# OSU-NLP-Group/saev

Measured on AMD Instinct MI355X. Metric: activations/sec (train step), d_in=1024 x32 k=32, higher is better.
Workload: dtype f32 (encoder: fp16 MFMA first pass with a rigorous error margin, survivors recomputed exactly in fp32; all else fp32)

## Files before the change

### saev_amd/csrc/ctx.hip

```cpp
#include <hip/hip_runtime.h>

#include <algorithm>
#include <cmath>
#include <cstdio>
#include <cstdlib>
#include <cstring>
#include <dlfcn.h>
#include <mutex>
#include <string>
#include <vector>

#include "kernels.h"

namespace {
constexpr int AUX_KSPLIT_MAX = 16;
constexpr int CAND_CAP = 4096;
constexpr int CAND_STRIDE = CAND_CAP + 256;
constexpr int TIMING_RING = 512;
constexpr int DEAD_LAG = 4;
constexpr int DEAD_RING = 16;
enum { AUX_NONE = 0, AUX_SMALL_DEVICE = 1, AUX_SMALL_HOST = 2, AUX_DENSE = 3 };
}

struct saev_ctx {
    saev_cfg cfg{};
    saev_debug_cfg dbg{};
    int device = 0;
    std::string err;
    float* params = nullptr;
    float* grads = nullptr;
    float* adam_m = nullptr;
    float* adam_v = nullptr;
    long n_params = 0;
    long off_W_dec = 0, off_b_dec = 0, off_W_enc = 0, off_b_enc = 0;
    int shard_world = 1;
    long chunk_a = 0, chunk_b = 0;
    double* sumsq_bound = nullptr;
    hipEvent_t wdec_ready = nullptr;
    hipEvent_t wenc_ready = nullptr;
    std::vector<void*> allocs;
    size_t scratch_bytes = 0, aux_bytes = 0;
    int cuts_last[MAX_PREFIXES] = {0};
    int32_t *cand_cnt = nullptr, *gmax = nullptr, *cand_idx = nullptr;
    int gmax_stride = 0;
    float* cand_val = nullptr;
    float* h_dense = nullptr;
    int32_t *idx = nullptr, *aux_idx = nullptr;
    float *val = nullptr, *aux_val = nullptr;
    float *x_hat = nullptr, *g = nullptr, *g_aux = nullptr;
    RowStats* rowstats = nullptr;
    uint32_t* bitmap = nullptr;
    int32_t* grp_prefix = nullptr;
    int32_t* scan_totals = nullptr;
    int32_t csc_epoch = 0;
    int bitmap_words = 0;
    int back_rows = 0;
    int bitmap_words_last = 0;
    bool bitmap_clean = false;
    int bitmap_clean_words = 0;
    int bitmap_prefill_words = 0, bitmap_prefill_rows = 0;
    bool last_backward_gathered = false;
    int32_t *counts = nullptr, *starts = nullptr;
    int2* pairs = nullptr;
    float* colsum_partials = nullptr;
    float* dval_pairs = nullptr;
    double *sumsq_partials = nullptr, *sumsq_total = nullptr;
    bool wenc_sq_valid = false;
    float2* row_proj = nullptr;
    float* enc_sq = nullptr;
    bool row_proj_valid = false, tail_proj_in_adam = false;
    bool wenc_t_pending = false;
    int64_t* toks = nullptr;
    int32_t *fired = nullptr, *dead = nullptr;
    int32_t* flags = nullptr;
    int32_t *chunk_starts = nullptr, *part_starts = nullptr, *work_latent = nullptr;
    float *dW_encT = nullptr, *partials = nullptr, *db_partials = nullptr;
    bool dws_ok = false;
    int dws_rows = 0;
    bool dws_pairs = false;
    float *gS = nullptr, *xS = nullptr, *dvp = nullptr;
    float* xS_ov = nullptr;
    float* xS_bwd = nullptr;
    float* dval_rows = nullptr;
    bool dval_fwd = false;
    float* wn2 = nullptr;
    float* sq_wave = nullptr;
    int sq_wave_n = 0;
    bool wn2_fresh = false;
    float* WdS = nullptr;
    double* dec_part = nullptr;
    bool wds_fresh = false;
    bool dval_pairs_ready = false;
    bool fused_forward = false;
    bool fwd_slices = false;
    bool fwd_step = false;
    float* rs_part = nullptr;
    float* xS_c = nullptr;
    int2 *pv = nullptr, *pv2 = nullptr;
    int32_t *plat = nullptr, *cut_lat = nullptr, *cut_list = nullptr;
    int32_t* lat_unused = nullptr;
    bool fused_step = false;
    bool unused_valid = false;
    int P = 1;
    int32_t cuts[MAX_PREFIXES] = {0};
    float* G = nullptr;
    float* GS = nullptr;
    int P_cap = 0;
    int n_dead_host = 0, k_use_host = 0;
    int64_t tokens_seen = 0;
    bool tracker_dirty = false;
    int nd_cap = 0;
    DeadRecord* rec_host = nullptr;
    DeadRecord* rec_dev = nullptr;
    hipEvent_t dead_ev[DEAD_RING];
    bool dead_ev_created = false;
    int64_t dead_steps = 0;
    int64_t rec_valid_from = 1;
    int aux_route = AUX_NONE;
    int64_t n_readbacks = 0;
    std::vector<void*> aux_allocs;
    int32_t* dead_list = nullptr;
    float *Wenc_dead = nullptr, *Wdec_dead = nullptr, *H_dead = nullptr, *A_dead = nullptr, *dWd = nullptr, *dWe = nullptr,
          *dbe = nullptr, *aux_partials = nullptr, *WencT_dead = nullptr, *aux_small_part = nullptr, *aux_small_part2 = nullptr, *aux_small_partbe = nullptr;
    bool aux_dev_count = false;
    bool aux_small = false;
    int aux_mfma_bound = 0;
    int aux_ndp = AUX_SMALL_MAX;
    int aux_mfma_cap = AUX_SMALL_MAX;
    bool aux_mfma = false;
    bool aux_fused = false;
    bool aux_all = false;
    uint8_t* A_mask = nullptr;
    _Float16 *aux_ws1 = nullptr, *aux_ws2 = nullptr, *aux_xsA = nullptr, *aux_xsg = nullptr, *aux_kA = nullptr, *aux_kD = nullptr, *aux_kX = nullptr;
    bool aux_both = false;
    float* aux_parts = nullptr;
    int aux_kpad = 0;
    float *bias_dead = nullptr, *zero_bias = nullptr, *aux_scales = nullptr;
    float* aux_sync = nullptr;
    int aux_Dp2 = 0;
    float *row_margin = nullptr, *wnorm_scratch = nullptr, *surv_val = nullptr;
    int32_t *surv_idx = nullptr, *surv_cnt = nullptr, *surv_rng = nullptr;
    int rs_lat_range = 0, rs_n_ranges = 0;
    int32_t* tau_max = nullptr;
    float* heur_state = nullptr;
    float *f16r_scales = nullptr, *mu = nullptr, *xnorm = nullptr, *b_shift = nullptr, *dot_part = nullptr, *xabs_part = nullptr,
          *sq_part = nullptr, *wmax_prev = nullptr;
    bool wmax_known = false;
    bool mu_ready = false;
    bool stream_ok = false;
    float *WeS = nullptr;
    float *xn_part = nullptr, *amax_part = nullptr, *cmax_part = nullptr;
    float* b_seen = nullptr;
    int32_t *stale_host = nullptr, *stale_dev = nullptr;
    uint32_t* wchk = nullptr;
    float *mu_keep = nullptr, *xside_keep = nullptr;
    bool fwd_streamed = false;
    bool fwd_moves_mu = false;
    int64_t fwd_mu_serial = -1;
    bool borrow_streamed = false;
    bool follow_stream = false;
    bool wchk_valid = false;
    bool fwd_reused_wimg = false;
    uint32_t stale_salt = 0;
    int scale_par = 0;
    bool prep_valid = false;
    bool wimg_fresh = false;
    int64_t mu_serial = 0, wimg_mu_serial = -1;
    bool wimg_bf16_fresh = false;
    bool stream_step = false;
    bool stats_pending = false, stats_lists = false;
    bool aux_stats_pending = false;
    bool dead_list_ready = false;
    bool train_fused = false;
    const float* gather_pool = nullptr;
    const int64_t* gather_rows = nullptr;
    float *upper_c = nullptr, *mu_c = nullptr, *xnorm_c = nullptr, *xabs_c = nullptr;
    _Float16* xs_c = nullptr;
    saev_ctx* leader = nullptr;
    void* comm = nullptr;
    int comm_rank = 0, comm_world = 0;
    std::vector<saev_ctx*> followers;
    const float* xprep_x = nullptr;
    int xprep_n = 0;
    int64_t xprep_serial = 0;
    int64_t leader_serial_seen = 0;
    _Float16 *xs = nullptr, *ws = nullptr;
    int Dp = 0, S_pad = 0, MB_pad = 0;
    int max_work = 0, max_part = 0;
    float* upper = nullptr;
    saev_step_stats* stats = nullptr;
    double* stats_scratch = nullptr;
    int* tickets = nullptr;
    const float *ov_x = nullptr, *ov_g = nullptr, *ov_val = nullptr;
    const int32_t* ov_idx = nullptr;
    int ov_n = 0;
    float* db_aux = nullptr;
    bool trust_grads = false;
    const float* x_last = nullptr;
    int n_last = 0;
    int training_last = 0;
    int P_last = 1;
    bool timing = false;
    hipEvent_t ev_start[TIMING_RING], ev_stop[TIMING_RING];
    bool ev_created = false;
    long ev_count = 0;
};

#define HIPCHK(ctx, expr)                                                                    \
    do {                                                                                     \
        hipError_t _e = (expr);                                                              \
        if (_e != hipSuccess) {                                                              \
            (ctx)->err = std::string(#expr) + ": " + hipGetErrorString(_e);                  \
            return SAEV_HIP_ERROR;                                                           \
        }                                                                                    \
    } while (0)

#define REQUIRE(ctx, cond, code, msg)                                                        \
    do {                                                                                     \
        if (!(cond)) {                                                                       \
            (ctx)->err = (msg);                                                              \
            return (code);                                                                   \
        }                                                                                    \
    } while (0)

namespace {

template <typename T>
int alloc(saev_ctx* c, T** p, size_t count) {
    void* q = nullptr;
    if (count == 0) count = 1;
    hipError_t e = hipMalloc(&q, count * sizeof(T));
    if (e != hipSuccess) {
        c->err = std::string("hipMalloc failed: ") + hipGetErrorString(e);
        return SAEV_HIP_ERROR;
    }
// ... 56 lines not shown

int saev_create(const saev_cfg* cfg, int device, saev_ctx** out) { return saev_create_ex(cfg, nullptr, device, out); }

int saev_create_ex(const saev_cfg* cfg, const saev_debug_cfg* dbg, int device, saev_ctx** out) {
    if (!cfg || !out) return SAEV_INVALID_ARG;
    *out = nullptr;
    if (cfg->activation != SAEV_ACT_TOPK && cfg->activation != SAEV_ACT_RELU) return SAEV_INVALID_ARG;
    saev_cfg relu_cfg;
    if (cfg->activation == SAEV_ACT_RELU) {
        if (cfg->k_aux != 0) return SAEV_UNSUPPORTED;
        relu_cfg = *cfg;
        relu_cfg.top_k = 1;
        cfg = &relu_cfg;
    }
    if (cfg->d_model <= 0 || cfg->d_sae <= 0 || cfg->top_k <= 0 || cfg->max_batch <= 0) return SAEV_INVALID_ARG;
    if ((uint64_t)cfg->max_batch * CAND_STRIDE * 4ull >= (1ull << 32)) return SAEV_INVALID_ARG;
    if (cfg->d_model % 4 != 0 || cfg->d_sae % 4 != 0 || cfg->d_model > 4096) return SAEV_UNSUPPORTED;
    if (cfg->k_aux < 0 || cfg->k_aux > 1024) return SAEV_UNSUPPORTED;
    if (cfg->encoder_mode != SAEV_ENCODER_F32 && cfg->encoder_mode != SAEV_ENCODER_F16X3 && cfg->encoder_mode != SAEV_ENCODER_BF16 &&
        cfg->encoder_mode != SAEV_ENCODER_F16R)
        return SAEV_INVALID_ARG;
    saev_ctx* c = new saev_ctx();
    c->cfg = *cfg;
    c->cfg.top_k = std::min(cfg->top_k, cfg->d_sae);
    if (dbg != nullptr && dbg->struct_size > 0)
        std::memcpy(&c->dbg, dbg, std::min((size_t)dbg->struct_size, sizeof(saev_debug_cfg)));
    c->device = device;
    if (hipSetDevice(device) != hipSuccess) {
        delete c;
        return SAEV_HIP_ERROR;
    }
    const long S = cfg->d_sae, D = cfg->d_model, MB = cfg->max_batch, K = c->cfg.top_k, KA = cfg->k_aux;
    const long MBB = std::max<long>(MB, cfg->max_backward_rows);
    c->back_rows = (int)MBB;
    if ((uint64_t)MBB * K >= (1ull << 31)) { delete c; return SAEV_INVALID_ARG; }
    {
        saev_layout_t lay;
        saev_layout(cfg, &lay);
        c->shard_world = std::max(1, cfg->shard_world);
        c->chunk_a = lay.chunk_a; c->chunk_b = lay.chunk_b;
        c->off_W_dec = lay.off_W_dec; c->off_b_dec = lay.off_b_dec; c->off_W_enc = lay.off_W_enc; c->off_b_enc = lay.off_b_enc;
        c->n_params = lay.n_total;
    }
    int rc = SAEV_OK;
#define A(p, n) if (rc == SAEV_OK) rc = alloc(c, &c->p, (size_t)(n))
    c->gmax_stride = (int)((MB + 255) / 256 * 256);
    A(cand_cnt, MB); A(gmax, (size_t)64 * c->gmax_stride); A(cand_idx, MB * CAND_STRIDE); A(cand_val, MB * CAND_STRIDE);
    A(h_dense, MB * S);
    A(idx, MB * K); A(val, MB * K);
    if (KA > 0) { A(aux_idx, MB * KA); A(aux_val, MB * KA); A(g_aux, MB * D); A(dead_list, S); }
    A(x_hat, MB * D); A(g, MB * D);
    A(rowstats, MB);
    c->bitmap_words = (int)(((MBB + 31) / 32 + 7) / 8 * 8);
    A(bitmap, S * c->bitmap_words);
    A(grp_prefix, S * (c->bitmap_words / 8));
    A(scan_totals, ((S + 1023) / 1024) * 4);
    A(counts, S); A(starts, S + 1); A(pairs, MBB * K); A(dval_pairs, MBB * (size_t)cfg->top_k);
    {
        const long max_pairs = MBB * K;
        c->max_work = (int)(S + (max_pairs + DW_CHUNK - 1) / DW_CHUNK);
        c->max_part = (int)(2 * ((max_pairs + DW_CHUNK - 1) / DW_CHUNK) + 2);
    }
    A(chunk_starts, S + 1); A(part_starts, S); A(work_latent, c->max_work);
    A(dW_encT, S * D); A(partials, (size_t)c->max_part * 2 * D); A(db_partials, c->max_part); A(row_proj, S); A(enc_sq, S);
    {
        const bool rows_only = c->dbg.dw_route == 1;
        c->dws_ok = !rows_only && D % DWS_SLICE == 0 && (uint64_t)S * D * 4ull < (1ull << 32) && MBB < (1l << 24) &&
                    (uint64_t)MBB * K < (1ull << 31);
    }
    c->fwd_slices = c->cfg.encoder_mode == SAEV_ENCODER_F16R && (c->dbg.fwd_route == 0 || c->dbg.fwd_route == 2) && c->dbg.fused_chain == 0 && D % RS_SLICE == 0 &&
                    (uint64_t)S * 128ull < (1ull << 32) - 256ull && fused_supported(c->cfg);
    if (c->fwd_slices) {
        A(rs_part, (size_t)(D / RS_SLICE) * MB * REFINE_CAP); A(surv_rng, MB * RS_MAX_RANGES);
        c->rs_lat_range = (int)std::max<long>(RS_LAT_RANGE, ((S + RS_MAX_RANGES - 1) / RS_MAX_RANGES + 255) / 256 * 256);
        c->rs_n_ranges = (int)((S + c->rs_lat_range - 1) / c->rs_lat_range);
    }
    if (c->fwd_slices && !c->dws_ok) A(xS, MBB * D);
    if (c->dws_ok) {
        A(gS, MBB * D); A(xS, MBB * D); A(dvp, (size_t)(D / DWS_SLICE) * MBB * K);
        if (c->dbg.dw_route != 2 && decode_forms_dval((int)D, (int)K)) A(dval_rows, MB * K);
        if (c->dval_rows != nullptr && c->dbg.dw_route == 4 && decode_slices_supported((int)D, (int)S, (int)K, (int)K) && c->cfg.normalize_w_dec) {
            A(WdS, S * D); A(dec_part, (size_t)(D / 32) * MB * 3);
        }
        A(pv, MBB * K); A(pv2, MBB * K); A(plat, MBB * K); A(cut_lat, (MBB * K + DWS_RUN - 1) / DWS_RUN); A(cut_list, 4 * (1 + (MBB * K + DWS_RUN - 1) / DWS_RUN)); A(lat_unused, S);
        if (c->dval_rows != nullptr && c->dbg.fin_route == 0) { A(wn2, S); A(sq_wave, (size_t)2 * dw_slices_waves((int)D, (int)(MBB * K))); }
    }
    A(colsum_partials, ((MBB + 63) / 64) * D);
    A(sumsq_partials, 2 * 1024 + (S + 3) / 4 + 8 + transpose_blocks((int)S, (int)D)); A(sumsq_total, 1);
    if (c->cfg.encoder_mode != SAEV_ENCODER_F32 || KA > 0) {
        c->Dp = (int)((D + 31) / 32 * 32);
        c->S_pad = (int)((S + 255) / 256 * 256);
        c->MB_pad = (int)((MB + 255) / 256 * 256);
        A(zero_bias, std::max(S, D)); A(aux_scales, 16); A(aux_sync, absmax_parts_max((int)MB));
    }
    if (c->cfg.encoder_mode != SAEV_ENCODER_F32) {
        A(xs, (size_t)c->MB_pad * 2 * c->Dp);
        A(ws, (size_t)c->S_pad * 2 * c->Dp);
        A(row_margin, MB); A(wnorm_scratch, std::max((S + 3) / 4, 3 * ((S + 255) / 256))); A(f16r_scales, 16); A(mu, D); A(xnorm, 2 * MB); A(b_shift, S);
        A(xabs_part, (MB + 3) / 4);
        if (c->cfg.encoder_mode == SAEV_ENCODER_F16R) { A(dot_part, (size_t)2 * (c->Dp / 32) * c->S_pad); A(sq_part, (size_t)2 * (c->Dp / 32) * c->S_pad); A(wmax_prev, 1); }
        if (c->cfg.encoder_mode == SAEV_ENCODER_F16R) { A(surv_idx, MB * REFINE_CAP); A(surv_val, MB * REFINE_CAP); A(surv_cnt, MB); }
    }
    c->stream_ok = c->fwd_slices && c->cfg.bound_mode == 0 && c->dbg.prep_route == 0 && D % 32 == 0 && c->Dp == (int)D;
    if (c->stream_ok) {
        A(WeS, S * D); A(xn_part, (size_t)(D / 32) * c->MB_pad * 2);
        A(amax_part, (size_t)(c->MB_pad / 256) * (D / 32)); A(cmax_part, (size_t)(c->MB_pad / 256) * (D / 32)); A(b_seen, S);
        A(mu_keep, D); A(xside_keep, 4);
    }
    if (c->stream_ok || c->cfg.encoder_mode == SAEV_ENCODER_BF16) A(wchk, (size_t)2 * ((S + 255) / 256) * ((D + 31) / 32));
    A(toks, S); A(fired, S); A(dead, S); A(flags, 16); A(upper, 1); A(stats, 1);
    A(tau_max, MB); A(heur_state, 8); A(stats_scratch, STATS_SCRATCH_DOUBLES); A(tickets, 8); A(db_aux, D);
#undef A
    if (rc != SAEV_OK) {
        for (void* p : c->allocs) hipFree(p);
        delete c;
        return rc;
    }
    hipMemset(c->toks, 0, S * sizeof(int64_t));
    hipMemset(c->fired, 0, S * sizeof(int32_t));
    hipMemset(c->dead, 0, S * sizeof(int32_t));
    hipMemset(c->flags, 0, 16 * sizeof(int32_t));
    if (c->stream_ok || c->cfg.encoder_mode == SAEV_ENCODER_BF16) {
        void* hp = nullptr;
        if (hipHostMalloc(&hp, 64, hipHostMallocMapped) == hipSuccess &&
            hipHostGetDevicePointer(reinterpret_cast<void**>(&c->stale_dev), hp, 0) == hipSuccess) {
            c->stale_host = static_cast<int32_t*>(hp);
            c->stale_host[0] = 0; c->stale_host[1] = 0;
        } else {
            if (hp) hipHostFree(hp);
            c->stale_host = nullptr; c->stale_dev = nullptr;
        }
    }
    hipMemset(c->scan_totals, 0, ((S + 1023) / 1024) * 4 * sizeof(int32_t));
    hipMemset(c->stats, 0, sizeof(saev_step_stats));
    hipMemset(c->stats_scratch, 0, STATS_SCRATCH_DOUBLES * sizeof(double));
    hipMemset(c->tickets, 0, 8 * sizeof(int));
    {
        const float init[8] = {2.6f, 0.f, 0.f, 0.f, 0.f, 0.f, 0.f, 0.f};
        hipMemcpy(c->heur_state, init, sizeof(init), hipMemcpyHostToDevice);
    }
    hipMemset(c->rowstats, 0, MB * sizeof(RowStats));
    if (c->xs) hipMemset(c->xs, 0, (size_t)c->MB_pad * 2 * c->Dp * sizeof(_Float16));
    if (c->zero_bias) hipMemset(c->zero_bias, 0, std::max(S, D) * sizeof(float));
    if (c->f16r_scales) hipMemset(c->f16r_scales, 0, 16 * sizeof(float));
    if (KA > 0) {
        const int s4 = (int)((S + 3) / 4 * 4);
        const int want = cfg->aux_dead_cap > 0 ? cfg->aux_dead_cap : std::max(4096, 8 * (int)KA);
        const int cap = std::min((want + 3) / 4 * 4, s4);
        rc = alloc_aux_buffers(c, cap);
        if (rc == SAEV_OK) {
            void* h = nullptr;
            if (hipHostMalloc(&h, DEAD_RING * sizeof(DeadRecord), hipHostMallocMapped) != hipSuccess ||
                hipHostGetDevicePointer(reinterpret_cast<void**>(&c->rec_dev), h, 0) != hipSuccess) {
                rc = SAEV_HIP_ERROR;
            } else {
                c->rec_host = static_cast<DeadRecord*>(h);
                std::memset(h, 0, DEAD_RING * sizeof(DeadRecord));
                for (int i = 0; i < DEAD_RING && rc == SAEV_OK; ++i)
                    if (hipEventCreateWithFlags(&c->dead_ev[i], hipEventDisableTiming) != hipSuccess) rc = SAEV_HIP_ERROR;
                c->dead_ev_created = rc == SAEV_OK;
            }
        }
        if (rc != SAEV_OK) {
            for (void* q : c->allocs) hipFree(q);
            for (void* q : c->aux_allocs) hipFree(q);
            if (c->rec_host) hipHostFree(c->rec_host);
            delete c;
// ... 192 lines not shown
    c->ev_count = 0;
    return SAEV_OK;
}

float saev_last_encoder_ms(saev_ctx* c) {
    if (!c || !c->ev_created || c->ev_count == 0) return -1.f;
    const long n = std::min<long>(c->ev_count, TIMING_RING);
    double tot = 0;
    for (long i = 0; i < n; ++i) {
        float ms = 0.f;
        if (hipEventElapsedTime(&ms, c->ev_start[i], c->ev_stop[i]) != hipSuccess) return -1.f;
        tot += ms;
    }
    return (float)(tot / n);
}


int saev_normalize_w_dec(saev_ctx* c, void* stream) {
    if (!c) return SAEV_INVALID_ARG;
    REQUIRE(c, c->params, SAEV_NOT_BOUND, "parameters not bound");
    if (!c->cfg.normalize_w_dec) return SAEV_OK;
    HIPCHK(c, launch_normalize_rows(c->params + c->off_W_dec, c->cfg.d_sae, c->cfg.d_model, (hipStream_t)stream));
    return SAEV_OK;
}

static bool bind_x_sources(saev_ctx* c, const float* x, int n, bool allow_borrow) {
    saev_ctx* l = c->leader;
    const bool borrow = allow_borrow && l != nullptr && l->xprep_x == x && l->xprep_n == n && l->xprep_serial != c->leader_serial_seen;
    saev_ctx* src = borrow ? l : c;
    c->upper_c = src->upper; c->mu_c = src->mu; c->xnorm_c = src->xnorm; c->xabs_c = src->xabs_part; c->xs_c = src->xs;
    c->borrow_streamed = borrow && l->fwd_streamed && l->mu_keep != nullptr;
    if (c->borrow_streamed) c->mu_c = l->mu_keep;
    c->fwd_step = c->fwd_slices && (src == c || src->fwd_slices);
    c->xS_c = c->fwd_step ? src->xS : nullptr;
    if (borrow) c->leader_serial_seen = l->xprep_serial;
    return borrow;
}

static int wait_wenc(saev_ctx* c, hipStream_t s) {
    if (c->wenc_ready != nullptr) {
        hipEvent_t ev = c->wenc_ready;
        c->wenc_ready = nullptr;
        HIPCHK(c, hipStreamWaitEvent(s, ev, 0));
    }
    return SAEV_OK;
}

static int prepare_encoder(saev_ctx* c, const float* x, int n, int32_t* pre_flag, hipStream_t s,
                           const float* xmax_dev = nullptr, bool x_borrowed = false, bool defer_margins = false) {
    if (c->cfg.encoder_mode == SAEV_ENCODER_F32) return SAEV_OK;
    const int D = c->cfg.d_model, S = c->cfg.d_sae;
    const bool bf = c->cfg.encoder_mode == SAEV_ENCODER_BF16;
    if (c->cfg.encoder_mode == SAEV_ENCODER_F16R) {
        if (!c->wmax_known) {
            { int rcw = wait_wenc(c, s); if (rcw != SAEV_OK) return rcw; }
            HIPCHK(c, launch_transpose(c->params + c->off_W_enc, c->dW_encT, D, S, s));
            HIPCHK(c, launch_wnorm_max(c->dW_encT, S, D, c->wnorm_scratch, c->wmax_prev, s));
            c->wmax_known = true;
        }
        if (!x_borrowed) {
            if (!c->mu_ready) { HIPCHK(c, launch_colsum(x, n, D, c->colsum_partials, c->mu, 0, nullptr, s, 0, 1.0f / (float)n)); c->mu_serial++; }
            HIPCHK(c, launch_center_stats(x, c->mu, n, D, c->xnorm, c->xabs_part, s, xmax_dev));
        }
        c->mu_ready = false;
        if (c->borrow_streamed)
            HIPCHK(c, launch_follower_scales(c->leader->xside_keep, c->wmax_prev, scl(c), pre_flag != nullptr ? pre_flag : c->flags, 0, s));
        else
        HIPCHK(c, launch_f16r_scales(c->xabs_c, (n + 3) / 4, c->wmax_prev, scl(c), s));
        float* const wt_out = (c->fwd_step && c->stream_ok) ? c->WeS : c->dW_encT;
        if (!x_borrowed && c->wenc_ready == nullptr) {
            HIPCHK(c, launch_split_f16r(x, n, D, c->Dp, c->xs, scl(c), c->mu, c->params + c->off_W_enc, S, c->S_pad, c->ws,
                                        reinterpret_cast<double*>(c->dot_part), c->sq_part, wt_out, s, c->fwd_step ? c->xS : nullptr,
                                        c->fwd_step ? 1 : 0));
        } else {
            if (!x_borrowed) HIPCHK(c, launch_split_rows(x, n, D, c->Dp, c->xs, 2, s, 1.0f, scl(c), c->mu, c->fwd_step ? c->xS : nullptr));
            { int rcw = wait_wenc(c, s); if (rcw != SAEV_OK) return rcw; }
            HIPCHK(c, launch_split_wT(c->params + c->off_W_enc, D, S, c->S_pad, c->Dp, 1.0f, c->ws, 2, s, scl(c) + 1,
                                      c->mu_c, reinterpret_cast<double*>(c->dot_part), c->sq_part, wt_out, c->fwd_step ? 1 : 0));
        }
        c->wimg_fresh = c->stream_ok && c->fwd_step && !x_borrowed && c->leader == nullptr;
        c->wimg_mu_serial = c->mu_serial;
        HIPCHK(c, launch_bias_finish(reinterpret_cast<const double*>(c->dot_part), c->sq_part, c->Dp, S, c->S_pad,
                                     scl(c) + 1, c->params + c->off_b_enc, c->b_shift, c->wnorm_scratch, s, c->b_seen));
        if (!defer_margins)
            HIPCHK(c, launch_row_margins(c->xnorm_c, n, D, c->wnorm_scratch, (S + 255) / 256, scl(c), pre_flag,
                                         c->wmax_prev, c->row_margin, s));
        return SAEV_OK;
    }
    if (!x_borrowed) HIPCHK(c, launch_split_rows(x, n, D, c->Dp, c->xs, bf ? 1 : 0, s));
    { int rcw = wait_wenc(c, s); if (rcw != SAEV_OK) return rcw; }
    c->fwd_reused_wimg = bf && c->wimg_bf16_fresh;
    if (!(bf && c->wimg_bf16_fresh))
        HIPCHK(c, launch_split_wT(c->params + c->off_W_enc, D, S, c->S_pad, c->Dp, bf ? 1.0f : 256.0f, c->ws, bf ? 1 : 0, s));
    if (bf && c->dbg.prep_route == 0 && c->Dp == D && D % 32 == 0) c->wimg_bf16_fresh = true;
    return SAEV_OK;
}

static int run_encoder(saev_ctx* c, const float* x, int n, int epi, float* h_out, const int32_t* flag, int when,
                       hipStream_t s, bool predicted = false) {
    const bool f16r = c->cfg.encoder_mode == SAEV_ENCODER_F16R;
    if (c->cfg.encoder_mode != SAEV_ENCODER_F32 && !(f16r && epi == EPI_DENSE)) {
        const bool bf = c->cfg.encoder_mode == SAEV_ENCODER_BF16;
        EncodeF16Args a{};
        a.xs = c->xs_c; a.ws = c->ws;
        a.b_enc = f16r ? c->b_shift : c->params + c->off_b_enc;
        a.n_rows = n; a.Dp = c->Dp; a.S = c->cfg.d_sae; a.w_scale = (bf || f16r) ? 1.0f : 256.0f;
        a.scale_dev = f16r ? scl(c) : nullptr;
        a.arith = bf ? 1 : (f16r ? 2 : 0);
        a.row_margin = f16r ? c->row_margin : nullptr;
        const int enc_wgs = c->dbg.enc_wgs > 0 ? c->dbg.enc_wgs : 256;
        a.mfma32 = c->dbg.enc_mfma == 32 ? 1 : 0;
        a.s_splits = encoder_splits(n, a.S, encode_f16x3_tile_rows(), encode_f16x3_tile_latents(), enc_wgs);
        a.no_rot = c->dbg.enc_rot == 1 ? 1 : 0;
        a.h_out = h_out;
        a.ngroups = f16_ngroups(c); a.top_k = c->cfg.top_k;
        a.gmax = c->gmax; a.gmax_stride = c->gmax_stride; a.cand_cnt = c->cand_cnt; a.cand_val = c->cand_val; a.cand_idx = c->cand_idx;
        a.cand_cap = CAND_CAP; a.cand_stride = CAND_STRIDE;
        a.enable_flag = flag; a.enable_when = when;
        if (predicted) { a.heur_z = c->heur_state; a.tau_max = c->tau_max; }
        {
            const int rf = c->dbg.refresh_first > 0 ? c->dbg.refresh_first : 8, re = c->dbg.refresh_every;
            a.refresh_first = std::max(1, rf);
            a.refresh_every = (re >= 1 && (re & (re - 1)) == 0) ? re : 2;
            if (a.ngroups > 32 && re <= 0) a.refresh_every = 1;
        }
        HIPCHK(c, launch_encode_f16x3(a, epi, s));
        return SAEV_OK;
    }
    EncodeArgs a{};
    a.x = x;
    a.W_enc = c->params + c->off_W_enc;
    a.b_enc = c->params + c->off_b_enc;
    a.n_rows = n;
    a.D = c->cfg.d_model;
    a.S = c->cfg.d_sae;
    a.s_splits = encoder_splits(n, a.S, encode_gemm_tile_rows(), encode_gemm_tile_latents(), 512);
    a.h_out = h_out;
    a.ngroups = c->cfg.top_k <= 32 ? 32 : 64;
    a.gmax = c->gmax;
    a.gmax_stride = c->gmax_stride;
    a.cand_cnt = c->cand_cnt;
    a.cand_val = c->cand_val;
    a.cand_idx = c->cand_idx;
    a.cand_cap = CAND_CAP; a.cand_stride = CAND_STRIDE;
    a.enable_flag = flag;
    a.enable_when = when;
    HIPCHK(c, launch_encode_gemm(a, epi, s));
    return SAEV_OK;
}

int saev_encode_dense(saev_ctx* c, const float* x, int32_t n, float* h_out, void* stream) {
    if (!c) return SAEV_INVALID_ARG;
    REQUIRE(c, c->params, SAEV_NOT_BOUND, "parameters not bound");
    REQUIRE(c, x && h_out && n > 0, SAEV_INVALID_ARG, "saev_encode_dense: bad arguments");
    REQUIRE(c, n <= c->cfg.max_batch || c->cfg.encoder_mode == SAEV_ENCODER_F32, SAEV_INVALID_ARG,
            "saev_encode_dense: n_rows > max_batch");
    bind_x_sources(c, x, n, false);
    c->xprep_x = nullptr;
    if (c->cfg.encoder_mode != SAEV_ENCODER_F16R) {
        int rc = prepare_encoder(c, x, n, nullptr, (hipStream_t)stream);
        if (rc != SAEV_OK) return rc;
    }
    return run_encoder(c, x, n, EPI_DENSE, h_out, nullptr, 0, (hipStream_t)stream);
}

int saev_topk_dense(saev_ctx* c, const float* h, int32_t n, int32_t k, const int32_t* mask, int32_t* idx_out,
                    float* val_out, void* stream) {
    if (!c) return SAEV_INVALID_ARG;
    REQUIRE(c, h && idx_out && val_out && n > 0 && k > 0, SAEV_INVALID_ARG, "saev_topk_dense: bad arguments");
    REQUIRE(c, k <= c->cfg.d_sae, SAEV_INVALID_ARG, "saev_topk_dense: k > d_sae");
    SelectDenseArgs a{};
    a.h = h; a.n_rows = n; a.S = c->cfg.d_sae; a.k = k; a.mask = mask;
    a.idx_out = idx_out; a.val_out = val_out; a.out_stride = k;
    HIPCHK(c, launch_select_dense(a, (hipStream_t)stream));
    return SAEV_OK;
}

static int encode_topk_impl(saev_ctx* c, const float* x, int n, int32_t* idx_out, float* val_out,
                            const int32_t* pre_flag, hipStream_t s, const float* xmax_dev = nullptr, bool x_borrowed = false) {
    const int K = c->cfg.top_k;
    int32_t* need_dense = c->flags + 1;
    const bool f16r_mode = c->cfg.encoder_mode == SAEV_ENCODER_F16R;
    const bool predict_mode = fused_supported(c->cfg) && c->cfg.bound_mode != 0 && c->cfg.encoder_mode != SAEV_ENCODER_F32 &&
                              f16_ngroups(c) == 32;
    const bool one_launch_pre = fused_supported(c->cfg) && !predict_mode;
    if (c->follow_stream) {
        HIPCHK(c, launch_follower_scales(c->leader->xside_keep, c->wmax_prev, scl(c), const_cast<int32_t*>(pre_flag), 1, s));
    } else if (!c->stream_step) {
        int rc0 = prepare_encoder(c, x, n, const_cast<int32_t*>(pre_flag), s, xmax_dev, x_borrowed, one_launch_pre);
        if (rc0 != SAEV_OK) return rc0;
        rc0 = wait_wenc(c, s);
        if (rc0 != SAEV_OK) return rc0;
    }
    if (fused_supported(c->cfg)) {
        const int ng = c->cfg.encoder_mode == SAEV_ENCODER_F32 ? (c->cfg.top_k <= 32 ? 32 : 64) : f16_ngroups(c);
        const bool f16r = c->cfg.encoder_mode == SAEV_ENCODER_F16R;
        auto select_stage = [&](const int32_t* flag, int when, int32_t* bad, const int32_t* tau_max, int32_t* ovf = nullptr,
                                const int32_t* first_flag = nullptr) -> int {
            SelectCandArgs sc{};
            sc.cand_cnt = c->cand_cnt; sc.cand_val = c->cand_val; sc.cand_idx = c->cand_idx;
            sc.cand_cap = CAND_CAP; sc.cand_stride = CAND_STRIDE; sc.n_rows = n; sc.k = K;
            sc.idx_out = idx_out; sc.val_out = val_out; sc.out_stride = K;
            sc.enable_flag = first_flag ? first_flag : flag; sc.enable_when = when;
            sc.tau_max = tau_max; sc.invalid = bad; sc.ovf = ovf;
            if (f16r) {
                sc.row_margin = c->row_margin; sc.x = x; sc.W_encT = c->dW_encT; sc.b_enc = c->params + c->off_b_enc;
                sc.D = c->cfg.d_model; sc.refine_overflow = bad;
                sc.surv_idx = c->surv_idx; sc.surv_val = c->surv_val; sc.surv_cnt = c->surv_cnt;
                if (c->fwd_step) { sc.surv_rng = c->surv_rng; sc.lat_range = c->rs_lat_range; sc.n_ranges = c->rs_n_ranges; }
                const bool chain_fused = c->dbg.fused_chain != 0;
                if (chain_fused && tau_max == nullptr && first_flag != nullptr) {
                    HIPCHK(c, launch_select_refine(sc, s));
                    return SAEV_OK;
                }
                HIPCHK(c, launch_select_cand(sc, s));
                sc.enable_flag = flag; sc.ovf = nullptr;
                if (c->fwd_step) {
                    RefineSlicesArgs rs{};
                    rs.surv_idx = c->surv_idx; rs.surv_cnt = c->surv_cnt; rs.surv_val = c->surv_val; rs.surv_rng = c->surv_rng;
                    rs.xS = c->xS_c; rs.WeS = c->stream_ok ? c->WeS : c->dW_encT; rs.b_enc = sc.b_enc; rs.part = c->rs_part;
                    rs.n_rows = n; rs.S = c->cfg.d_sae; rs.D = c->cfg.d_model;
                    rs.lat_range = c->rs_lat_range; rs.n_ranges = c->rs_n_ranges;
                    rs.enable_flag = flag; rs.enable_when = when;
                    const bool fold = c->dbg.fwd_route != 2;
                    HIPCHK(c, launch_refine_slices(rs, s, !fold));
                    if (fold) { sc.sum_part = c->rs_part; sc.sum_bias = sc.b_enc; sc.sum_n = c->cfg.d_model / RS_SLICE; sc.sum_plane = (size_t)n * REFINE_CAP; }
                } else {
                    HIPCHK(c, launch_refine_exact(sc, s));
                }
                sc.row_margin = nullptr; sc.tau_max = nullptr;
                sc.cand_cnt = c->surv_cnt; sc.cand_val = c->surv_val; sc.cand_idx = c->surv_idx; sc.cand_cap = REFINE_CAP; sc.cand_stride = REFINE_CAP;
            }
            HIPCHK(c, launch_select_cand(sc, s));
            return SAEV_OK;
        };
        const bool predict = c->cfg.bound_mode != 0 && ng == 32 && c->cfg.encoder_mode != SAEV_ENCODER_F32;
        int32_t *bad1 = c->flags + 9, *run2 = c->flags + 10, *gate = c->flags + 11;
        if (predict) {
            HIPCHK(c, launch_heur_gate(c->heur_state, pre_flag, gate, s));
            HIPCHK(c, launch_encoder_init(c->cand_cnt, n, c->gmax, 0, s, c->tau_max));
            timing_begin(c, s);
            int rc = run_encoder(c, x, n, EPI_TOPK, nullptr, gate, 0, s, true);
            if (rc != SAEV_OK) return rc;
            timing_end(c, s);
            HIPCHK(c, launch_overflow_check(c->cand_cnt, n, CAND_CAP, gate, bad1, c->flags + 2, c->flags + 3, s, need_dense,
                                            nullptr, c->heur_state + 3, nullptr, pre_flag));
            rc = select_stage(bad1, 0, bad1, c->tau_max);
            if (rc != SAEV_OK) return rc;
            HIPCHK(c, launch_heur_update(c->heur_state, bad1, c->heur_state + 3, K, gate, s));
            HIPCHK(c, launch_encoder_init(c->cand_cnt, n, c->gmax, ng * c->gmax_stride, s, nullptr, bad1, 1));
            rc = run_encoder(c, x, n, EPI_TOPK, nullptr, bad1, 1, s);
            if (rc != SAEV_OK) return rc;
            HIPCHK(c, launch_overflow_check(c->cand_cnt, n, CAND_CAP, pre_flag, need_dense, c->flags + 2, c->flags + 3, s, need_dense,
                                            run2, nullptr, bad1));
            rc = select_stage(run2, 1, need_dense, nullptr);
            if (rc != SAEV_OK) return rc;
        } else {
            const int S_ = c->cfg.d_sae;
            if (c->stream_step) {
                const int D_ = c->cfg.d_model;
                XprepArgs xp{};
                xp.x = c->gather_pool != nullptr ? c->gather_pool : x; xp.rows = c->gather_rows; xp.x_out = c->gather_pool != nullptr ? const_cast<float*>(x) : nullptr;
                xp.n = n; xp.D = D_; xp.nks = D_ / 32; xp.n_pad = c->MB_pad; xp.scales = scl(c); xp.mu = c->mu; xp.xs = c->xs; xp.xS = c->xS;
                xp.xn_part = c->xn_part; xp.col_part = c->colsum_partials; xp.amax_part = c->amax_part; xp.cmax_part = c->cmax_part;
                xp.W_enc = c->params + c->off_W_enc; xp.WeS = c->WeS; xp.b_enc = c->params + c->off_b_enc; xp.b_seen = c->b_seen;
                xp.S = S_; xp.salt = ++c->stale_salt; xp.stale = c->flags + 12;
                if (!c->followers.empty()) { xp.mu_keep = c->mu_keep; xp.xside_keep = c->xside_keep; }
                HIPCHK(c, launch_xprep(xp, s));
                PreEncode2Args pe{};
                pe.cand_cnt = c->cand_cnt; pe.n_rows = n; pe.gmax = c->gmax; pe.n_gmax = ng * c->gmax_stride;
                pe.xn_part = c->xn_part; pe.nks = D_ / 32; pe.n_pad = c->MB_pad; pe.D = D_;
                pe.wg_part = c->wnorm_scratch; pe.n_part = (S_ + 255) / 256; pe.scales = scl(c); pe.scales_next = scl_next(c);
                pe.pre_flag = const_cast<int32_t*>(pre_flag); pe.wmax_prev = c->wmax_prev; pe.margin = c->row_margin; pe.xnorm = c->xnorm;
                pe.flags1 = c->flags + 1; pe.col_part = c->colsum_partials; pe.n_rowblk = (n + 255) / 256; pe.mu = c->mu;
                pe.inv_n = 1.0f / (float)n; pe.update_mu = c->train_fused ? 1 : 0;
                pe.amax_part = c->amax_part; pe.cmax_part = c->cmax_part; pe.n_img = ((n + 255) / 256) * (D_ / 32);
                pe.upper = c->upper; pe.stats = c->stats; pe.stale = c->flags + 12; pe.stale_host = c->stale_dev;
                pe.xside_keep = c->followers.empty() ? nullptr : c->xside_keep;
                HIPCHK(c, launch_pre_encode2(pe, s));
                if (c->train_fused) c->mu_serial++;
            } else
            HIPCHK(c, launch_pre_encode(c->cand_cnt, n, c->gmax, ng * c->gmax_stride, f16r_mode ? c->xnorm_c : nullptr, c->cfg.d_model,
                                        c->wnorm_scratch, (S_ + 255) / 256, f16r_mode ? scl(c) : nullptr, const_cast<int32_t*>(pre_flag),
                                        c->wmax_prev, c->row_margin, c->flags + 1, s));
            timing_begin(c, s);
            int rc = run_encoder(c, x, n, EPI_TOPK, nullptr, pre_flag, 0, s);
            if (rc != SAEV_OK) return rc;
            timing_end(c, s);
            rc = select_stage(need_dense, 0, need_dense, nullptr, c->flags + 1, pre_flag);
            if (rc != SAEV_OK) return rc;
        }
    } else {
        HIPCHK(c, launch_init_i32(need_dense, 1, 1, s));
        HIPCHK(c, hipMemsetAsync(c->flags + 2, 0, 2 * sizeof(int32_t), s));
        timing_begin(c, s);
        timing_end(c, s);
    }
    int rc = run_encoder(c, x, n, EPI_DENSE, c->h_dense, need_dense, 1, s);
    if (rc != SAEV_OK) return rc;
    SelectDenseArgs sd{};
    sd.h = c->h_dense; sd.n_rows = n; sd.S = c->cfg.d_sae; sd.k = K;
    sd.idx_out = idx_out; sd.val_out = val_out; sd.out_stride = K;
    sd.enable_flag = need_dense; sd.enable_when = 1;
    HIPCHK(c, launch_select_dense(sd, s));
    return SAEV_OK;
}

int saev_encode_topk(saev_ctx* c, const float* x, int32_t n, int32_t* idx_out, float* val_out, void* stream) {
    if (!c) return SAEV_INVALID_ARG;
    REQUIRE(c, c->cfg.activation == SAEV_ACT_TOPK, SAEV_UNSUPPORTED, "saev_encode_topk: a ReLU context runs the forward entries only");
    REQUIRE(c, c->params, SAEV_NOT_BOUND, "parameters not bound");
    REQUIRE(c, x && idx_out && val_out && n > 0 && n <= c->cfg.max_batch, SAEV_INVALID_ARG,
            "saev_encode_topk: bad arguments (n_rows must be in 1..max_batch)");
    hipStream_t s = (hipStream_t)stream;
    HIPCHK(c, hipMemsetAsync(c->flags, 0, sizeof(int32_t), s));
    bind_x_sources(c, x, n, false);
    c->xprep_x = nullptr;
    c->stream_step = false;
    c->follow_stream = false;
    return encode_topk_impl(c, x, n, idx_out, val_out, c->flags, s);
}

int saev_scatter_dense(saev_ctx* c, const int32_t* idx, const float* val, int32_t n, int32_t k, float* f_out,
                       void* stream) {
    if (!c) return SAEV_INVALID_ARG;
    REQUIRE(c, idx && val && f_out && n > 0 && k > 0, SAEV_INVALID_ARG, "saev_scatter_dense: bad arguments");
    HIPCHK(c, launch_scatter_dense(idx, val, n, k, k, c->cfg.d_sae, f_out, (hipStream_t)stream));
    return SAEV_OK;
}

int saev_decode_sparse(saev_ctx* c, const int32_t* idx, const float* val, int32_t n, int32_t k,
                       const int64_t* prefixes_host, int32_t n_prefixes, float* x_hats_out, void* stream) {
    if (!c) return SAEV_INVALID_ARG;
    REQUIRE(c, c->params, SAEV_NOT_BOUND, "parameters not bound");
    REQUIRE(c, idx && val && x_hats_out && n > 0 && k > 0, SAEV_INVALID_ARG, "saev_decode_sparse: bad arguments");
    const int S = c->cfg.d_sae, D = c->cfg.d_model;
    int64_t single = S;
    if (!prefixes_host) { prefixes_host = &single; n_prefixes = 1; }
    REQUIRE(c, n_prefixes >= 1 && prefixes_host[n_prefixes - 1] == S && prefixes_host[0] >= 1, SAEV_INVALID_ARG,
            "prefixes must end at d_sae and start at >= 1");
    for (int p = 1; p < n_prefixes; ++p)
        REQUIRE(c, prefixes_host[p] > prefixes_host[p - 1], SAEV_INVALID_ARG, "prefixes must be strictly increasing");
    REQUIRE(c, n <= c->cfg.max_batch || n_prefixes == 1, SAEV_INVALID_ARG, "n_rows > max_batch");
    hipStream_t s = (hipStream_t)stream;
    for (int p = 0; p < n_prefixes; ++p) {
        DecodeArgs a{};
        a.x = nullptr;
        a.idx = idx; a.val = val; a.code_stride = k; a.k = k;
        a.W_dec = c->params + c->off_W_dec; a.b_dec = c->params + c->off_b_dec;
        a.n_rows = n; a.D = D; a.S = S; a.idx_limit = (int)prefixes_host[p];
// ... 530 lines not shown
                c->aux_route = AUX_SMALL_DEVICE;
                return auxk_small_forward(c, s, bound);
            }
            if ((bound + 3) / 4 * 4 <= c->nd_cap) {
                c->aux_route = AUX_DENSE;
                c->aux_dev_count = true;
                c->n_dead_host = bound;
                c->k_use_host = std::min(c->cfg.k_aux, bound);
                return auxk_forward(c, s);
            }
        }
    }
    int32_t host[2] = {0, 0};
    HIPCHK(c, hipMemcpyAsync(host, c->flags + 4, 2 * sizeof(int32_t), hipMemcpyDeviceToHost, s));
    HIPCHK(c, hipStreamSynchronize(s));
    c->n_readbacks++;
    c->n_dead_host = host[0];
    c->k_use_host = host[1];
    if (c->n_dead_host <= 0) return SAEV_OK;
    if ((c->n_dead_host + 3) / 4 * 4 > c->nd_cap && !(c->n_dead_host <= small_max && c->cfg.d_model <= 2048)) {
        const int s4 = (S + 3) / 4 * 4;
        const int cap = std::min(s4, std::max(2 * c->nd_cap, (2 * c->n_dead_host + 1023) / 1024 * 1024));
        for (void* q : c->aux_allocs) hipFree(q);
        c->aux_allocs.clear();
        c->aux_bytes = 0;
        c->nd_cap = 0;
        int rcg = alloc_aux_buffers(c, cap);
        if (rcg != SAEV_OK) {
            c->err = "AuxK: " + std::to_string(c->n_dead_host) + " dead latents exceed saev_cfg.aux_dead_cap and the buffers could not be grown to " +
                     std::to_string(cap) + " (out of device memory)";
            return rcg;
        }
        std::fprintf(stderr, "[saev_amd] AuxK: %d dead latents exceeded the dead-set buffers; grown to %d inside the step "
                             "(device-synchronising; saev_cfg.aux_dead_cap sizes them up front)\n", c->n_dead_host, cap);
    }
    if (c->n_dead_host <= small_max && c->cfg.d_model <= 2048) {
        c->aux_route = AUX_SMALL_HOST;
        return auxk_small_forward(c, s, c->n_dead_host);
    }
    c->aux_route = AUX_DENSE;
    return auxk_forward(c, s);
}


int saev_backward_begin(saev_ctx* c, void* stream) {
    if (!c) return SAEV_INVALID_ARG;
    REQUIRE(c, c->x_last && c->training_last, SAEV_INVALID_ARG, "saev_backward_begin: no training forward in flight");
    REQUIRE(c, c->grads, SAEV_NOT_BOUND, "gradient buffer not bound");
    hipStream_t s = (hipStream_t)stream;
    const int S = c->cfg.d_sae, D = c->cfg.d_model, K = c->cfg.top_k;
    const bool ov = c->ov_x != nullptr;
    const int n = ov ? c->ov_n : c->n_last;
    const int words = ((n + 31) / 32 + 7) / 8 * 8;
    c->row_proj_valid = false;
    CscArgs a{};
    a.idx = ov ? c->ov_idx : c->idx; a.code_stride = K; a.k = K; a.k_dev = nullptr; a.n_rows = n; a.S = S;
    a.bitmap = c->bitmap; a.words = words; a.grp_prefix = c->grp_prefix; a.scan_totals = c->scan_totals;
    a.counts = c->counts; a.starts = c->starts; a.pairs = c->pairs;
    a.chunk_starts = c->chunk_starts; a.part_starts = c->part_starts; a.work_latent = c->work_latent;
    const bool ov_slices = ov && c->dws_ok && c->P_last == 1 && n <= c->back_rows;
    c->dws_pairs = ov ? ov_slices : c->dws_rows == n;
    if (ov_slices) {
        c->xS_bwd = c->xS;
        if (!c->followers.empty()) {
            if (c->xS_ov == nullptr) {
                int rca = alloc(c, &c->xS_ov, (size_t)c->back_rows * D);
                if (rca != SAEV_OK) return rca;
            }
            c->xS_bwd = c->xS_ov;
        }
        HIPCHK(c, launch_slice_major_copy(c->ov_g, c->ov_x, n, D, c->gS, c->xS_bwd, s));
        c->dws_rows = 0;
    }
    c->csc_epoch = c->csc_epoch == 0x7fffffff ? 1 : c->csc_epoch + 1;
    a.epoch = c->dbg.csc_route == 2 ? 0 : c->csc_epoch;
    if (c->dws_pairs) {
        a.zero_word = c->cut_list;
        a.pv = c->pv; a.plat = c->plat; a.val = ov ? c->ov_val : c->val;
        a.P = c->P_last;
        for (int p = 0; p < c->P_last; ++p) a.cuts[p] = c->cuts_last[p];
        if (!ov && c->dval_fwd) { a.pv2 = c->pv2; a.dval = c->dval_rows; }
    }
    c->dval_pairs_ready = c->dws_pairs && a.pv2 != nullptr;
    if (c->fused_step && c->dws_pairs) { a.pairs = nullptr; a.chunk_starts = nullptr; a.part_starts = nullptr; a.work_latent = nullptr; }
    const float* gmat = ov ? c->ov_g : (c->P_last > 1 ? c->G : c->g);
    const bool prefilled = !ov && c->bitmap_prefill_words == words && c->bitmap_prefill_rows == n;
    HIPCHK(c, launch_csc_build(a, s, c->bitmap_clean && words <= c->bitmap_clean_words, gmat, D, (long)c->P_last * D,
                               c->colsum_partials, c->grads + c->off_b_dec, prefilled));
    c->bitmap_prefill_words = 0;
    c->last_backward_gathered = ov;
    c->bitmap_clean = false;
    c->bitmap_words_last = words;
    if (c->aux_route != AUX_NONE) {
        int rc = auxk_backward(c, s);
        if (rc != SAEV_OK) return rc;
    }
    return SAEV_OK;
}

int saev_backward_rows(saev_ctx* c, int32_t lat_lo, int32_t lat_hi, void* stream) {
    return saev_backward_rows_part(c, lat_lo, lat_hi, 0, stream);
}

int saev_backward_rows_part(saev_ctx* c, int32_t lat_lo, int32_t lat_hi, int32_t part, void* stream) {
    if (!c) return SAEV_INVALID_ARG;
    REQUIRE(c, part >= 0 && part <= 2, SAEV_INVALID_ARG, "saev_backward_rows_part: part must be 0 (both), 1 (decoder) or 2 (encoder)");
    REQUIRE(c, c->x_last && c->training_last && c->grads, SAEV_INVALID_ARG, "saev_backward_rows: call saev_backward_begin first");
    const int S = c->cfg.d_sae, D = c->cfg.d_model, K = c->cfg.top_k;
    const bool ov = c->ov_x != nullptr;
    const int n = ov ? c->ov_n : c->n_last;
    REQUIRE(c, 0 <= lat_lo && lat_lo < lat_hi && lat_hi <= S, SAEV_INVALID_ARG, "saev_backward_rows: bad latent range");
    hipStream_t s = (hipStream_t)stream;
    DwRowsArgs a{};
    a.starts = c->starts; a.chunk_starts = c->chunk_starts; a.work_latent = c->work_latent;
    a.part_starts = c->part_starts; a.pairs = c->pairs; a.val = ov ? c->ov_val : c->val; a.W_dec = c->params + c->off_W_dec;
    a.g = ov ? c->ov_g : (c->P_last > 1 ? c->G : c->g);
    a.x = ov ? c->ov_x : c->x_last;
    a.D = D; a.S = S; a.k_dev = nullptr; a.accumulate = 0;
    a.P = c->P_last;
    for (int p = 0; p < c->P_last; ++p) a.cuts[p] = c->cuts_last[p];
    a.dW_dec = c->grads + c->off_W_dec; a.dW_encT = c->dW_encT; a.db_enc = c->grads + c->off_b_enc;
    a.partials = c->partials; a.db_partials = c->db_partials;
    a.lat_lo = lat_lo; a.lat_hi = lat_hi;
    a.part = part; a.dval = c->dval_pairs;
    const bool all_rows = part == 0 && lat_lo == 0 && lat_hi == S;
    const bool clears = part != 2 && lat_lo == 0 && lat_hi == S && c->bitmap_words_last > 0;
    if (clears) { a.clear_bitmap = c->bitmap; a.clear_words = c->bitmap_words_last; }
    a.row_proj = all_rows ? c->row_proj : nullptr; a.project = c->cfg.remove_parallel_grads ? 1 : 0;
    a.enc_sq = all_rows ? c->enc_sq : nullptr;
    const int max_work = (lat_hi - lat_lo) + (int)(((long)n * K + DW_CHUNK - 1) / DW_CHUNK);
    if (lat_lo == 0 && lat_hi == S && c->dws_pairs && (ov || c->dws_rows == n)) {
        DwSlicesArgs w{};
        w.starts = c->starts; w.pv = c->pv; w.pv2 = c->pv2; w.plat = c->plat; w.gS = c->P_last > 1 ? c->GS : c->gS; w.W_dec = a.W_dec; w.P = c->P_last;
        w.xS = ov ? c->xS_bwd : (c->fwd_step ? c->xS_c : c->xS);
        w.n_rows = n; w.D = D; w.S = S; w.pair_cap = (int)((long)c->back_rows * K);
        w.dvp = c->dvp; w.dW_dec = a.dW_dec; w.dW_encT = a.dW_encT; w.db_enc = a.db_enc;
        const size_t runs_cap = ((size_t)w.pair_cap + DWS_RUN - 1) / DWS_RUN;
        w.part_dec = c->partials; w.part_enc = c->partials + 2 * runs_cap * D;
        w.cut_lat = c->cut_lat; w.cut_list = c->cut_list;
        w.lat_unused = (all_rows && c->fused_step) ? c->lat_unused : nullptr;
        c->unused_valid = w.lat_unused != nullptr;
        w.row_proj = a.row_proj; w.project = a.project; w.enc_sq = a.enc_sq;
        w.clear_bitmap = a.clear_bitmap; w.clear_words = a.clear_words;
        w.have_dval = c->dval_pairs_ready ? 1 : 0;
        c->sq_wave_n = 0;
        if (c->dval_pairs_ready && c->wn2_fresh && part == 0) {
            w.wn2 = c->wn2;
            if (c->fused_step && all_rows && c->sq_wave != nullptr && c->dbg.fin_route != 2) {
                c->sq_wave_n = dw_slices_waves(D, (int)((long)n * K));
                w.sq_wave_dec = c->sq_wave; w.sq_wave_enc = c->sq_wave + c->sq_wave_n;
            }
        }
        HIPCHK(c, launch_dw_slices(w, (int)((long)n * K), part, s));
    } else {
        c->unused_valid = false;
        HIPCHK(c, launch_dw_rows(a, max_work, s));
    }
    if (c->aux_route == AUX_DENSE)
        HIPCHK(c, launch_scatter_add_dead(c->dead_list, c->n_dead_host, D, c->dWd, c->dWe, c->dbe, c->grads + c->off_W_dec,
                                          c->dW_encT, c->grads + c->off_b_enc, lat_lo, lat_hi, s,
                                          c->aux_dev_count ? c->flags + 4 : nullptr, part, a.row_proj, a.W_dec, a.project, a.enc_sq,
                                          c->unused_valid ? c->lat_unused : nullptr, c->sq_wave_n > 0 ? c->starts : nullptr));
    else if (c->aux_route != AUX_NONE)
        HIPCHK(c, launch_scatter_add_dead(c->dead_list, c->aux_mfma ? c->aux_ndp : AUX_SMALL_MAX, D, c->dWd, c->dWe, c->dbe, c->grads + c->off_W_dec,
                                          c->dW_encT, c->grads + c->off_b_enc, lat_lo, lat_hi, s, c->flags + 4, part,
                                          a.row_proj, a.W_dec, a.project, a.enc_sq, c->unused_valid ? c->lat_unused : nullptr,
                                          c->sq_wave_n > 0 ? c->starts : nullptr));
    if (ov && c->aux_route != AUX_NONE && part != 2 && lat_lo == 0)
        HIPCHK(c, launch_colsum(c->db_aux, 1, D, c->colsum_partials, c->grads + c->off_b_dec, 1, nullptr, s));
    c->row_proj_valid = all_rows;
    if (clears) { c->bitmap_clean = true; c->bitmap_clean_words = c->bitmap_words_last; }
    return SAEV_OK;
}

float* saev_grad_w_enc_t(saev_ctx* c) { return c ? c->dW_encT : nullptr; }

int saev_bind_w_enc_t(saev_ctx* c, float* scratch) {
    if (!c || !scratch) return SAEV_INVALID_ARG;
    c->dW_encT = scratch;
    return SAEV_OK;
}

int saev_copy_step_state(saev_ctx* c, int32_t n_rows, float* g_out, int32_t* idx_out, float* val_out, void* stream) {
    if (!c) return SAEV_INVALID_ARG;
    REQUIRE(c, c->n_last > 0 && c->training_last && n_rows == c->n_last, SAEV_INVALID_ARG,
            "saev_copy_step_state: n_rows must be the row count of the training forward in flight");
    hipStream_t s = (hipStream_t)stream;
    const size_t nk = (size_t)n_rows * c->cfg.top_k, nd = (size_t)n_rows * c->cfg.d_model * (size_t)c->P_last;
    if (g_out) HIPCHK(c, hipMemcpyAsync(g_out, c->P_last > 1 ? c->G : c->g, nd * sizeof(float), hipMemcpyDeviceToDevice, s));
    if (idx_out) HIPCHK(c, hipMemcpyAsync(idx_out, c->idx, nk * sizeof(int32_t), hipMemcpyDeviceToDevice, s));
    if (val_out) HIPCHK(c, hipMemcpyAsync(val_out, c->val, nk * sizeof(float), hipMemcpyDeviceToDevice, s));
    return SAEV_OK;
}

int saev_backward_override(saev_ctx* c, const float* x_all, const float* g_all, const int32_t* idx_all, const float* val_all,
                           int32_t n_all) {
    if (!c) return SAEV_INVALID_ARG;
    if (x_all == nullptr) { c->ov_x = nullptr; c->ov_n = 0; return SAEV_OK; }
    REQUIRE(c, g_all && idx_all && val_all && n_all > 0, SAEV_INVALID_ARG, "saev_backward_override: NULL buffer");
    REQUIRE(c, n_all <= c->back_rows, SAEV_INVALID_ARG,
            "saev_backward_override: the gathered row count exceeds saev_cfg.max_backward_rows (set it to the GLOBAL batch)");
    REQUIRE(c, c->x_last && c->training_last, SAEV_INVALID_ARG, "saev_backward_override: no training forward in flight");
    REQUIRE(c, ((uintptr_t)x_all % 16) == 0 && ((uintptr_t)g_all % 16) == 0, SAEV_INVALID_ARG, "x_all / g_all must be 16-byte aligned");
    c->ov_x = x_all; c->ov_g = g_all; c->ov_idx = idx_all; c->ov_val = val_all; c->ov_n = n_all;
    return SAEV_OK;
}

int32_t saev_aux_compact_rows(const saev_ctx* c) {
    if (!c || c->aux_route == AUX_NONE) return 0;
    return c->aux_route == AUX_DENSE ? (c->n_dead_host + 3) / 4 * 4 : (c->aux_mfma ? c->aux_ndp : AUX_SMALL_MAX);
}

static int aux_compact_copy(saev_ctx* c, float* buf, bool out, hipStream_t s) {
    const size_t rows = (size_t)saev_aux_compact_rows(c), D = c->cfg.d_model;
    if (rows == 0) return SAEV_OK;
    REQUIRE(c, buf != nullptr, SAEV_INVALID_ARG, "saev_aux_compact_*: NULL buffer");
    float* seg[4] = {c->dWd, c->dWe, c->dbe, c->db_aux};
    const size_t len[4] = {rows * D, rows * D, rows, D};
    size_t off = 0;
    for (int i = 0; i < 4; ++i) {
        if (out) HIPCHK(c, hipMemcpyAsync(buf + off, seg[i], len[i] * sizeof(float), hipMemcpyDeviceToDevice, s));
        else HIPCHK(c, hipMemcpyAsync(seg[i], buf + off, len[i] * sizeof(float), hipMemcpyDeviceToDevice, s));
        off += len[i];
    }
    return SAEV_OK;
}
int saev_aux_compact_export(saev_ctx* c, float* buf, void* stream) {
    if (!c) return SAEV_INVALID_ARG;
    return aux_compact_copy(c, buf, true, (hipStream_t)stream);
}
// ... 68 lines not shown
    if (rc != SAEV_OK) return rc;
    hipStream_t s = (hipStream_t)stream;
    const long S = c->cfg.d_sae, D = c->cfg.d_model;
    c->tail_proj_in_adam = false;
    if (c->wenc_t_pending) {
        REQUIRE(c, c->row_proj_valid && shard_rank < 0, SAEV_INVALID_ARG, "saev_tail_prepare: pending transposed gradient without a full backward");
        c->row_proj_valid = false;
        HIPCHK(c, launch_sumsq_final_ex(nullptr, 0, c->row_proj, (int)S, c->grads + S * D, r.a_hi - S * D,
                                        c->grads + c->off_b_enc, r.b_hi - c->off_b_enc, saev_sumsq_device(c), c->sumsq_partials,
                                        c->tickets + 1, s, c->enc_sq, c->sq_wave_n > 0 ? c->sq_wave : nullptr, 2l * c->sq_wave_n));
        c->sq_wave_n = 0;
        c->tail_proj_in_adam = true;
        return SAEV_OK;
    }
    if (c->trust_grads && c->wenc_sq_valid && c->row_proj_valid && shard_rank < 0) {
        c->wenc_sq_valid = false; c->row_proj_valid = false;
        const double* tsq = c->sumsq_partials + 2 * sumsq_blocks() + (S + 3) / 4;
        HIPCHK(c, launch_sumsq_final_ex(tsq, transpose_blocks((int)S, (int)D), c->row_proj, (int)S, c->grads + S * D, r.a_hi - S * D,
                                        c->grads + c->off_b_enc, r.b_hi - c->off_b_enc, saev_sumsq_device(c), c->sumsq_partials,
                                        c->tickets + 1, s));
        c->tail_proj_in_adam = true;
        return SAEV_OK;
    }
    c->row_proj_valid = false;
    const long row_lo = std::min(r.a_lo / D, S), row_hi = std::min(r.a_hi / D, S);
    const int n_rows = (int)(row_hi - row_lo);
    const int nb = sumsq_blocks();
    double* part = c->sumsq_partials;
    HIPCHK(c, launch_rpg(c->grads + row_lo * D, c->params + row_lo * D, n_rows, (int)D, s, part + 2 * nb,
                         c->cfg.remove_parallel_grads ? 1 : 0));
    const long rest_lo = std::max(r.a_lo, S * D);
    HIPCHK(c, launch_sumsq_partials(c->grads + rest_lo, std::max(0L, r.a_hi - rest_lo), part, s));
    c->wenc_sq_valid = false;
    HIPCHK(c, launch_sumsq_partials(c->grads + r.b_lo, r.b_hi - r.b_lo, part + nb, s));
    HIPCHK(c, launch_sumsq_final(part, 2 * nb + (n_rows + 3) / 4, saev_sumsq_device(c), s));
    return SAEV_OK;
}

int saev_tail_apply(saev_ctx* c, float lr, float max_norm, float grad_scale, int64_t adam_step, int32_t shard_rank,
                    void* stream) {
    if (!c) return SAEV_INVALID_ARG;
    REQUIRE(c, c->cfg.activation == SAEV_ACT_TOPK, SAEV_UNSUPPORTED, "saev_tail_apply: a ReLU context runs the forward entries only");
    REQUIRE(c, c->params && c->grads && c->adam_m && c->adam_v, SAEV_NOT_BOUND,
            "saev_tail_apply: params/grads/adam state not bound");
    REQUIRE(c, adam_step >= 1, SAEV_INVALID_ARG, "adam_step is 1-based");
    TailRanges r;
    int rc = tail_ranges(c, shard_rank, &r);
    if (rc != SAEV_OK) return rc;
    hipStream_t s = (hipStream_t)stream;
    c->wn2_fresh = false;
    const bool emit_follow = c->leader != nullptr && c->borrow_streamed && c->leader->fwd_moves_mu && c->dbg.group_route == 0 &&
                             c->cfg.encoder_mode == SAEV_ENCODER_F16R && c->fwd_step;
    const bool emit = c->train_fused && c->stream_ok && (c->leader == nullptr ? c->prep_valid && (c->followers.empty() || c->dbg.group_route == 0) : emit_follow) &&
                      shard_rank < 0 && c->tail_proj_in_adam && c->wenc_t_pending;
    c->wimg_fresh = false;
    const bool chk_was_valid = c->wchk_valid;
    c->wchk_valid = false;
    const bool emit_bf16 = c->train_fused && c->cfg.encoder_mode == SAEV_ENCODER_BF16 && c->wimg_bf16_fresh && shard_rank < 0 &&
                           c->tail_proj_in_adam && c->wenc_t_pending;
    c->wimg_bf16_fresh = false;
    AdamArgs a{};
    a.lr = lr; a.beta1 = 0.9f; a.beta2 = 0.999f; a.eps = 1e-8f;
    a.omb1 = (float)(1.0 - 0.9); a.omb2 = (float)(1.0 - 0.999);
    a.bc1 = (float)(1.0 - std::pow(0.9, (double)adam_step));
    a.bc2_sqrt = (float)std::sqrt(1.0 - std::pow(0.999, (double)adam_step));
    a.grad_scale = grad_scale; a.max_norm = max_norm; a.sumsq = saev_sumsq_device(c); a.stats = c->stats;
    const long lo[2] = {r.a_lo, r.b_lo}, hi[2] = {r.a_hi, r.b_hi};
    if (shard_rank < 0 && c->tail_proj_in_adam && c->wenc_t_pending) {
        c->tail_proj_in_adam = false; c->wenc_t_pending = false;
        const long S = c->cfg.d_sae, D = c->cfg.d_model;
        a.p = c->params; a.g = c->grads; a.m = c->adam_m; a.v = c->adam_v; a.n = c->n_params;
        AdamImageArgs im{};
        if (emit) {
            if (!c->stream_step) HIPCHK(c, hipMemcpyAsync(scl_next(c), scl(c), 8 * sizeof(float), hipMemcpyDeviceToDevice, s));
            im.ws = c->ws; im.WeS = c->WeS; im.dot_part = reinterpret_cast<double*>(c->dot_part); im.sq_part = c->sq_part;
            im.mu = c->leader != nullptr ? c->leader->mu : c->mu; im.wmax_prev = c->wmax_prev; im.scales_next = scl_next(c); im.nks = c->Dp / 32; im.S_pad = c->S_pad;
        }
        if (emit_bf16) { im.ws = c->ws; im.nks = c->Dp / 32; im.S_pad = c->S_pad; im.mode = 1; }
        if ((emit || emit_bf16) && c->wchk != nullptr && c->dbg.own_check == 0) {
            im.chk = c->wchk; im.late = c->stale_dev != nullptr ? c->stale_dev + 1 : nullptr;
            im.verify = (chk_was_valid && c->fwd_reused_wimg && im.late != nullptr) ? 1 : 0;
            im.early = (emit && c->leader == nullptr) ? c->flags + 13 : nullptr;
        }
        HIPCHK(c, launch_adam_fused(a, c->row_proj, c->dW_encT, (int)S, (int)D, S * D, c->off_W_enc - S * D, c->off_W_enc,
                                    c->off_b_enc, c->n_params - c->off_b_enc, s, c->unused_valid ? c->lat_unused : nullptr,
                                    (emit || emit_bf16) ? &im : nullptr));
        c->unused_valid = false;
        c->wchk_valid = (emit || emit_bf16) && c->wchk != nullptr && c->dbg.own_check == 0;
        c->wimg_bf16_fresh = emit_bf16;
        if (emit) {
            HIPCHK(c, launch_bias_finish(reinterpret_cast<const double*>(c->dot_part), c->sq_part, c->Dp, (int)S, c->S_pad, scl_next(c) + 1,
                                         c->params + c->off_b_enc, c->b_shift, c->wnorm_scratch, s, c->b_seen));
            c->scale_par ^= 1;
            c->wimg_fresh = true;
            c->wimg_mu_serial = c->leader != nullptr ? c->leader->mu_serial : c->mu_serial;
        }
        return SAEV_OK;
    }
    if (shard_rank < 0 && c->tail_proj_in_adam) {
        c->tail_proj_in_adam = false;
        const long S = c->cfg.d_sae, D = c->cfg.d_model;
        a.p = c->params; a.g = c->grads; a.m = c->adam_m; a.v = c->adam_v; a.n = S * D;
        HIPCHK(c, launch_adam_rows(a, c->row_proj, (int)S, (int)D, s));
        a.p += S * D; a.g += S * D; a.m += S * D; a.v += S * D; a.n = c->n_params - S * D;
        HIPCHK(c, launch_adam(a, s));
        return SAEV_OK;
    }
    c->tail_proj_in_adam = false;
    if (shard_rank < 0) {
        a.p = c->params; a.g = c->grads; a.m = c->adam_m; a.v = c->adam_v; a.n = c->n_params;
        HIPCHK(c, launch_adam(a, s));
        return SAEV_OK;
    }
    for (int h = 0; h < 2; ++h) {
        a.p = c->params + lo[h]; a.g = c->grads + lo[h]; a.m = c->adam_m + lo[h]; a.v = c->adam_v + lo[h]; a.n = hi[h] - lo[h];
        HIPCHK(c, launch_adam(a, s));
    }
    return SAEV_OK;
}

int saev_step_tail(saev_ctx* c, float lr, float max_norm, float grad_scale, int64_t adam_step, void* stream) {
    int rc = saev_tail_prepare(c, -1, stream);
    if (rc != SAEV_OK) return rc;
    return saev_tail_apply(c, lr, max_norm, grad_scale, adam_step, -1, stream);
}

int saev_train_step_gather(saev_ctx* c, const float* pool, const int64_t* rows, float* x_out, int32_t n, float lr, float max_norm,
                           int64_t adam_step, void* stream) {
    if (!c) return SAEV_INVALID_ARG;
    REQUIRE(c, pool && rows && x_out, SAEV_INVALID_ARG, "saev_train_step_gather: NULL buffer");
    c->gather_pool = pool; c->gather_rows = rows;
    const int rc = saev_train_step(c, x_out, n, lr, max_norm, adam_step, stream);
    c->gather_pool = nullptr; c->gather_rows = nullptr;
    return rc;
}

int saev_params_touched(saev_ctx* c) {
    if (!c) return SAEV_INVALID_ARG;
    c->wchk_valid = false;
    c->wimg_fresh = false;
    c->wimg_bf16_fresh = false;
    c->wn2_fresh = false;
    return SAEV_OK;
}

int saev_train_step(saev_ctx* c, const float* x, int32_t n, float lr, float max_norm, int64_t adam_step,
                    void* stream) {
    if (!c) return SAEV_INVALID_ARG;
    c->fused_forward = c->dws_ok && c->GS != nullptr;
    c->train_fused = true;
    int rc = saev_step_forward(c, x, n, n, 1, stream);
    c->fused_forward = false;
    if (rc != SAEV_OK) { c->train_fused = false; return rc; }
    rc = saev_step_dead(c, n, stream);
    if (rc != SAEV_OK) { c->train_fused = false; return rc; }
    c->fused_step = true;
    rc = saev_backward_begin(c, stream);
    if (rc == SAEV_OK) rc = saev_backward_rows(c, 0, c->cfg.d_sae, stream);
    c->fused_step = false;
    if (rc != SAEV_OK) { c->train_fused = false; return rc; }
    c->wenc_t_pending = true;
    rc = saev_step_tail(c, lr, max_norm, 1.0f, adam_step, stream);
    c->wenc_t_pending = false;
    c->train_fused = false;
    return rc;
}

namespace {
struct RcclApi {
    void* lib = nullptr;
    int (*GetUniqueId)(void*) = nullptr;
    int (*CommInitRank)(void**, int, const void*, int) = nullptr;
    int (*CommDestroy)(void*) = nullptr;
    int (*CommAbort)(void*) = nullptr;
    int (*AllReduce)(const void*, void*, size_t, int, int, void*, hipStream_t) = nullptr;
// ... 100 lines not shown
```

### saev_amd/csrc/kernels.h

```cpp
#pragma once
#include <hip/hip_runtime.h>
#include <stdint.h>

#include "../../include/saev_amd.h"

enum { EPI_DENSE = 0, EPI_TOPK = 1 };

struct EncodeArgs {
    const float* x;
    const float* W_enc;
    const float* b_enc;
    int n_rows, D, S;
    int s_splits;
    float* h_out;
    int ngroups;
    int32_t* gmax;
    int gmax_stride;
    int32_t* cand_cnt;
    float* cand_val;
    int32_t* cand_idx;
    int cand_cap;
    int cand_stride;
    const int32_t* enable_flag;
    int enable_when;
// ... 77 lines not shown
hipError_t launch_pow2_scale(const float* absmax, float* pair, hipStream_t stream);
hipError_t launch_center_stats(const float* x, const float* mu, int n, int D, float* xnorm, float* wg_absmax,
                               hipStream_t stream, const float* xmax = nullptr);
hipError_t launch_row_margins(const float* xnorm, int n, int D, const float* wg_part, int n_part, const float* scales,
                              int32_t* pre_flag, float* wmax_prev, float* margin, hipStream_t stream);
hipError_t launch_overflow_check(const int32_t* cand_cnt, int n_rows, int cap, const int32_t* pre_flag,
                                 int32_t* need_dense, int32_t* n_overflow, int32_t* cand_max, hipStream_t stream,
                                 int32_t* dense_out = nullptr, int32_t* run_out = nullptr, float* cand_mean = nullptr,
                                 const int32_t* enable_flag = nullptr, const int32_t* dense_src = nullptr);

struct __attribute__((aligned(8))) RowStats {
    float sse_scaled;
    float l0;
    float l1;
    float aux_sse;
    double sse64;
    double sumsq64;
};

struct DecodeArgs {
    const float* x;
    const int32_t* idx;
    const float* val;
    int code_stride, k;
    const float* W_dec;
    const float* b_dec;
    int n_rows, D, S;
    int idx_limit;
    const float* upper;
    float gscale;
    int training;
    float* g;
    float* x_hat;
    int32_t* fired;
    RowStats* rowstats;
    float* gS;
    float* xS;
    float* dval_out;
    uint32_t* csc_bitmap;
    int csc_words;
};
hipError_t launch_decode(const DecodeArgs& a, hipStream_t stream);
bool decode_forms_dval(int D, int k);
bool decode_matry_forms_dval(int D, int k);
struct DecodeSliceArgs {
    DecodeArgs d;
    const float* WdS;
    double* part;
    float* dvp;
    long dvp_pitch;
};
bool decode_slices_supported(int D, int S, int k, int code_stride);
hipError_t launch_decode_slices(const DecodeSliceArgs& a, hipStream_t stream);

constexpr int MAX_PREFIXES = 16;
struct MatryArgs {
    int P;
    int32_t cuts[MAX_PREFIXES];
    float* G;
    int g_rows_all;
};
hipError_t launch_decode_matry(const DecodeArgs& a, const MatryArgs& m, hipStream_t stream);

struct CscArgs {
    const int32_t* idx;
    int code_stride, k;
    const int32_t* k_dev;
    int n_rows, S;
    uint32_t* bitmap;
    int words;
    int32_t* grp_prefix;
    int32_t* counts;
    int32_t* scan_totals;
    int32_t* starts;
    int2* pairs;
    int32_t* chunk_starts;
    int32_t* part_starts;
    int32_t* work_latent;
    int2* pv;
    int32_t* plat;
    const float* val;
    int2* pv2;
    const float* dval;
    int P;
    int32_t cuts[16];
    int32_t* zero_word;
    int32_t epoch;
};
hipError_t launch_csc_build(const CscArgs& a, hipStream_t stream, bool bitmap_clean = false, const float* colsum_m = nullptr,
                            int colsum_D = 0, long colsum_row_stride = 0, float* colsum_partials = nullptr,
                            float* colsum_out = nullptr, bool prefilled = false);

constexpr int DW_CHUNK = 64;

struct DwRowsArgs {
    const int32_t* starts;
    const int32_t* chunk_starts;
    const int32_t* work_latent;
    const int32_t* part_starts;
    const int2* pairs;
    const float* val;
    const float* W_dec;
    const float* g;
    const float* x;
    int D, S;
    int P;
    int32_t cuts[MAX_PREFIXES];
    const int32_t* k_dev;
    int accumulate;
    float* dW_dec;
    float* dW_encT;
    float* db_enc;
    float* partials;
    float* db_partials;
    int lat_lo, lat_hi;
    int part;
    float* dval;
    float2* row_proj;
    int project;
    float* enc_sq;
    uint32_t* clear_bitmap;
    int clear_words;
};
hipError_t launch_dw_rows(const DwRowsArgs& a, int max_work, hipStream_t stream);

constexpr int DWS_RUN = 64, DWS_SLICE = 32;
constexpr int DWS_FIRST = 1, DWS_LAST = 2, DWS_END = 4;
struct DwSlicesArgs {
    const int32_t* starts;
    const int2* pv;
    int2* pv2;
    const int32_t* plat;
    const float* gS;
    const float* xS;
    const float* W_dec;
    int n_rows, D, S, pair_cap;
    int P;
    float* dvp;
    float* dW_dec;
    float* dW_encT;
    float* db_enc;
    float* part_dec;
    float* part_enc;
    int32_t* cut_lat;
    int32_t* cut_list;
    float2* row_proj;
    int project;
    float* enc_sq;
    uint32_t* clear_bitmap;
    int clear_words;
    int32_t* lat_unused;
    int have_dval;
    const float* wn2;
    float* sq_wave_dec;
    float* sq_wave_enc;
};
hipError_t launch_dw_slices(const DwSlicesArgs& a, int max_pairs, int part, hipStream_t stream);
int dw_slices_waves(int D, int max_pairs);
hipError_t launch_slice_major_copy(const float* g, const float* x, int n, int D, float* gS, float* xS, hipStream_t stream);
hipError_t launch_transpose(const float* in, float* out, int S, int D, hipStream_t stream, double* sq_part = nullptr);
int transpose_blocks(int S, int D);

hipError_t launch_colsum(const float* m, int n_rows, int D, float* partials, float* out, int accumulate,
                         const int32_t* k_dev, hipStream_t stream, long row_stride = 0, float out_scale = 1.0f,
                         int col_mult = 0);
hipError_t launch_colsum_absmax(const float* m, int n_rows, int D, float* partials, float* out, float* wg_scratch,
                                float* absmax_out, hipStream_t stream, float out_scale = 1.0f,
                                saev_step_stats* zero_stats = nullptr, int32_t* zero_flag = nullptr);

hipError_t launch_normalize_rows(float* W, int S, int D, hipStream_t stream, float* WS = nullptr, float* wn2 = nullptr);
hipError_t launch_rpg(float* gW, const float* W, int S, int D, hipStream_t stream, double* sq_partials = nullptr,
                      int project = 1);
int sumsq_blocks();
hipError_t launch_sumsq_partials(const float* g, long n, double* partials, hipStream_t stream);
hipError_t launch_sumsq_final(const double* partials, int nb, double* total, hipStream_t stream);
hipError_t launch_sumsq(const float* g, long n, double* partials, double* total, hipStream_t stream);
struct AdamArgs {
    float* p; const float* g; float* m; float* v;
    long n;
    float lr, beta1, beta2, eps, bc1, bc2_sqrt;
    float omb1, omb2;
    float grad_scale;
    float max_norm;
    const double* sumsq;
    saev_step_stats* stats;
};
hipError_t launch_adam(const AdamArgs& a, hipStream_t stream);
hipError_t launch_adam_rows(const AdamArgs& a, const float2* row_proj, int S, int D, hipStream_t stream);
hipError_t launch_sumsq_final_ex(const double* partials, int nb, const float2* row_proj, int n_rows, const float* e1, long n1,
                                 const float* e2, long n2, double* total, double* blk_part, int* ticket, hipStream_t stream,
                                 const float* enc_sq = nullptr,
                                 const float* plain = nullptr, long n_plain = 0);
struct AdamImageArgs {
    _Float16* ws; float* WeS; double* dot_part; float* sq_part;
    const float* mu; const float* wmax_prev; float* scales_next;
    int nks, S_pad;
    int mode;
    uint32_t* chk; int32_t* late; int verify;
    const int32_t* early;
};
hipError_t launch_adam_fused(const AdamArgs& a, const float2* row_proj, const float* gT, int S, int D, long off_b_dec, long n_b_dec,
                             long off_W_enc, long off_b_enc, long n_b_enc, hipStream_t stream, const int32_t* lat_unused = nullptr,
                             const AdamImageArgs* img = nullptr);
constexpr int SUMSQ_EX_BLOCKS = 32;

struct DeadRecord {
    int64_t step;
    int64_t cum_tokens;
    int64_t horizon_tokens;
    int32_t n_dead;
    int32_t n_near;
};

struct DeadArgs {
    int64_t* toks;
    int32_t* fired;
    int32_t* dead;
    int S;
    int64_t add_tokens, threshold;
    int k_aux;
    int32_t* n_dead;
    int32_t* k_use;
    saev_step_stats* stats;
    int32_t* scratch;
    int64_t horizon_tokens;
    int64_t step, cum_tokens;
    DeadRecord* rec;
    int32_t* dead_list;
};
hipError_t launch_dead_update(const DeadArgs& a, hipStream_t stream);
hipError_t launch_stats_dead(const RowStats* rs, int n_rows, int D, int P, float alpha, const float* upper, const int32_t* n_overflow,
                             saev_step_stats* stats, double* scratch, const int32_t* cand_cnt, int cand_cap, const DeadArgs& d,
                             hipStream_t stream);
hipError_t launch_absmax(const float* x, long n, float* out_zeroed, hipStream_t stream);
hipError_t launch_gather_rows(const float* pool, const int64_t* rows, int n_rows, int D, float* out, hipStream_t stream);
hipError_t launch_scatter_dense(const int32_t* idx, const float* val, int n_rows, int k, int stride, int S, float* f,
                                hipStream_t stream);
hipError_t launch_stats_reduce(const RowStats* rs, int n_rows, int D, int P, float alpha, int with_aux, const float* upper,
                               const int32_t* n_overflow_and_max, saev_step_stats* stats, hipStream_t stream,
                               const int32_t* n_dead_dev, double* scratch,
                               const int32_t* cand_cnt = nullptr, int cand_cap = 0);
constexpr int STATS_SCRATCH_DOUBLES = 16 * 8 + 1;

struct EncodeF16Args {
    const _Float16* xs;
    const _Float16* ws;
    const float* b_enc;
    int n_rows, Dp, S;
    float w_scale;
    int arith;
    const float* row_margin;
    const float* scale_dev;
    const float* scale_dev_b;
    int s_splits;
    int no_rot;
    float* h_out;
    int ngroups;
    int top_k;
    int32_t* gmax;
    int gmax_stride;
    int32_t* cand_cnt;
    float* cand_val;
    int32_t* cand_idx;
    int cand_cap, cand_stride;
    const int32_t* enable_flag;
    int enable_when;
    const float* heur_z;
    int32_t* tau_max;
    int refresh_first, refresh_every;
    int n_batches;
    int blk_imgs;
    long out_bstride;
    int mfma32;
};
hipError_t launch_encode_f16x3(const EncodeF16Args& a, int epi, hipStream_t stream);
int encode_f16x3_tile_rows();
int encode_f16x3_tile_latents();
hipError_t launch_split_rows(const float* x, int n, int D, int Dp, void* xs, int mode, hipStream_t stream, float scale = 1.0f,
                             const float* scale_dev = nullptr,
                             const float* mu = nullptr,
                             float* xS = nullptr);
hipError_t launch_split_wT(const float* W, int D, int S, int S_pad, int Dp, float scale, void* ws, int mode,
                           hipStream_t stream, const float* scale_dev = nullptr,
                           const float* mu = nullptr, double* dot_part = nullptr, float* sq_part = nullptr,
                           float* W_T = nullptr,
                           int wt_slices = 0);
struct XprepArgs {
    const float* x;
    const int64_t* rows;
    float* x_out;
    int n, D, nks, n_pad;
    const float* scales;
    const float* mu;
    _Float16* xs;
    float* xS;
    float* xn_part;
    float* col_part;
    float* amax_part;
    float* cmax_part;
    const float* W_enc; const float* WeS; const float* b_enc; const float* b_seen;
    int S; uint32_t salt; int32_t* stale;
    float* mu_keep; float* xside_keep;
};
hipError_t launch_xprep(const XprepArgs& a, hipStream_t stream);
struct PreEncode2Args {
    int32_t* cand_cnt; int n_rows;
    int32_t* gmax; int n_gmax;
    const float* xn_part; int nks, n_pad, D;
    const float* wg_part; int n_part;
    const float* scales;
    float* scales_next;
    int32_t* pre_flag;
    float* wmax_prev;
    float* margin;
    float* xnorm;
    int32_t* flags1;
    const float* col_part; int n_rowblk;
    float* mu; float inv_n; int update_mu;
    const float* amax_part; const float* cmax_part; int n_img;
    float* upper;
    int32_t* stale; int32_t* stale_host;
    float* xside_keep;
    saev_step_stats* stats;
    int nb_rows;
};
hipError_t launch_pre_encode2(PreEncode2Args a, hipStream_t stream);
hipError_t launch_follower_scales(const float* xside, const float* wmax, float* scales, int32_t* pre_flag, int keep_w, hipStream_t stream);
hipError_t launch_split_both(const float* M, int R, int C, float scale, const float* scale_dev, void* rf, int kp_r, void* tf, int kp_t,
                             hipStream_t stream);
hipError_t launch_split_f16r(const float* x, int n, int D, int Dp, void* xs, const float* scales, const float* mu, const float* W,
                             int S, int S_pad, void* ws, double* dot_part, float* sq_part, float* W_T, hipStream_t stream,
                             float* xS = nullptr, int wt_slices = 0);
hipError_t launch_bias_finish(const double* dot_part, const float* sq_part, int Dp, int S, int S_pad, const float* w_scale,
                              const float* b_enc, float* b_shift, float* wg_part, hipStream_t stream, float* b_seen = nullptr);
hipError_t launch_max_reduce(const float* v, int n, float* out, hipStream_t stream);

hipError_t launch_dead_compact(const int32_t* dead, int S, int32_t* list, hipStream_t s,
                               const int32_t* n_dead_dev = nullptr);
hipError_t launch_gather_dead(const float* W_enc, const float* W_dec, const int32_t* dl, int nd, int ndp, int D, int S,
                              float* Wenc_dead, float* Wdec_dead, hipStream_t s,
                              const int32_t* nd_dev = nullptr);
hipError_t launch_dead_bias_vec(const float* b_enc, const int32_t* dl, int nd, int ndp, float* out, hipStream_t s,
                                bool pad_zero = false,
                                const int32_t* nd_dev = nullptr);
hipError_t launch_aux_scatter(const int32_t* idx, const float* val, int n_rows, int k, int stride, int ndp, float* A,
                              uint8_t* mask, hipStream_t s, const int32_t* k_dev = nullptr);
hipError_t launch_aux_resid(float* E, const float* x, const float* x_hat, const float* b_dec, int n_rows, int D,
                            float gscale, RowStats* rowstats, hipStream_t s, const int32_t* nd_dev = nullptr, float* part = nullptr,
                            float* pair = nullptr);
int absmax_parts_max(int n_rows_cap);
hipError_t launch_absmax_pow2(const float* x, long n, float* part, float* pair, hipStream_t s);
hipError_t launch_mask_apply_absmax(float* dA, const uint8_t* mask, long n, float* part, float* pair, hipStream_t s);
bool aux_select_supported(int ndp);
hipError_t launch_aux_select(const float* H, int n_rows, int ndp, int k, const int32_t* k_dev, float* A, uint8_t* mask, float* part,
                             float* pair, hipStream_t s);
hipError_t launch_mask_apply(float* dA, const uint8_t* mask, long n, hipStream_t s);
constexpr int AUX_SMALL_MAX = 64;
constexpr int AUX_SMALL_DEFAULT = 40;
hipError_t launch_gather_dead_small(const float* W_enc, const float* W_dec, const int32_t* dl, const int32_t* nd_dev, int D,
                                    int S, float* WencT_dead, float* Wdec_dead, hipStream_t s, int cap = AUX_SMALL_MAX);
hipError_t launch_aux_small_fwd(const float* x, const float* x_hat, const float* WencT_dead, const float* Wdec_dead,
                                const float* b_enc, const float* b_dec, const int32_t* dl, int n_rows, int D,
                                const int32_t* nd_dev, float gscale, float* A, float* dA, float* g_aux, RowStats* rowstats,
                                hipStream_t s);
hipError_t launch_aux_small_wsum(const float* part, int n_blk, int D, const int32_t* nd_dev, float* dWd, float* dWe, hipStream_t s,
                                 int ndp = AUX_SMALL_MAX);
constexpr int AUX_FUSED_MAX = 8;
constexpr int AUX_FUSED_ROWS = 32;
#ifndef AUX_FUSED_PF8
#define AUX_FUSED_PF8 1
#endif
#ifndef AUX_FUSED_PF4
#define AUX_FUSED_PF4 1
#endif
bool aux_fused_supported(int D);
constexpr int AUX_MFMA_MAX = 128;
bool aux_mfma_supported(int D);
hipError_t launch_aux_mfma_forward(const float* x, const float* x_hat, const float* WencT_dead, const float* Wdec_dead, const float* b_enc,
                                   const float* b_dec, const int32_t* dl, int n_rows, int D, const int32_t* nd_dev, float gscale, float* A,
                                   float* dA, float* g_aux, RowStats* rowstats, hipStream_t s, int bound, int ndp = AUX_SMALL_MAX);
hipError_t launch_aux_mfma_wgrad(const float* A, const float* dA, const float* g_aux, const float* x, int n_rows, int D,
                                 const int32_t* nd_dev, float* part, float* partb, float* partbe, hipStream_t s, int bound, int ndp = AUX_SMALL_MAX);
hipError_t launch_aux_fused_wsum(const float* part, int n_blk, int D, const int32_t* nd_dev, float* dWd, float* dWe, hipStream_t s,
                                 const float* partb, float* db_out, int db_accumulate, const float* partbe, float* dbe,
// ... 46 lines not shown
```

### saev_amd/csrc/select.hip

```cpp
#include "common.h"
#include "kernels.h"

namespace {

constexpr int SD_THREADS = 256;

__device__ __forceinline__ int block_excl_scan_256(int v, int* lds_wave_tot, int& total) {
    const int lane = threadIdx.x & 63, w = threadIdx.x >> 6;
    int incl = v;
#pragma unroll
    for (int o = 1; o < 64; o <<= 1) {
        int n = __shfl_up(incl, o, 64);
        if (lane >= o) incl += n;
    }
    if (lane == 63) lds_wave_tot[w] = incl;
    __syncthreads();
    int base = 0, tot = 0;
#pragma unroll
    for (int i = 0; i < 4; ++i) {
        const int t = lds_wave_tot[i];
        if (i < w) base += t;
        tot += t;
    }
    total = tot;
    __syncthreads();
    return base + incl - v;
}

__global__ __launch_bounds__(SD_THREADS) void select_dense_kernel(SelectDenseArgs a) {
    if (a.enable_flag != nullptr && (*a.enable_flag != 0) != (a.enable_when != 0)) return;
    __shared__ int hist[256];
    __shared__ int sh_digit, sh_need;
    __shared__ int wave_tot[4];

    const int row = blockIdx.x;
    const int S = a.S;
    int k = a.k_dev ? min(*a.k_dev, a.k) : a.k;
    if (a.k_dev && k <= 0) return;
    const float* h = a.h + (size_t)row * S;
    const int tid = threadIdx.x;
    const int S4 = S >> 2;

    uint32_t prefix = 0, pmask = 0;
    int need = k;

    for (int pass = 0; pass < 4; ++pass) {
        const int shift = 24 - 8 * pass;
        hist[tid] = 0;
        __syncthreads();
        for (int q = tid; q < S4; q += SD_THREADS) {
            const f32x4 v = *reinterpret_cast<const f32x4*>(h + 4 * q);
            int4 mk = {1, 1, 1, 1};
            if (a.mask) mk = *reinterpret_cast<const int4*>(a.mask + 4 * q);
            const int m[4] = {mk.x, mk.y, mk.z, mk.w};
#pragma unroll
            for (int e = 0; e < 4; ++e) {
                const uint32_t key = f2ukey(v[e]);
                if (m[e] != 0 && (key & pmask) == prefix) atomicAdd(&hist[(key >> shift) & 255], 1);
            }
        }
        __syncthreads();
        if (tid < 64) {
            const int c0 = hist[4 * tid], c1 = hist[4 * tid + 1], c2 = hist[4 * tid + 2], c3 = hist[4 * tid + 3];
            const int c = c0 + c1 + c2 + c3;
            int suf = c;
#pragma unroll
            for (int o = 1; o < 64; o <<= 1) {
                int n = __shfl_down(suf, o, 64);
                if (tid + o < 64) suf += n;
            }
            const unsigned long long ge = __ballot(suf >= need);
            const int L = 63 - __builtin_clzll(ge | 1ull);
            if (tid == L) {
                int running = suf - c;
                const int cs[4] = {c0, c1, c2, c3};
                int d = 4 * tid, nn = need;
                for (int j = 3; j >= 0; --j) {
                    if (running + cs[j] >= need) { d = 4 * tid + j; nn = need - running; break; }
                    running += cs[j];
                }
                sh_digit = d;
                sh_need = nn;
            }
        }
        __syncthreads();
        prefix |= (uint32_t)sh_digit << shift;
        pmask |= 0xFFu << shift;
        need = sh_need;
        __syncthreads();
    }
    const uint32_t T = prefix;
    int base_gt = 0, base_eq = 0;
    int32_t* oi = a.idx_out + (size_t)row * a.out_stride;
    float* ov = a.val_out + (size_t)row * a.out_stride;
    for (int q0 = 0; q0 < S4; q0 += SD_THREADS) {
        const int q = q0 + tid;
        f32x4 v = {0, 0, 0, 0};
        int flg[4] = {0, 0, 0, 0}, feq[4] = {0, 0, 0, 0};
        if (q < S4) {
            v = *reinterpret_cast<const f32x4*>(h + 4 * q);
            int4 mk = {1, 1, 1, 1};
            if (a.mask) mk = *reinterpret_cast<const int4*>(a.mask + 4 * q);
            const int m[4] = {mk.x, mk.y, mk.z, mk.w};
#pragma unroll
            for (int e = 0; e < 4; ++e) {
                const uint32_t key = f2ukey(v[e]);
                flg[e] = (m[e] != 0 && key > T);
                feq[e] = (m[e] != 0 && key == T);
            }
        }
        const int ngt = flg[0] + flg[1] + flg[2] + flg[3];
        const int neq = feq[0] + feq[1] + feq[2] + feq[3];
        int tot;
        const int ex = block_excl_scan_256(ngt | (neq << 16), wave_tot, tot);
        int gt_before = base_gt + (ex & 0xFFFF);
        int eq_before = base_eq + (ex >> 16);
#pragma unroll
        for (int e = 0; e < 4; ++e) {
            if (flg[e]) {
                const int pos = gt_before + min(eq_before, need);
                oi[pos] = 4 * q + e;
                ov[pos] = v[e];
                ++gt_before;
            } else if (feq[e]) {
                if (eq_before < need) {
                    const int pos = gt_before + eq_before;
                    oi[pos] = 4 * q + e;
                    ov[pos] = v[e];
                }
                ++eq_before;
            }
        }
        base_gt += tot & 0xFFFF;
        base_eq += tot >> 16;
    }
}


__device__ __forceinline__ float wave_reduce_scatter8(float (&p)[8], int lane) {
    int bit = 32;
#pragma unroll
    for (int h = 4; h >= 1; h >>= 1, bit >>= 1) {
        const bool up = (lane & bit) != 0;
#pragma unroll
        for (int i = 0; i < h; ++i) {
            const float keep = up ? p[i + h] : p[i];
            const float send = up ? p[i] : p[i + h];
            p[i] = keep + __shfl_xor(send, bit, 64);
        }
    }
    float r = p[0];
    for (; bit >= 1; bit >>= 1) r += __shfl_xor(r, bit, 64);
    return r;
}

__device__ __forceinline__ void sort_by_idx_and_store(const SelectCandArgs& a, int row, int k, int32_t my_idx, float my_val,
                                                      int lane) {
#pragma unroll
    for (int size = 2; size <= 64; size <<= 1) {
#pragma unroll
        for (int stride = size >> 1; stride > 0; stride >>= 1) {
            const int32_t o_idx = __shfl_xor(my_idx, stride, 64);
            const float o_val = __shfl_xor(my_val, stride, 64);
            const bool up = ((lane & size) == 0);
            const bool lower = ((lane & stride) == 0);
            const bool take_other = (lower == up) ? (o_idx < my_idx) : (o_idx > my_idx);
            if (take_other) { my_idx = o_idx; my_val = o_val; }
        }
    }
    if (lane < a.k) {
        const bool ok = lane < k;
        a.idx_out[(size_t)row * a.out_stride + lane] = ok ? my_idx : -1;
        a.val_out[(size_t)row * a.out_stride + lane] = ok ? my_val : 0.f;
    }
}

template <int EPL>
__device__ __forceinline__ void select_cand_row(const SelectCandArgs& a, int row, int n, int32_t (&s_idx)[4][64],
                                                float (&s_val)[4][64], const float* cv, const int32_t* ci) {
    const int lane = threadIdx.x & 63;
    const int w = threadIdx.x >> 6;
    const int k = min(a.k, n);

    uint32_t key[EPL];
    int32_t idx[EPL];
#pragma unroll
    for (int e = 0; e < EPL; ++e) {
        const int p = e * 64 + lane;
        if (p < n) { key[e] = f2ukey(cv[p]); idx[e] = ci[p]; }
        else { key[e] = 0u; idx[e] = 0x7fffffff; }
    }
    auto kth_largest = [&]() {
        uint32_t t = 0;
        for (int bit = 31; bit >= 0; --bit) {
            const uint32_t trial = t | (1u << bit);
            int c = 0;
#pragma unroll
            for (int e = 0; e < EPL; ++e) c += __popcll(__ballot(key[e] >= trial));
            if (c == k) {
                uint32_t m = 0xffffffffu;
#pragma unroll
                for (int e = 0; e < EPL; ++e) m = min(m, key[e] >= trial ? key[e] : 0xffffffffu);
#pragma unroll
                for (int o = 32; o > 0; o >>= 1) m = min(m, (uint32_t)__shfl_xor((int)m, o, 64));
                return m;
            }
            if (c > k) t = trial;
        }
        return t;
    };
    uint32_t T = kth_largest();
    if (a.tau_max != nullptr && lane == 0 && (n < a.k || ukey2f(T) < key2f(a.tau_max[row]))) *a.invalid = 1;
    if (a.row_margin != nullptr) {
        const uint32_t key_lo = f2ukey(ukey2f(T) - a.row_margin[row]);
        int32_t* so = a.surv_idx + (size_t)row * REFINE_CAP;
        int base = 0;
        const int n_rng = a.surv_rng != nullptr ? a.n_ranges : 1;
// ... 735 lines not shown
    if (threadIdx.x == 0) {
        const float m = *absmax;
        pair[0] = (m > 0.f && m < 3.0e38f) ? exp2f(13.0f - floorf(log2f(m))) : 1.0f;
        pair[1] = 1.0f;
    }
}
__global__ __launch_bounds__(256) void f16r_scales_kernel(const float* xmax_part, int n_part, const float* wmax, float* scales) {
    __shared__ float sh[4];
    float m = 0.f;
    for (int i = threadIdx.x; i < n_part; i += 256) m = fmaxf(m, xmax_part[i]);
    m = wave_max(m);
    if ((threadIdx.x & 63) == 0) sh[threadIdx.x >> 6] = m;
    __syncthreads();
    if (threadIdx.x == 0) {
        const float xm = fmaxf(fmaxf(sh[0], sh[1]), fmaxf(sh[2], sh[3])), wm = *wmax;
        scales[0] = (xm > 0.f && xm < 3.0e38f) ? exp2f(13.0f - floorf(log2f(xm))) : 1.0f;
        scales[1] = (wm > 0.f && wm < 3.0e38f) ? exp2f(13.0f - floorf(log2f(wm))) : 1.0f;
        scales[2] = scales[0];
        scales[3] = 1.0f;
    }
}

__global__ void overflow_check_kernel(const int32_t* cand_cnt, int n_rows, int cap, const int32_t* pre_flag,
                                      int32_t* bad_out, int32_t* n_overflow, int32_t* cand_max, int32_t* dense_out,
                                      int32_t* run_out, float* cand_mean, const int32_t* enable_flag,
                                      const int32_t* dense_src) {
    if (enable_flag != nullptr && *enable_flag == 0) {
        if (threadIdx.x == 0 && run_out != nullptr) *run_out = 0;
        return;
    }
    __shared__ int sh, shmax, shsum;
    if (threadIdx.x == 0) { sh = 0; shmax = 0; shsum = 0; }
    __syncthreads();
    int c = 0, m = 0, t = 0;
    for (int i = threadIdx.x; i < n_rows; i += blockDim.x) { const int v = cand_cnt[i]; c += (v > cap); m = max(m, v); t += min(v, cap); }
    c = wave_sum_i(c);
    t = wave_sum_i(t);
#pragma unroll
    for (int o = 32; o > 0; o >>= 1) m = max(m, __shfl_xor(m, o, 64));
    if ((threadIdx.x & 63) == 0) { if (c) atomicAdd(&sh, c); atomicMax(&shmax, m); atomicAdd(&shsum, t); }
    __syncthreads();
    if (threadIdx.x == 0) {
        const int pre = (pre_flag && *pre_flag) ? 1 : 0;
        *n_overflow = sh;
        *cand_max = shmax;
        if (cand_mean != nullptr) *cand_mean = (float)shsum / (float)max(n_rows, 1);
        if (run_out == nullptr) {
            *bad_out = (pre || sh > 0) ? 1 : 0;
            if (dense_out != nullptr) *dense_out = dense_src != nullptr ? (*dense_src != 0 ? 1 : 0) : pre;
        } else {
            const int dense = (*dense_out != 0 || sh > 0) ? 1 : 0;
            *dense_out = dense;
            *run_out = dense ? 0 : 1;
        }
    }
}

__global__ void heur_gate_kernel(float* state, const int32_t* pre_flag, int32_t* gate) {
    if (threadIdx.x != 0) return;
    int g = (pre_flag != nullptr && *pre_flag != 0) ? 1 : 0;
    if (state[5] > 0.f) { state[5] -= 1.f; g = 1; }
    *gate = g;
}
__global__ void heur_update_kernel(float* state, const int32_t* bad, const float* cand_mean, int k, const int32_t* gate) {
    if (threadIdx.x != 0 || *gate != 0) return;
    float z = state[0];
    state[2] += 1.f;
    if (*bad != 0) {
        z -= 0.3f;
        state[1] += 1.f;
        state[4] += 1.f;
        if (state[4] >= 3.f) { state[4] = 0.f; state[5] = 256.f; z = 1.5f; }
    } else {
        state[4] = 0.f;
        if (*cand_mean > 3.f * (float)k) z += 0.002f;
    }
    state[0] = fminf(fmaxf(z, 0.5f), 3.5f);
}

}

hipError_t launch_select_dense(const SelectDenseArgs& a, hipStream_t stream) {
    if (a.n_rows <= 0) return hipSuccess;
    hipLaunchKernelGGL(select_dense_kernel, dim3(a.n_rows), dim3(SD_THREADS), 0, stream, a);
    return hipGetLastError();
}

hipError_t launch_select_cand(const SelectCandArgs& a, hipStream_t stream) {
    if (a.n_rows <= 0) return hipSuccess;
    if (a.cand_cap > 4096 || (a.sum_part != nullptr && a.cand_cap > REFINE_CAP)) return hipErrorInvalidValue;
    if (a.k > 32) hipLaunchKernelGGL(select_cand_kernel<true>, dim3((a.n_rows + 3) / 4), dim3(256), 0, stream, a);
    else hipLaunchKernelGGL(select_cand_kernel<false>, dim3((a.n_rows + 3) / 4), dim3(256), 0, stream, a);
    return hipGetLastError();
}

hipError_t launch_init_i32(int32_t* p, int32_t v, int n, hipStream_t stream) {
    if (n <= 0) return hipSuccess;
    hipLaunchKernelGGL(init_i32_kernel, dim3((n + 255) / 256), dim3(256), 0, stream, p, v, n);
    return hipGetLastError();
}

hipError_t launch_encoder_init(int32_t* cand_cnt, int n_rows, int32_t* gmax, int n_gmax, hipStream_t stream, int32_t* tau_max,
                               const int32_t* enable_flag, int enable_when) {
    const int n = n_rows > n_gmax ? n_rows : n_gmax;
    if (n <= 0) return hipSuccess;
    hipLaunchKernelGGL(encoder_init_kernel, dim3((n + 255) / 256), dim3(256), 0, stream, cand_cnt, n_rows, gmax, n_gmax, tau_max,
                       enable_flag, enable_when);
    return hipGetLastError();
}
hipError_t launch_pre_encode(int32_t* cand_cnt, int n_rows, int32_t* gmax, int n_gmax, const float* xnorm, int D,
                             const float* wg_part, int n_part, const float* scales, int32_t* pre_flag, float* wmax_prev,
                             float* margin, int32_t* flags1, hipStream_t stream) {
    const int n = std::max(1, n_rows > n_gmax ? n_rows : n_gmax);
    hipLaunchKernelGGL(pre_encode_kernel, dim3((n + 255) / 256), dim3(256), 0, stream, cand_cnt, n_rows, gmax, n_gmax, xnorm, D,
                       wg_part, n_part, scales, pre_flag, wmax_prev, margin, flags1);
    return hipGetLastError();
}
hipError_t launch_follower_scales(const float* xside, const float* wmax, float* scales, int32_t* pre_flag, int keep_w, hipStream_t stream) {
    hipLaunchKernelGGL(follower_scales_kernel, dim3(1), dim3(64), 0, stream, xside, wmax, scales, pre_flag, keep_w);
    return hipGetLastError();
}
hipError_t launch_pre_encode2(PreEncode2Args a, hipStream_t stream) {
    a.nb_rows = (std::max(1, std::max(a.n_rows, a.n_gmax)) + 255) / 256;
    hipLaunchKernelGGL(pre_encode2_kernel, dim3(a.nb_rows + (a.D + 255) / 256), dim3(256), 0, stream, a);
    return hipGetLastError();
}
hipError_t launch_heur_gate(float* state, const int32_t* pre_flag, int32_t* gate, hipStream_t stream) {
    hipLaunchKernelGGL(heur_gate_kernel, dim3(1), dim3(64), 0, stream, state, pre_flag, gate);
    return hipGetLastError();
}
hipError_t launch_heur_update(float* state, const int32_t* bad, const float* cand_mean, int k, const int32_t* gate,
                              hipStream_t stream) {
    hipLaunchKernelGGL(heur_update_kernel, dim3(1), dim3(64), 0, stream, state, bad, cand_mean, k, gate);
    return hipGetLastError();
}
hipError_t launch_step_zero(saev_step_stats* stats, float* upper, int32_t* flag0, hipStream_t stream) {
    hipLaunchKernelGGL(step_zero_kernel, dim3(1), dim3(64), 0, stream, stats, upper, flag0);
    return hipGetLastError();
}

hipError_t launch_wnorm_max(const float* W_encT, int S, int D, float* wg_scratch, float* wmax, hipStream_t stream) {
    const int nwg = (S + 3) / 4;
    hipLaunchKernelGGL(rownorm_wgmax_kernel, dim3(nwg), dim3(256), 0, stream, W_encT, S, D, wg_scratch);
    hipLaunchKernelGGL(max_reduce_kernel, dim3(1), dim3(1024), 0, stream, wg_scratch, nwg, wmax);
    return hipGetLastError();
}
hipError_t launch_f16r_scales(const float* xmax_part, int n_part, const float* wmax, float* scales, hipStream_t stream) {
    hipLaunchKernelGGL(f16r_scales_kernel, dim3(1), dim3(256), 0, stream, xmax_part, n_part, wmax, scales);
    return hipGetLastError();
}
hipError_t launch_pow2_scale(const float* absmax, float* pair, hipStream_t stream) {
    hipLaunchKernelGGL(pow2_scale_kernel, dim3(1), dim3(64), 0, stream, absmax, pair);
    return hipGetLastError();
}
hipError_t launch_center_stats(const float* x, const float* mu, int n, int D, float* xnorm, float* wg_absmax,
                               hipStream_t stream, const float* xmax) {
    hipLaunchKernelGGL(center_stats_kernel, dim3((n + 3) / 4), dim3(256), 0, stream, x, mu, n, D, xnorm, wg_absmax, xmax);
    return hipGetLastError();
}
hipError_t launch_max_reduce(const float* v, int n, float* out, hipStream_t stream) {
    hipLaunchKernelGGL(max_reduce_kernel, dim3(1), dim3(1024), 0, stream, v, n, out);
    return hipGetLastError();
}
hipError_t launch_row_margins(const float* xnorm, int n, int D, const float* wg_part, int n_part, const float* scales,
                              int32_t* pre_flag, float* wmax_prev, float* margin, hipStream_t stream) {
    hipLaunchKernelGGL(row_margin_kernel, dim3((n + 255) / 256), dim3(256), 0, stream, xnorm, n, D, wg_part, n_part, scales,
                       pre_flag, wmax_prev, margin);
// ... 50 lines not shown
```

### saev_amd/csrc/sparse.hip

```cpp
#include "common.h"
#include "kernels.h"

namespace {

template <int NV>
__device__ __forceinline__ void gather_rows_accum(f32x4 (&acc)[NV], const float* __restrict__ W, int D, int D4,
                                                  const int32_t* idx_row, const float* val_row, int k, int limit,
                                                  int lane) {
    for (int j0 = 0; j0 < k; j0 += 64) {
        const int cnt = min(64, k - j0);
        int32_t my_i = -1;
        float my_v = 0.f;
        if (lane < cnt) { my_i = idx_row[j0 + lane]; my_v = val_row[j0 + lane]; }
#pragma unroll 4
        for (int jj = 0; jj < cnt; ++jj) {
            const int32_t i = __shfl(my_i, jj, 64);
            const float v = __shfl(my_v, jj, 64);
            if (i < 0 || i >= limit) continue;
            const f32x4* wr = reinterpret_cast<const f32x4*>(W + (size_t)i * D);
#pragma unroll
            for (int n = 0; n < NV; ++n) {
                const int q = lane + 64 * n;
                if (q < D4) {
                    const f32x4 w = wr[q];
// ... 500 lines not shown
    const uint4* bm = reinterpret_cast<const uint4*>(a.bitmap + (size_t)i * a.words);
    int base = 0;
    for (int g0 = 0; g0 < groups; g0 += 64) {
        const int g = g0 + lane;
        int c = 0;
        if (g < groups) {
            const uint4 lo = bm[2 * g], hi = bm[2 * g + 1];
            c = __popc(lo.x) + __popc(lo.y) + __popc(lo.z) + __popc(lo.w) + __popc(hi.x) + __popc(hi.y) + __popc(hi.z) + __popc(hi.w);
        }
        int incl = c;
#pragma unroll
        for (int o = 1; o < 64; o <<= 1) {
            const int n = __shfl_up(incl, o, 64);
            if (lane >= o) incl += n;
        }
        if (g < groups) a.grp_prefix[(size_t)i * groups + g] = base + incl - c;
        base += __shfl(incl, 63, 64);
    }
    if (lane == 0) a.counts[i] = base;
}
__global__ __launch_bounds__(256) void csc_count_kernel(CscArgs a) { csc_count_body(a, blockIdx.x); }

__global__ __launch_bounds__(1024) void csc_scan_block_kernel(CscArgs a) {
    if (a.k_dev && *a.k_dev <= 0) return;
    __shared__ int wave_tot[16][3];
    const int tid = threadIdx.x, lane = tid & 63, w = tid >> 6;
    const int i = blockIdx.x * 1024 + tid;
    int v[3] = {0, 0, 0};
    if (i < a.S) {
        const int c = a.counts[i];
        const int nch = (c + DW_CHUNK - 1) / DW_CHUNK;
        v[0] = c; v[1] = max(1, nch); v[2] = nch > 1 ? nch : 0;
    }
    int incl[3] = {v[0], v[1], v[2]};
#pragma unroll
    for (int o = 1; o < 64; o <<= 1) {
#pragma unroll
        for (int q = 0; q < 3; ++q) {
            const int n = __shfl_up(incl[q], o, 64);
            if (lane >= o) incl[q] += n;
        }
    }
    if (lane == 63)
        for (int q = 0; q < 3; ++q) wave_tot[w][q] = incl[q];
    __syncthreads();
    int off[3] = {0, 0, 0};
    for (int j = 0; j < w; ++j)
        for (int q = 0; q < 3; ++q) off[q] += wave_tot[j][q];
    if (i < a.S) {
        a.starts[i] = off[0] + incl[0] - v[0];
        if (a.chunk_starts) {
            a.chunk_starts[i] = off[1] + incl[1] - v[1];
            a.part_starts[i] = off[2] + incl[2] - v[2];
        }
    }
    if (tid == 1023)
        for (int q = 0; q < 3; ++q) a.scan_totals[blockIdx.x * 3 + q] = off[q] + incl[q];
}
__global__ __launch_bounds__(1024) void csc_scan_offset_kernel(CscArgs a) {
    if (a.k_dev && *a.k_dev <= 0) return;
    __shared__ int base[3];
    const int tid = threadIdx.x, lane = tid & 63;
    if (tid < 64) {
        int s3[3] = {0, 0, 0};
        for (int b = lane; b < (int)blockIdx.x; b += 64)
            for (int q = 0; q < 3; ++q) s3[q] += a.scan_totals[b * 3 + q];
        for (int q = 0; q < 3; ++q) s3[q] = wave_sum_i(s3[q]);
        if (lane == 0)
            for (int q = 0; q < 3; ++q) base[q] = s3[q];
    }
    __syncthreads();
    const int i = blockIdx.x * 1024 + tid;
    if (i < a.S) {
        a.starts[i] += base[0];
        if (a.chunk_starts) { a.chunk_starts[i] += base[1]; a.part_starts[i] += base[2]; }
    }
    if (blockIdx.x == gridDim.x - 1 && tid == 0) {
        if (a.zero_word != nullptr) *a.zero_word = 0;
        a.starts[a.S] = base[0] + a.scan_totals[blockIdx.x * 3 + 0];
        if (a.chunk_starts) a.chunk_starts[a.S] = base[1] + a.scan_totals[blockIdx.x * 3 + 1];
    }
}

__global__ void csc_place_kernel(CscArgs a) {
    const int k = a.k_dev ? min(*a.k_dev, a.k) : a.k;
    if (k <= 0) return;
    const long n = (long)a.n_rows * k;
    const int groups = a.words >> 3;
    for (long p = (long)blockIdx.x * blockDim.x + threadIdx.x; p < max(n, (long)a.S); p += (long)gridDim.x * blockDim.x) {
        if (p < a.S && a.chunk_starts) {
            const int c1 = a.chunk_starts[p + 1];
            for (int c = a.chunk_starts[p]; c < c1; ++c) a.work_latent[c] = (int)p;
        }
        if (p >= n) continue;
        const int b = (int)(p / k), j = (int)(p % k);
        const int32_t i = a.idx[(size_t)b * a.code_stride + j];
        if (i < 0 || i >= a.S) continue;
        const int g = b >> 8, wi = (b >> 5) & 7;
        const uint4* grp = reinterpret_cast<const uint4*>(a.bitmap + (size_t)i * a.words + 8 * g);
        const uint4 lo = grp[0], hi = grp[1];
        const uint32_t wd[8] = {lo.x, lo.y, lo.z, lo.w, hi.x, hi.y, hi.z, hi.w};
        int rank = a.grp_prefix[(size_t)i * groups + g];
#pragma unroll
        for (int e = 0; e < 8; ++e) {
            const uint32_t m = e < wi ? 0xffffffffu : (e == wi ? ((1u << (b & 31)) - 1u) : 0u);
            rank += __popc(wd[e] & m);
        }
        const int slot = a.starts[i] + rank;
        if (a.pairs != nullptr) a.pairs[slot] = int2{b, (int)((size_t)b * a.code_stride + j)};
        if (a.pv != nullptr) {
            const int fl = (rank == 0 ? DWS_FIRST : 0) | (rank == a.counts[i] - 1 ? DWS_LAST : 0);
            int pblk = 0;
            if (a.P > 1) while (pblk < a.P - 1 && i >= a.cuts[pblk]) ++pblk;
            a.pv[slot] = int2{((pblk * a.n_rows + b) << 7) | fl, __float_as_int(a.val[(size_t)b * a.code_stride + j])};
            a.plat[slot] = i;
            if (a.pv2 != nullptr) a.pv2[slot] = int2{(b << 7) | fl, __float_as_int(a.dval[(size_t)b * a.code_stride + j])};
        }
    }
}


template <int NV>
__device__ __forceinline__ void write_row_proj(float2* row_proj, int i, const f32x4 (&g)[NV], const f32x4 (&w)[NV], int project,
                                               int lane) {
    float sc;
    const float sq = rpg_row_stats<NV>(g, w, project, &sc);
    if (lane == 0) row_proj[i] = float2{sc, sq};
}

template <int NV>
__device__ __forceinline__ float row_sumsq(const f32x4 (&g)[NV]) {
    float sq = 0.f;
#pragma unroll
    for (int n = 0; n < NV; ++n)
#pragma unroll
        for (int e = 0; e < 4; ++e) sq = __builtin_fmaf(g[n][e], g[n][e], sq);
    return wave_sum(sq);
}

#ifndef DW_MIN_WAVES
#define DW_MIN_WAVES 1
#endif
#ifndef DW_GROUP
#define DW_GROUP 8
#endif
template <int NV>
__global__ __launch_bounds__(256, DW_MIN_WAVES) void dw_rows_kernel(DwRowsArgs a) {
    if (a.k_dev && *a.k_dev <= 0) return;
    const int lane = threadIdx.x & 63;
    const int wi = a.chunk_starts[a.lat_lo] + blockIdx.x * 4 + (threadIdx.x >> 6);
    const int n_work = a.chunk_starts[a.lat_hi];
    if (wi >= n_work) return;
    const int i = a.work_latent[wi];
    const int c = wi - a.chunk_starts[i];
    const int nch = a.chunk_starts[i + 1] - a.chunk_starts[i];
    const int D = a.D, D4 = D >> 2;
    const int seg_beg = a.starts[i], seg_end = a.starts[i + 1];
    int pblk = 0;
    if (a.P > 1) while (pblk < a.P - 1 && i >= a.cuts[pblk]) ++pblk;
    const size_t g_stride = (size_t)a.P * D;
    const float* gbase = a.g + (size_t)pblk * D;
    const int beg = seg_beg + c * DW_CHUNK;
    const int end = min(seg_end, beg + DW_CHUNK);
    f32x4 accd[NV], acce[NV], wv[NV];
    {
        const f32x4* wr = reinterpret_cast<const f32x4*>(a.W_dec + (size_t)i * D);
#pragma unroll
        for (int n = 0; n < NV; ++n) {
            accd[n] = f32x4{0.f, 0.f, 0.f, 0.f};
            acce[n] = f32x4{0.f, 0.f, 0.f, 0.f};
            wv[n] = (a.part != 2 && lane + 64 * n < D4) ? wr[lane + 64 * n] : f32x4{0.f, 0.f, 0.f, 0.f};
        }
    }
    int my_b = 0;
    float my_v = 0.f, my_dv = 0.f;
    const int cnt = end - beg;
    const int part = a.part;
    if (lane < cnt) {
        const int2 pr = a.pairs[beg + lane];
        my_b = pr.x;
        my_v = a.val[pr.y];
        if (part == 2) my_dv = a.dval[beg + lane];
        if (a.clear_bitmap != nullptr) a.clear_bitmap[(size_t)i * a.clear_words + (my_b >> 5)] = 0u;
    }
    float dbs = 0.f;
    constexpr int G = DW_GROUP, GS = (G == 8 ? 3 : 4);
    for (int j0 = 0; j0 < cnt; j0 += G) {
        float p[G];
        float r = 0.f;
        if (part != 2) {
#pragma unroll
        for (int t = 0; t < G; t += 2) {
            p[t] = 0.f; p[t + 1] = 0.f;
// ... 69 lines not shown
            f32x4* pe = reinterpret_cast<f32x4*>(oe) + q;
            if (part != 2) { if (direct && a.accumulate) *pd = *pd + accd[n]; else *pd = accd[n]; }
            if (part != 1) { if (direct && a.accumulate) *pe = *pe + acce[n]; else *pe = acce[n]; }
        }
    }
    if (lane == 0 && part != 1) {
        if (direct) a.db_enc[i] = a.accumulate ? (a.db_enc[i] + dbs) : dbs;
        else a.db_partials[a.part_starts[i] + c] = dbs;
    }
    if (a.row_proj != nullptr && direct && part != 2 && !a.accumulate) write_row_proj<NV>(a.row_proj, i, accd, wv, a.project, lane);
    if (a.enc_sq != nullptr && direct && part != 1 && !a.accumulate) {
        const float sq = row_sumsq<NV>(acce);
        if (lane == 0) a.enc_sq[i] = sq;
    }
}

template <int NV>
__global__ __launch_bounds__(256) void dw_combine_kernel(DwRowsArgs a) {
    if (a.k_dev && *a.k_dev <= 0) return;
    const int lane = threadIdx.x & 63;
    const int i = a.lat_lo + blockIdx.x * 4 + (threadIdx.x >> 6);
    if (i >= a.lat_hi) return;
    const int enc = blockIdx.y;
    if ((enc == 0 && a.part == 2) || (enc == 1 && a.part == 1)) return;
    const int nch = a.chunk_starts[i + 1] - a.chunk_starts[i];
    if (nch <= 1) return;
    const int c0 = a.part_starts[i], c1 = c0 + nch;
    const int D = a.D, D4 = D >> 2;
    const float* base = a.partials + (enc ? D : 0);
    f32x4 acc[NV];
#pragma unroll
    for (int n = 0; n < NV; ++n) acc[n] = f32x4{0.f, 0.f, 0.f, 0.f};
    float dbs = 0.f;
    int c = c0;
    constexpr int TRIP = NV <= 4 ? 8 : (NV <= 8 ? 4 : 2);
    for (; c + TRIP <= c1; c += TRIP) {
        f32x4 t[TRIP][NV];
#pragma unroll
        for (int u = 0; u < TRIP; ++u) {
            const f32x4* p = reinterpret_cast<const f32x4*>(base + (size_t)(c + u) * 2 * D);
#pragma unroll
            for (int n = 0; n < NV; ++n) t[u][n] = (lane + 64 * n < D4) ? p[lane + 64 * n] : f32x4{0.f, 0.f, 0.f, 0.f};
        }
#pragma unroll
        for (int n = 0; n < NV; ++n) {
            if constexpr (TRIP == 8) acc[n] += ((t[0][n] + t[1][n]) + (t[2][n] + t[3][n])) + ((t[4][n] + t[5][n]) + (t[6][n] + t[7][n]));
            else if constexpr (TRIP == 4) acc[n] += (t[0][n] + t[1][n]) + (t[2][n] + t[3][n]);
            else acc[n] += t[0][n] + t[1][n];
        }
        if (enc) {
#pragma unroll
            for (int u = 0; u < TRIP; ++u) dbs += a.db_partials[c + u];
        }
    }
    for (; c < c1; ++c) {
        const f32x4* p = reinterpret_cast<const f32x4*>(base + (size_t)c * 2 * D);
#pragma unroll
        for (int n = 0; n < NV; ++n)
            if (lane + 64 * n < D4) acc[n] += p[lane + 64 * n];
        if (enc) dbs += a.db_partials[c];
    }
    f32x4* o = reinterpret_cast<f32x4*>((enc ? a.dW_encT : a.dW_dec) + (size_t)i * D);
#pragma unroll
    for (int n = 0; n < NV; ++n) {
        const int q = lane + 64 * n;
        if (q < D4) o[q] = a.accumulate ? o[q] + acc[n] : acc[n];
    }
    if (enc) {
        if (lane == 0) a.db_enc[i] = a.accumulate ? (a.db_enc[i] + dbs) : dbs;
        if (a.enc_sq != nullptr && !a.accumulate) {
            const float sq = row_sumsq<NV>(acc);
            if (lane == 0) a.enc_sq[i] = sq;
        }
    } else if (a.row_proj != nullptr && !a.accumulate) {
        f32x4 wv[NV];
        const f32x4* wr = reinterpret_cast<const f32x4*>(a.W_dec + (size_t)i * D);
#pragma unroll
        for (int n = 0; n < NV; ++n) wv[n] = (lane + 64 * n < D4) ? wr[lane + 64 * n] : f32x4{0.f, 0.f, 0.f, 0.f};
        write_row_proj<NV>(a.row_proj, i, acc, wv, a.project, lane);
    }
}


typedef int i32x2 __attribute__((ext_vector_type(2)));
typedef int i32x4 __attribute__((ext_vector_type(4)));

__device__ __forceinline__ f32x4 buf_load16(__amdgpu_buffer_rsrc_t r, uint32_t voff) {
    const i32x4 v = __builtin_amdgcn_raw_buffer_load_b128(r, voff, 0, 0);
    return f32x4{__int_as_float(v[0]), __int_as_float(v[1]), __int_as_float(v[2]), __int_as_float(v[3])};
}
__device__ __forceinline__ float group8_sum(float v) {
    v += __int_as_float(__builtin_amdgcn_mov_dpp(__float_as_int(v), 0xB1, 0xF, 0xF, true));
    v += __int_as_float(__builtin_amdgcn_mov_dpp(__float_as_int(v), 0x4E, 0xF, 0xF, true));
    v += __int_as_float(__builtin_amdgcn_mov_dpp(__float_as_int(v), 0x141, 0xF, 0xF, true));
    return v;
}

__global__ __launch_bounds__(256) void slice_major_copy_kernel(const float* __restrict__ g, const float* __restrict__ x, int n, int D,
                                                               float* __restrict__ gS, float* __restrict__ xS) {
    const int lane = threadIdx.x & 63;
    const int row = blockIdx.x * 4 + (threadIdx.x >> 6);
    if (row >= n) return;
    const f32x4* gr = reinterpret_cast<const f32x4*>(g + (size_t)row * D);
    const f32x4* xr = reinterpret_cast<const f32x4*>(x + (size_t)row * D);
    for (int q = lane; q < (D >> 2); q += 64) {
        const size_t o = ((size_t)(q >> 3) * n + row) * 8 + (q & 7);
        reinterpret_cast<f32x4*>(gS)[o] = gr[q];
        reinterpret_cast<f32x4*>(xS)[o] = xr[q];
    }
}

template <bool DEC, bool DVAL = true>
__global__ __launch_bounds__(256, (DEC && DVAL) ? 4 : 5) void dw_slices_kernel(DwSlicesArgs a, int wg_per_slice) {
    constexpr bool PASS_A = DEC && DVAL;
    constexpr int L = DWS_RUN;
    const int lane = threadIdx.x & 63, gi = lane >> 3, li = lane & 7;
    const int xcd = blockIdx.x & 7, q = blockIdx.x >> 3;
    const int slice = xcd + 8 * (q / wg_per_slice);
    const bool sq_on = (DEC ? a.sq_wave_dec : a.sq_wave_enc) != nullptr;
    auto sq_slot = [&]() -> float* {
        return (DEC ? a.sq_wave_dec : a.sq_wave_enc) + ((size_t)blockIdx.x * 4 + __builtin_amdgcn_readfirstlane((int)(threadIdx.x >> 6)));
    };
    if (slice * DWS_SLICE >= a.D) { if (sq_on && lane == 0) *sq_slot() = 0.f; return; }
    const int NP = a.starts[a.S];
    const int run0 = ((q % wg_per_slice) * 4 + (threadIdx.x >> 6)) * 8;
    if (run0 * L >= NP) { if (sq_on && lane == 0) *sq_slot() = 0.f; return; }
    const int run = run0 + gi;
    const int col = slice * DWS_SLICE + li * 4;
    const uint32_t colb = (uint32_t)col * 4u, rowb = (uint32_t)a.D * 4u, li16 = (uint32_t)li * 16u;
    auto bound = [&](int r) -> int {
        const long nb = (long)r * L;
        if (nb >= NP) return NP;
        const int lat = a.plat[nb];
        const int s = a.starts[lat];
        return (a.starts[lat + 1] - s < L) ? s : (int)nb;
    };
    const int p0 = bound(run), p1 = bound(run + 1);
    const bool live = p0 < p1;
    const int2* const pv = DEC ? a.pv : a.pv2;
    float* const out = DEC ? a.dW_dec : a.dW_encT;
    float* const part = DEC ? a.part_dec : a.part_enc;
    f32x4 acc = {0.f, 0.f, 0.f, 0.f};
    f32x4 w4 = {0.f, 0.f, 0.f, 0.f};
    float* const dvp = PASS_A ? a.dvp + (size_t)slice * a.pair_cap : nullptr;
    __shared__ float sh_sq[256];
    sh_sq[threadIdx.x] = 0.f;
    const int sel = (lane & 56) << 2;
    const __amdgpu_buffer_rsrc_t mres = __builtin_amdgcn_make_buffer_rsrc(
        const_cast<float*>(DEC ? a.gS : a.xS) + (size_t)slice * a.n_rows * DWS_SLICE * (DEC && a.P > 1 ? a.P : 1), 0,
        (uint32_t)a.n_rows * 128u * (uint32_t)(DEC && a.P > 1 ? a.P : 1), 0x00020000);
    const __amdgpu_buffer_rsrc_t wres = __builtin_amdgcn_make_buffer_rsrc(const_cast<float*>(a.W_dec), 0, (uint32_t)a.S * rowb, 0x00020000);

    auto load_info = [&](int t, int2& e, int& lat) {
        const int p = p0 + 8 * t + li;
        e = int2{0, 0};
        lat = 0;
        if (p < p1) {
            const i32x2 v = reinterpret_cast<const i32x2*>(pv)[p];
            e = int2{v[0], v[1]};
            lat = a.plat[p];
            if (p == p1 - 1) e.x |= DWS_END;
            if (p == p0) e.x &= ~DWS_FIRST;
        }
    };
    constexpr int PB = 4;
    auto issue = [&](const int2& e, int lat, int j0, int (&xj)[PB], int (&lj)[PB], f32x4 (&gt)[PB], f32x4 (&wt)[PB]) {
#pragma unroll
        for (int j = 0; j < PB; ++j) {
            xj[j] = __builtin_amdgcn_ds_bpermute(sel + 4 * (j0 + j), e.x);
            lj[j] = __builtin_amdgcn_ds_bpermute(sel + 4 * (j0 + j), lat);
            gt[j] = buf_load16(mres, ((uint32_t)xj[j] & ~127u) | li16);
            if (PASS_A && (xj[j] & DWS_FIRST)) wt[j] = buf_load16(wres, (uint32_t)lj[j] * rowb + colb);
        }
    };
    auto consume = [&](const int2& e, int j0, const int (&xc)[PB], const int (&lc)[PB], const f32x4 (&gc)[PB], const f32x4 (&wc)[PB],
                       const f32x4& wnext0, bool& head_open, float& dmine) {
        float vc[PB];
#pragma unroll
        for (int j = 0; j < PB; ++j) vc[j] = __int_as_float(__builtin_amdgcn_ds_bpermute(sel + 4 * (j0 + j), e.y));
#pragma unroll
        for (int j = 0; j < PB; ++j) {
            if (PASS_A) {
                float d = gc[j][0] * w4[0] + gc[j][1] * w4[1] + gc[j][2] * w4[2] + gc[j][3] * w4[3];
                d = group8_sum(d);
                dmine = li == j0 + j ? d : dmine;
            }
            acc += vc[j] * gc[j];
            if (xc[j] & (DWS_LAST | DWS_END)) {
                float* o;
                if (head_open) o = part + ((size_t)run * 2 + 0) * a.D + col;
                else if (!(xc[j] & DWS_LAST)) o = part + ((size_t)run * 2 + 1) * a.D + col;
                else {
                    o = out + (size_t)lc[j] * a.D + col;
                    if (sq_on)
                        sh_sq[threadIdx.x] += __builtin_fmaf(acc[3], acc[3], __builtin_fmaf(acc[2], acc[2], __builtin_fmaf(acc[1], acc[1], acc[0] * acc[0])));
                }
                *reinterpret_cast<f32x4*>(o) = acc;
                if (DEC && slice == 0 && li == 0 && (xc[j] & DWS_END)) {
                    const int cl = (!head_open && !(xc[j] & DWS_LAST)) ? lc[j] : -1;
                    a.cut_lat[run] = cl;
                    if (cl >= 0 && a.cut_list != nullptr)
                        reinterpret_cast<i32x4*>(a.cut_list)[1 + atomicAdd(&a.cut_list[0], 1)] = i32x4{run, cl, a.starts[cl], a.starts[cl + 1]};
                }
                head_open = false;
                acc = f32x4{0.f, 0.f, 0.f, 0.f};
                if (PASS_A) w4 = j + 1 < PB ? wc[j + 1 < PB ? j + 1 : 0] : wnext0;
            }
        }
    };
    int2 e_c, e_n;
    int lat_c, lat_n;
    int xa[PB], xb[PB], la[PB], lb[PB];
    f32x4 ga[PB], gb[PB], wa[PB], wb[PB];
    bool head_open = false;
    load_info(0, e_c, lat_c);
    if (live) {
        head_open = (pv[p0].x & DWS_FIRST) == 0;
        if (PASS_A) w4 = buf_load16(wres, (uint32_t)a.plat[p0] * rowb + colb);
    }
    issue(e_c, lat_c, 0, xa, la, ga, wa);
    load_info(1, e_n, lat_n);
#pragma unroll 1
    for (int t = 0; __any(p0 + 8 * t < p1); ++t) {
        float dmine = 0.f;
        issue(e_c, lat_c, PB, xb, lb, gb, wb);
        consume(e_c, 0, xa, la, ga, wa, wb[0], head_open, dmine);
        issue(e_n, lat_n, 0, xa, la, ga, wa);
        consume(e_c, PB, xb, lb, gb, wb, wa[0], head_open, dmine);
        if (PASS_A && p0 + 8 * t + li < p1) dvp[p0 + 8 * t + li] = dmine;
        e_c = e_n; lat_c = lat_n;
        load_info(t + 2, e_n, lat_n);
    }
    if (sq_on) {
        const float sq = wave_sum(sh_sq[threadIdx.x]);
        if (lane == 0) *sq_slot() = sq;
    }
}

__global__ __launch_bounds__(256) void dw_dval_sum_kernel(DwSlicesArgs a) {
    const int NP = a.starts[a.S];
    const int p = blockIdx.x * 256 + threadIdx.x;
    if (p >= NP) return;
    const int n_slices = a.D / DWS_SLICE;
    float s = 0.f;
    for (int c = 0; c < n_slices; ++c) s += a.dvp[(size_t)c * a.pair_cap + p];
    const int2 e = a.pv[p];
    const int b = a.P > 1 ? (e.x >> 7) % a.n_rows : (e.x >> 7);
    a.pv2[p] = int2{(b << 7) | (e.x & 127), __float_as_int(s)};
    if (a.clear_bitmap != nullptr) a.clear_bitmap[(size_t)a.plat[p] * a.clear_words + (b >> 5)] = 0u;
}

__global__ __launch_bounds__(256) void dw_clear_bitmap_kernel(DwSlicesArgs a) {
    const int NP = a.starts[a.S];
    const int p = blockIdx.x * 256 + threadIdx.x;
    if (p >= NP) return;
    a.clear_bitmap[(size_t)a.plat[p] * a.clear_words + (a.pv2[p].x >> 12)] = 0u;
}

template <int NV>
__global__ __launch_bounds__(256) void dw_finalize_cut_kernel(DwSlicesArgs a, int kind0) {
    constexpr int L = DWS_RUN;
    __shared__ f32x4 sh[3][NV * 64];
    __shared__ float shdb[4];
    const int lane = threadIdx.x & 63, w = threadIdx.x >> 6;
    const int NP = a.starts[a.S];
    const int r0 = blockIdx.x;
    if ((long)(r0 + 1) * L >= NP) return;
    const int i = a.cut_lat[r0];
    if (i < 0) return;
    const int s = a.starts[i], e = a.starts[i + 1];
    const int r1 = (e - 1) / L;
    const int enc = blockIdx.y + kind0;
    const int D = a.D, D4 = D >> 2;
    const float* const part = enc ? a.part_enc : a.part_dec;
    const int nh = r1 - r0, ch = (nh + 3) / 4;
    const int ra = r0 + 1 + w * ch, rb = min(r1 + 1, ra + ch);
    f32x4 acc[NV];
#pragma unroll
    for (int n = 0; n < NV; ++n) acc[n] = f32x4{0.f, 0.f, 0.f, 0.f};
    int r = ra;
    constexpr int TRIP = NV <= 4 ? 4 : 2;
    for (; r + TRIP <= rb; r += TRIP) {
        f32x4 t[TRIP][NV];
#pragma unroll
        for (int u = 0; u < TRIP; ++u) {
            const f32x4* p = reinterpret_cast<const f32x4*>(part + (size_t)(r + u) * 2 * D);
#pragma unroll
            for (int n = 0; n < NV; ++n) t[u][n] = (lane + 64 * n < D4) ? p[lane + 64 * n] : f32x4{0.f, 0.f, 0.f, 0.f};
        }
#pragma unroll
        for (int n = 0; n < NV; ++n) {
            if constexpr (TRIP == 4) acc[n] += (t[0][n] + t[1][n]) + (t[2][n] + t[3][n]);
            else acc[n] += t[0][n] + t[1][n];
        }
    }
    for (; r < rb; ++r) {
        const f32x4* p = reinterpret_cast<const f32x4*>(part + (size_t)r * 2 * D);
#pragma unroll
        for (int n = 0; n < NV; ++n)
            if (lane + 64 * n < D4) acc[n] += p[lane + 64 * n];
// ... 5 lines not shown
        for (int p0 = s + w * q4 + lane; p0 < pend; p0 += 64 * 8) {
            float t[8];
#pragma unroll
            for (int u = 0; u < 8; ++u) t[u] = (p0 + 64 * u < pend) ? __int_as_float(a.pv2[p0 + 64 * u].y) : 0.f;
#pragma unroll
            for (int u = 0; u < 8; ++u)
                if (p0 + 64 * u < pend) dbs += t[u];
        }
        dbs = wave_sum(dbs);
    }
    if (w != 0) {
#pragma unroll
        for (int n = 0; n < NV; ++n) sh[w - 1][lane + 64 * n] = acc[n];
    }
    if (lane == 0) shdb[w] = dbs;
    __syncthreads();
    if (w != 0) return;
    {
        const f32x4* p = reinterpret_cast<const f32x4*>(part + ((size_t)r0 * 2 + 1) * D);
#pragma unroll
        for (int n = 0; n < NV; ++n) {
            const f32x4 t = (lane + 64 * n < D4) ? p[lane + 64 * n] : f32x4{0.f, 0.f, 0.f, 0.f};
            acc[n] = (((t + acc[n]) + sh[0][lane + 64 * n]) + sh[1][lane + 64 * n]) + sh[2][lane + 64 * n];
        }
    }
    float* const row = (enc ? a.dW_encT : a.dW_dec) + (size_t)i * D;
#pragma unroll
    for (int n = 0; n < NV; ++n)
        if (lane + 64 * n < D4) reinterpret_cast<f32x4*>(row)[lane + 64 * n] = acc[n];
    if (enc) {
        if (lane == 0) a.db_enc[i] = ((shdb[0] + shdb[1]) + shdb[2]) + shdb[3];
        if (a.enc_sq != nullptr) {
            const float sq = row_sumsq<NV>(acc);
            if (lane == 0) a.enc_sq[i] = sq;
        }
    } else if (a.row_proj != nullptr) {
        f32x4 wv[NV];
        const f32x4* wr = reinterpret_cast<const f32x4*>(a.W_dec + (size_t)i * D);
#pragma unroll
        for (int n = 0; n < NV; ++n) wv[n] = (lane + 64 * n < D4) ? wr[lane + 64 * n] : f32x4{0.f, 0.f, 0.f, 0.f};
        write_row_proj<NV>(a.row_proj, i, acc, wv, a.project, lane);
    }
}

template <int NV>
__global__ __launch_bounds__(256) void dw_finalize_kernel(DwSlicesArgs a, int kind0) {
    constexpr int L = DWS_RUN;
    const int lane = threadIdx.x & 63;
    const int i = blockIdx.x * 4 + (threadIdx.x >> 6);
    if (i >= a.S) return;
    const int enc = blockIdx.y + kind0;
    const int D = a.D, D4 = D >> 2;
    const int s = a.starts[i], e = a.starts[i + 1];
    if (!enc && a.lat_unused != nullptr && lane == 0) a.lat_unused[i] = e == s ? 1 : 0;
    if (e - s >= L && s / L != (e - 1) / L) return;
    float* const row = (enc ? a.dW_encT : a.dW_dec) + (size_t)i * D;
    f32x4 acc[NV], wv[NV];
    const bool proj = !enc && a.row_proj != nullptr;
    const f32x4* wr = reinterpret_cast<const f32x4*>(a.W_dec + (size_t)i * D);
#pragma unroll
    for (int n = 0; n < NV; ++n) {
        acc[n] = f32x4{0.f, 0.f, 0.f, 0.f};
        wv[n] = f32x4{0.f, 0.f, 0.f, 0.f};
        if (lane + 64 * n < D4) {
            if (e > s) acc[n] = reinterpret_cast<const f32x4*>(row)[lane + 64 * n];
            else if (!(enc && a.lat_unused != nullptr)) reinterpret_cast<f32x4*>(row)[lane + 64 * n] = acc[n];
            if (proj) wv[n] = wr[lane + 64 * n];
        }
    }
    if (enc) {
        float dbs = 0.f;
        for (int p = s + lane; p < e; p += 64) dbs += __int_as_float(a.pv2[p].y);
        dbs = wave_sum(dbs);
        if (lane == 0) a.db_enc[i] = dbs;
        if (a.enc_sq != nullptr) {
            const float sq = row_sumsq<NV>(acc);
            if (lane == 0) a.enc_sq[i] = sq;
        }
    } else if (proj) {
        write_row_proj<NV>(a.row_proj, i, acc, wv, a.project, lane);
    }
}

template <int NV>
__global__ __launch_bounds__(256) void dw_finalize_light_kernel(DwSlicesArgs a, int n_cut_blocks) {
    constexpr int L = DWS_RUN;
    __shared__ f32x4 sh[3][NV * 64];
    __shared__ float shdb[4];
    const int lane = threadIdx.x & 63, w = threadIdx.x >> 6;
    const int D = a.D, D4 = D >> 2;
    if ((int)blockIdx.x < n_cut_blocks) {
      const i32x4 first = reinterpret_cast<const i32x4*>(a.cut_list)[1 + (blockIdx.x >> 1)];
      const int n_items = 2 * a.cut_list[0];
      for (int item = blockIdx.x; item < n_items; item += n_cut_blocks) {
        const i32x4 ent = item == (int)blockIdx.x ? first : reinterpret_cast<const i32x4*>(a.cut_list)[1 + (item >> 1)];
        const int r0 = ent[0], i = ent[1], s = ent[2], e = ent[3], enc = item & 1;
        const int r1 = (e - 1) / L;
        const float* const part = enc ? a.part_enc : a.part_dec;
        f32x4 tp[NV], wv[NV];
        if (w == 0) {
            const f32x4* p = reinterpret_cast<const f32x4*>(part + ((size_t)r0 * 2 + 1) * D);
            const f32x4* wr = reinterpret_cast<const f32x4*>(a.W_dec + (size_t)i * D);
            const bool need_w = !enc && a.row_proj != nullptr;
#pragma unroll
            for (int n = 0; n < NV; ++n) {
                const bool ok = lane + 64 * n < D4;
                tp[n] = ok ? p[lane + 64 * n] : f32x4{0.f, 0.f, 0.f, 0.f};
                wv[n] = (ok && need_w) ? wr[lane + 64 * n] : f32x4{0.f, 0.f, 0.f, 0.f};
            }
        }
        const int nh = r1 - r0, ch = (nh + 3) / 4;
        const int ra = r0 + 1 + w * ch, rb = min(r1 + 1, ra + ch);
        f32x4 acc[NV];
#pragma unroll
        for (int n = 0; n < NV; ++n) acc[n] = f32x4{0.f, 0.f, 0.f, 0.f};
        constexpr int TRIP = NV <= 4 ? 4 : 2;
        int r = ra;
        for (; r + 2 * TRIP <= rb; r += 2 * TRIP) {
            f32x4 t[2 * TRIP][NV];
#pragma unroll
            for (int u = 0; u < 2 * TRIP; ++u) {
                const f32x4* p = reinterpret_cast<const f32x4*>(part + (size_t)(r + u) * 2 * D);
#pragma unroll
                for (int n = 0; n < NV; ++n) t[u][n] = (lane + 64 * n < D4) ? p[lane + 64 * n] : f32x4{0.f, 0.f, 0.f, 0.f};
            }
#pragma unroll
            for (int n = 0; n < NV; ++n) {
                if constexpr (TRIP == 4) {
                    acc[n] += (t[0][n] + t[1][n]) + (t[2][n] + t[3][n]);
                    acc[n] += (t[4][n] + t[5][n]) + (t[6][n] + t[7][n]);
                } else {
                    acc[n] += t[0][n] + t[1][n];
                    acc[n] += t[2][n] + t[3][n];
                }
            }
        }
        for (; r + TRIP <= rb; r += TRIP) {
            f32x4 t[TRIP][NV];
#pragma unroll
            for (int u = 0; u < TRIP; ++u) {
                const f32x4* p = reinterpret_cast<const f32x4*>(part + (size_t)(r + u) * 2 * D);
#pragma unroll
                for (int n = 0; n < NV; ++n) t[u][n] = (lane + 64 * n < D4) ? p[lane + 64 * n] : f32x4{0.f, 0.f, 0.f, 0.f};
            }
#pragma unroll
            for (int n = 0; n < NV; ++n) {
                if constexpr (TRIP == 4) acc[n] += (t[0][n] + t[1][n]) + (t[2][n] + t[3][n]);
                else acc[n] += t[0][n] + t[1][n];
            }
        }
        for (; r < rb; ++r) {
            const f32x4* p = reinterpret_cast<const f32x4*>(part + (size_t)r * 2 * D);
#pragma unroll
            for (int n = 0; n < NV; ++n)
                if (lane + 64 * n < D4) acc[n] += p[lane + 64 * n];
        }
        float dbs = 0.f;
        if (enc) {
            const int cnt = e - s, q4 = (cnt + 3) / 4;
            const int pend = min(e, s + (w + 1) * q4);
            for (int p0 = s + w * q4 + lane; p0 < pend; p0 += 64 * 8) {
                int2 pe[8];
#pragma unroll
                for (int u = 0; u < 8; ++u) pe[u] = (p0 + 64 * u < pend) ? a.pv2[p0 + 64 * u] : int2{0, 0};
#pragma unroll
                for (int u = 0; u < 8; ++u) {
                    if (p0 + 64 * u < pend) {
                        dbs += __int_as_float(pe[u].y);
                        if (a.clear_bitmap != nullptr) a.clear_bitmap[(size_t)i * a.clear_words + (pe[u].x >> 12)] = 0u;
                    }
                }
            }
            dbs = wave_sum(dbs);
        }
        if (w != 0) {
#pragma unroll
            for (int n = 0; n < NV; ++n) sh[w - 1][lane + 64 * n] = acc[n];
        }
        if (lane == 0) shdb[w] = dbs;
        __syncthreads();
        if (w == 0) {
#pragma unroll
            for (int n = 0; n < NV; ++n) acc[n] = (((tp[n] + acc[n]) + sh[0][lane + 64 * n]) + sh[1][lane + 64 * n]) + sh[2][lane + 64 * n];
            float* const row = (enc ? a.dW_encT : a.dW_dec) + (size_t)i * D;
#pragma unroll
            for (int n = 0; n < NV; ++n)
                if (lane + 64 * n < D4) reinterpret_cast<f32x4*>(row)[lane + 64 * n] = acc[n];
            if (enc) {
                if (lane == 0) a.db_enc[i] = ((shdb[0] + shdb[1]) + shdb[2]) + shdb[3];
                if (a.enc_sq != nullptr) {
                    const float sq = row_sumsq<NV>(acc);
                    if (lane == 0) a.enc_sq[i] = sq;
                }
            } else if (a.row_proj != nullptr) {
                write_row_proj<NV>(a.row_proj, i, acc, wv, a.project, lane);
            }
        }
        __syncthreads();
      }
      return;
    }
    const int li = lane & 7;
    const int i = ((int)blockIdx.x - n_cut_blocks) * 32 + (int)(threadIdx.x >> 3);
    if (i >= a.S) return;
    const int s = a.starts[i], e = a.starts[i + 1];
    if (a.lat_unused != nullptr && li == 0) a.lat_unused[i] = e == s ? 1 : 0;
    if (e - s >= L && s / L != (e - 1) / L) return;
    if (e == s) {
        if (a.lat_unused == nullptr) {
            for (int q = li; q < D4; q += 8) {
                reinterpret_cast<f32x4*>(a.dW_dec + (size_t)i * D)[q] = f32x4{0.f, 0.f, 0.f, 0.f};
                reinterpret_cast<f32x4*>(a.dW_encT + (size_t)i * D)[q] = f32x4{0.f, 0.f, 0.f, 0.f};
            }
        }
        if (li == 0) {
            a.db_enc[i] = 0.f;
            if (a.enc_sq != nullptr) a.enc_sq[i] = 0.f;
            if (a.row_proj != nullptr) a.row_proj[i] = float2{0.f, 0.f};
        }
        return;
    }
    auto group_tree = [&](float (&v)[8]) -> float {
        float r = ((v[0] + v[4]) + (v[2] + v[6])) + ((v[1] + v[5]) + (v[3] + v[7]));
        r += __shfl_xor(r, 4, 64);
        r += __shfl_xor(r, 2, 64);
        r += __shfl_xor(r, 1, 64);
        return r;
    };
    float gsq = 0.f, esq = 0.f;
    const bool waves_hold_squares = a.sq_wave_dec != nullptr;
    if (!waves_hold_squares) {
        const f32x4* gd = reinterpret_cast<const f32x4*>(a.dW_dec + (size_t)i * D);
        const f32x4* ge = reinterpret_cast<const f32x4*>(a.dW_encT + (size_t)i * D);
#pragma unroll 4
        for (int q = li; q < D4; q += 8) {
            const f32x4 u = gd[q], v = ge[q];
            gsq = __builtin_fmaf(u[3], u[3], __builtin_fmaf(u[2], u[2], __builtin_fmaf(u[1], u[1], __builtin_fmaf(u[0], u[0], gsq))));
            esq = __builtin_fmaf(v[3], v[3], __builtin_fmaf(v[2], v[2], __builtin_fmaf(v[1], v[1], __builtin_fmaf(v[0], v[0], esq))));
        }
        gsq += __shfl_xor(gsq, 4, 64); gsq += __shfl_xor(gsq, 2, 64); gsq += __shfl_xor(gsq, 1, 64);
        esq += __shfl_xor(esq, 4, 64); esq += __shfl_xor(esq, 2, 64); esq += __shfl_xor(esq, 1, 64);
    }
    float dv8[8], dt8[8];
#pragma unroll
    for (int j = 0; j < 8; ++j) {
        float dbs = 0.f, dot = 0.f;
#pragma unroll
        for (int t = 0; t < 2; ++t) {
            const int p = s + li + 8 * j + 64 * t;
            if (p < e) {
                const int2 pd = a.pv2[p];
                const float dv = __int_as_float(pd.y);
                dbs += dv;
                dot = __builtin_fmaf(__int_as_float(a.pv[p].y), dv, dot);
                if (a.clear_bitmap != nullptr) a.clear_bitmap[(size_t)i * a.clear_words + (pd.x >> 12)] = 0u;
            }
        }
        dv8[j] = dbs; dt8[j] = dot;
    }
    const float dbs = group_tree(dv8), dot = group_tree(dt8);
    if (li == 0) {
        a.db_enc[i] = dbs;
        if (a.enc_sq != nullptr) a.enc_sq[i] = esq;
        if (a.row_proj != nullptr) {
            const float nsq = a.wn2[i];
            const float sc = (a.project && nsq > 0.f) ? dot / nsq : 0.f;
            a.row_proj[i] = float2{sc, waves_hold_squares ? -sc * dot : fmaxf(__builtin_fmaf(-sc, dot, gsq), 0.f)};
        }
    }
}

__global__ __launch_bounds__(256) void transpose_kernel(const float* __restrict__ in, float* __restrict__ out, int S,
                                                        int D, double* __restrict__ sq_part) {
    __shared__ float tile[64][65];
    __shared__ double sh[4];
    const int s0 = blockIdx.x * 64, d0 = blockIdx.y * 64;
    const int c4 = (threadIdx.x & 15) * 4, r0 = threadIdx.x >> 4;
    float q0 = 0.f, q1 = 0.f, q2 = 0.f, q3 = 0.f;
#pragma unroll
    for (int r = r0; r < 64; r += 16) {
        const int s = s0 + r, d = d0 + c4;
        f32x4 v = f32x4{0.f, 0.f, 0.f, 0.f};
        if (s < S && d < D) v = *reinterpret_cast<const f32x4*>(in + (size_t)s * D + d);
        tile[r][c4] = v[0]; tile[r][c4 + 1] = v[1]; tile[r][c4 + 2] = v[2]; tile[r][c4 + 3] = v[3];
        q0 += v[0] * v[0]; q1 += v[1] * v[1]; q2 += v[2] * v[2]; q3 += v[3] * v[3];
    }
    if (sq_part != nullptr) {
        const double q = wave_sum_d((double)q0 + (double)q1 + (double)q2 + (double)q3);
        if ((threadIdx.x & 63) == 0) sh[threadIdx.x >> 6] = q;
    }
    __syncthreads();
    if (sq_part != nullptr && threadIdx.x == 0) sq_part[(size_t)blockIdx.y * gridDim.x + blockIdx.x] = sh[0] + sh[1] + sh[2] + sh[3];
#pragma unroll
    for (int r = r0; r < 64; r += 16) {
        const int d = d0 + r, s = s0 + c4;
        if (d < D && s < S)
            *reinterpret_cast<f32x4*>(out + (size_t)d * S + s) = f32x4{tile[c4][r], tile[c4 + 1][r], tile[c4 + 2][r], tile[c4 + 3][r]};
    }
}


template <bool ABSMAX>
__global__ __launch_bounds__(256) void colsum_partial_kernel(const float* m, int n_rows, int D, float* partials,
                                                             const int32_t* k_dev, long row_stride, float* wg_absmax,
                                                             int col_mult) {
    if (k_dev && *k_dev <= 0) return;
    const int Dfull = D;
    if (k_dev && col_mult > 0) D = min(D, (*k_dev * col_mult + 3) & ~3);
    float amax = 0.f;
    const int r0 = blockIdx.x * 64;
    const int r1 = min(n_rows, r0 + 64);
    for (int q = threadIdx.x; q < (D >> 2); q += 256) {
        f32x4 s = {0.f, 0.f, 0.f, 0.f};
        int r = r0;
        for (; r + 8 <= r1; r += 8) {
            f32x4 v[8];
#pragma unroll
            for (int u = 0; u < 8; ++u) v[u] = reinterpret_cast<const f32x4*>(m + (size_t)(r + u) * row_stride)[q];
            s += ((v[0] + v[1]) + (v[2] + v[3])) + ((v[4] + v[5]) + (v[6] + v[7]));
            if constexpr (ABSMAX) {
#pragma unroll
                for (int u = 0; u < 8; ++u)
                    amax = fmaxf(fmaxf(fmaxf(amax, fabsf(v[u][0])), fabsf(v[u][1])), fmaxf(fabsf(v[u][2]), fabsf(v[u][3])));
            }
        }
        for (; r < r1; ++r) {
            const f32x4 v = reinterpret_cast<const f32x4*>(m + (size_t)r * row_stride)[q];
            s += v;
            if constexpr (ABSMAX) amax = fmaxf(fmaxf(fmaxf(amax, fabsf(v[0])), fabsf(v[1])), fmaxf(fabsf(v[2]), fabsf(v[3])));
        }
        reinterpret_cast<f32x4*>(partials + (size_t)blockIdx.x * Dfull)[q] = s;
    }
    if constexpr (ABSMAX) {
        __shared__ float sh[4];
        for (int o = 32; o > 0; o >>= 1) amax = fmaxf(amax, __shfl_xor(amax, o, 64));
        if ((threadIdx.x & 63) == 0) sh[threadIdx.x >> 6] = amax;
        __syncthreads();
// ... 370 lines not shown
    hipLaunchKernelGGL(decode_s_finish_kernel, dim3((d.n_rows + 3) / 4), dim3(256), 0, stream, a);
    return hipGetLastError();
}
hipError_t launch_decode_matry(const DecodeArgs& a, const MatryArgs& m, hipStream_t stream) {
    if (a.n_rows <= 0) return hipSuccess;
    if (a.dval_out != nullptr && a.x != nullptr && a.training && decode_matry_forms_dval(a.D, a.k)) {
        const size_t smem = (size_t)m.P * a.D * sizeof(float);
        static bool attr_set = false;
        if (!attr_set) {
            const void* fns[4] = {reinterpret_cast<const void*>(&decode_matry_q_kernel<1>), reinterpret_cast<const void*>(&decode_matry_q_kernel<2>),
                                  reinterpret_cast<const void*>(&decode_matry_q_kernel<3>), reinterpret_cast<const void*>(&decode_matry_q_kernel<4>)};
            for (const void* f : fns) {
                hipError_t e = hipFuncSetAttribute(f, hipFuncAttributeMaxDynamicSharedMemorySize, MAX_PREFIXES * 1024 * (int)sizeof(float));
                if (e != hipSuccess) return e;
            }
            attr_set = true;
        }
        switch (a.D / 256) {
            case 1: hipLaunchKernelGGL(decode_matry_q_kernel<1>, dim3(a.n_rows), dim3(64), smem, stream, a, m); break;
            case 2: hipLaunchKernelGGL(decode_matry_q_kernel<2>, dim3(a.n_rows), dim3(128), smem, stream, a, m); break;
            case 3: hipLaunchKernelGGL(decode_matry_q_kernel<3>, dim3(a.n_rows), dim3(192), smem, stream, a, m); break;
            default: hipLaunchKernelGGL(decode_matry_q_kernel<4>, dim3(a.n_rows), dim3(256), smem, stream, a, m); break;
        }
        return hipGetLastError();
    }
    return dispatch_nv(a.D, [&](auto nv) {
        hipLaunchKernelGGL(decode_matry_kernel<decltype(nv)::value>, dim3((a.n_rows + 3) / 4), dim3(256), 0, stream, a, m);
    });
}
hipError_t launch_csc_build(const CscArgs& a, hipStream_t stream, bool bitmap_clean, const float* colsum_m, int colsum_D,
                            long colsum_row_stride, float* colsum_partials, float* colsum_out, bool prefilled) {
    if (a.n_rows <= 0) return hipSuccess;
    const long n = (long)a.n_rows * a.k;
    const int blocks = prefilled ? 0 : (int)std::min<long>((n + 255) / 256, 4096);
    const int place_blocks = (int)std::min<long>((std::max<long>(n, a.S) + 255) / 256, 8192);
    if (!bitmap_clean && !prefilled) hipLaunchKernelGGL(csc_clear_kernel, dim3(2048), dim3(256), 0, stream, a);
    const int n_scan = (a.S + 1023) / 1024;
    ColsumPlain c{colsum_m, a.n_rows, colsum_D, colsum_partials, colsum_row_stride > 0 ? colsum_row_stride : (long)colsum_D,
                  colsum_out, (a.n_rows + 63) / 64};
    int colsum_in_scan = 0;
    if (colsum_m != nullptr && prefilled && a.epoch != 0) {
        hipLaunchKernelGGL(csc_count_colpart_kernel, dim3((a.S + 3) / 4 + c.n_blocks), dim3(256), 0, stream, a, (a.S + 3) / 4, c);
        colsum_in_scan = 1;
    } else if (colsum_m != nullptr) {
        hipLaunchKernelGGL(csc_fill_colsum_kernel, dim3(blocks + c.n_blocks), dim3(256), 0, stream, a, blocks, c);
        hipLaunchKernelGGL(csc_count_colsum_kernel, dim3((a.S + 3) / 4 + (colsum_D + 63) / 64), dim3(256), 0, stream, a, (a.S + 3) / 4, c);
    } else {
        if (blocks > 0) hipLaunchKernelGGL(csc_fill_kernel, dim3(blocks), dim3(256), 0, stream, a);
        hipLaunchKernelGGL(csc_count_kernel, dim3((a.S + 3) / 4), dim3(256), 0, stream, a);
    }
    if (a.epoch != 0 && n_scan <= 128) {
        hipLaunchKernelGGL(csc_scan_fused_kernel, dim3(n_scan + (colsum_in_scan ? (colsum_D + 63) / 64 : 0)), dim3(1024), 0, stream, a, n_scan, c,
                           colsum_in_scan);
    } else {
        hipLaunchKernelGGL(csc_scan_block_kernel, dim3(n_scan), dim3(1024), 0, stream, a);
        hipLaunchKernelGGL(csc_scan_offset_kernel, dim3(n_scan), dim3(1024), 0, stream, a);
    }
    hipLaunchKernelGGL(csc_place_kernel, dim3(place_blocks), dim3(256), 0, stream, a);
    return hipGetLastError();
}
hipError_t launch_dw_rows(const DwRowsArgs& a, int max_work, hipStream_t stream) {
    return dispatch_nv(a.D, [&](auto nv) {
        hipLaunchKernelGGL(dw_rows_kernel<decltype(nv)::value>, dim3((max_work + 3) / 4), dim3(256), 0, stream, a);
        hipLaunchKernelGGL(dw_combine_kernel<decltype(nv)::value>, dim3((a.lat_hi - a.lat_lo + 3) / 4, 2), dim3(256), 0, stream, a);
    });
}
hipError_t launch_slice_major_copy(const float* g, const float* x, int n, int D, float* gS, float* xS, hipStream_t stream) {
    if (n <= 0) return hipSuccess;
    hipLaunchKernelGGL(slice_major_copy_kernel, dim3((n + 3) / 4), dim3(256), 0, stream, g, x, n, D, gS, xS);
    return hipGetLastError();
}
int dw_slices_waves(int D, int max_pairs) {
    const int n_runs = (max_pairs + DWS_RUN - 1) / DWS_RUN;
    return ((D / DWS_SLICE + 7) / 8) * 8 * ((n_runs + 31) / 32) * 4;
}
hipError_t launch_dw_slices(const DwSlicesArgs& a_in, int max_pairs, int part, hipStream_t stream) {
    DwSlicesArgs a = a_in;
    if (a.D % DWS_SLICE != 0 || max_pairs <= 0) return hipErrorInvalidValue;
    const int n_runs = (max_pairs + DWS_RUN - 1) / DWS_RUN;
    const int wg_per_slice = (n_runs + 31) / 32;
    const int grid = ((a.D / DWS_SLICE + 7) / 8) * 8 * wg_per_slice;
    const bool light = part == 0 && a.have_dval && a.wn2 != nullptr;
    if (!light) { a.sq_wave_dec = nullptr; a.sq_wave_enc = nullptr; }
    if (part != 2 && a.have_dval) {
        hipLaunchKernelGGL((dw_slices_kernel<true, false>), dim3(grid), dim3(256), 0, stream, a, wg_per_slice);
        if (a.clear_bitmap != nullptr && !light) hipLaunchKernelGGL(dw_clear_bitmap_kernel, dim3((max_pairs + 255) / 256), dim3(256), 0, stream, a);
    } else if (part != 2) {
        hipLaunchKernelGGL(dw_slices_kernel<true>, dim3(grid), dim3(256), 0, stream, a, wg_per_slice);
        hipLaunchKernelGGL(dw_dval_sum_kernel, dim3((max_pairs + 255) / 256), dim3(256), 0, stream, a);
    }
    if (part != 1) hipLaunchKernelGGL(dw_slices_kernel<false>, dim3(grid), dim3(256), 0, stream, a, wg_per_slice);
    const int kinds = part == 0 ? 2 : 1, kind0 = part == 2 ? 1 : 0;
    if (light) {
        const int n_cut = a.cut_list != nullptr ? std::min(2 * (n_runs - 1), 8192) : 0;
        if (a.cut_list == nullptr && n_runs > 1) return hipErrorInvalidValue;
        return dispatch_nv(a.D, [&](auto nv) {
            hipLaunchKernelGGL(dw_finalize_light_kernel<decltype(nv)::value>, dim3(n_cut + (a.S + 31) / 32), dim3(256), 0, stream, a, n_cut);
        });
    }
    return dispatch_nv(a.D, [&](auto nv) {
        if (n_runs > 1) hipLaunchKernelGGL(dw_finalize_cut_kernel<decltype(nv)::value>, dim3(n_runs - 1, kinds), dim3(256), 0, stream, a, kind0);
        hipLaunchKernelGGL(dw_finalize_kernel<decltype(nv)::value>, dim3((a.S + 3) / 4, kinds), dim3(256), 0, stream, a, kind0);
    });
}
hipError_t launch_transpose(const float* in, float* out, int S, int D, hipStream_t stream, double* sq_part) {
    hipLaunchKernelGGL(transpose_kernel, dim3((S + 63) / 64, (D + 63) / 64), dim3(256), 0, stream, in, out, S, D, sq_part);
    return hipGetLastError();
}
int transpose_blocks(int S, int D) { return ((S + 63) / 64) * ((D + 63) / 64); }
hipError_t launch_colsum(const float* m, int n_rows, int D, float* partials, float* out, int accumulate,
                         const int32_t* k_dev, hipStream_t stream, long row_stride, float out_scale, int col_mult) {
    const int nb = (n_rows + 63) / 64;
    if (nb <= 0) return hipSuccess;
    hipLaunchKernelGGL(colsum_partial_kernel<false>, dim3(nb), dim3(256), 0, stream, m, n_rows, D, partials, k_dev,
                       row_stride > 0 ? row_stride : (long)D, (float*)nullptr, col_mult);
    hipLaunchKernelGGL(colsum_final_kernel, dim3((D + 63) / 64), dim3(256), 0, stream, partials, nb, D, out,
                       accumulate, k_dev, out_scale, col_mult, (const float*)nullptr, (float*)nullptr, (saev_step_stats*)nullptr,
                       (int32_t*)nullptr);
    return hipGetLastError();
}
hipError_t launch_colsum_absmax(const float* m, int n_rows, int D, float* partials, float* out, float* wg_scratch,
                                float* absmax_out, hipStream_t stream, float out_scale, saev_step_stats* zero_stats,
                                int32_t* zero_flag) {
    const int nb = (n_rows + 63) / 64;
    if (nb <= 0) return hipSuccess;
    hipLaunchKernelGGL(colsum_partial_kernel<true>, dim3(nb), dim3(256), 0, stream, m, n_rows, D, partials,
                       (const int32_t*)nullptr, (long)D, wg_scratch, 0);
    hipLaunchKernelGGL(colsum_final_kernel, dim3((D + 63) / 64), dim3(256), 0, stream, partials, nb, D, out, 0,
                       (const int32_t*)nullptr, out_scale, 0, (const float*)wg_scratch, absmax_out, zero_stats, zero_flag);
    return hipGetLastError();
}
```

### saev_amd/csrc/split.hip

```cpp
#include "common.h"
#include "kernels.h"

namespace {

typedef _Float16 half8 __attribute__((ext_vector_type(8)));

typedef __bf16 bf16x8 __attribute__((ext_vector_type(8)));

__device__ __forceinline__ half8 split8(const float (&v)[8], int part) {
    half8 o;
#pragma unroll
    for (int e = 0; e < 8; ++e) {
        const _Float16 h = (_Float16)v[e];
        o[e] = part == 0 ? h : (_Float16)(v[e] - (float)h);
    }
    return o;
}

__device__ __forceinline__ half8 round8_bf16(const float (&v)[8]) {
    bf16x8 o;
#pragma unroll
    for (int e = 0; e < 8; ++e) o[e] = (__bf16)v[e];
    return __builtin_bit_cast(half8, o);
}
// ... 99 lines not shown
                o[0] = f32x4{v[0] * inv, v[1] * inv, v[2] * inv, v[3] * inv};
                if (k + 4 < D) o[1] = f32x4{v[4] * inv, v[5] * inv, v[6] * inv, v[7] * inv};
            }
        }
    }
}

template <int MODE>
__global__ __launch_bounds__(1024) void split_wT_kernel(const float* __restrict__ W, int D, int S, int nks, float scale,
                                                        const float* __restrict__ scale_dev, _Float16* __restrict__ ws,
                                                        const float* __restrict__ mu, double* __restrict__ dot_part,
                                                        float* __restrict__ sq_part, float* __restrict__ W_T, int wt_slices) {
    constexpr int KS = MODE != 0 ? 32 : 16;
    __shared__ float tile[KS][257];
    __shared__ float mu_s[KS];
    split_wT_body<MODE>(blockIdx.x, gridDim.x, tile, mu_s, W, D, S, nks, scale, scale_dev, ws, mu, dot_part, sq_part, W_T, wt_slices);
}
__global__ __launch_bounds__(1024) void split_both_kernel(const float* __restrict__ M, int R, int C, float scale,
                                                          const float* __restrict__ scale_dev, _Float16* __restrict__ rf, int nks_r,
                                                          _Float16* __restrict__ tf, int nks_t) {
    __shared__ float tile[256][64];
    if (scale_dev != nullptr) scale *= *scale_dev;
    const int ctiles = (C + 63) / 64;
    const int rb = blockIdx.x / ctiles, ct = blockIdx.x % ctiles;
    const int r0 = rb * 256, c0 = ct * 64;
    for (int q = threadIdx.x; q < 256 * 16; q += 1024) {
        const int rl = q >> 4, cl = (q & 15) * 4;
        const int r = r0 + rl, c = c0 + cl;
        f32x4 v = f32x4{0.f, 0.f, 0.f, 0.f};
        if (r < R && c < C) v = *reinterpret_cast<const f32x4*>(M + (size_t)r * C + c) * scale;
        const int sw = rl & 31;
        tile[rl][cl ^ sw] = v[0]; tile[rl][(cl + 1) ^ sw] = v[1]; tile[rl][(cl + 2) ^ sw] = v[2]; tile[rl][(cl + 3) ^ sw] = v[3];
    }
    __syncthreads();
    const int i = threadIdx.x;
    if (rf != nullptr) {
        const int rl = i >> 2, p = i & 3;
        const int c = p ^ ((4 - ((rl >> 2) & 3)) & 3);
        const int part = c >> 1, h = c & 1;
#pragma unroll
        for (int j = 0; j < 4; ++j) {
            const int ks = c0 / 16 + j;
            if (ks >= nks_r) break;
            float v[8];
#pragma unroll
            for (int e = 0; e < 8; ++e) v[e] = tile[rl][(16 * j + 8 * h + e) ^ (rl & 31)];
            reinterpret_cast<half8*>(rf + ((size_t)rb * nks_r + ks) * 256 * 32)[i] = split8(v, part);
        }
    }
    if (tf != nullptr) {
        const int cb = c0 / 256, crow0 = c0 % 256;
#pragma unroll
        for (int qq = 0; qq < 4; ++qq) {
            const int idx = i + 1024 * qq;
            const int j = idx >> 8, within = idx & 255;
            const int cl = within >> 2, p = within & 3;
            const int rl_t = crow0 + cl;
            const int c = p ^ ((4 - ((rl_t >> 2) & 3)) & 3);
            const int part = c >> 1, h = c & 1;
            const int ks = r0 / 16 + j;
            if (ks >= nks_t) continue;
            float v[8];
#pragma unroll
            for (int e = 0; e < 8; ++e) v[e] = tile[16 * j + 8 * h + e][cl ^ ((16 * j + 8 * h + e) & 31)];
            reinterpret_cast<half8*>(tf + ((size_t)cb * nks_t + ks) * 256 * 32)[rl_t * 4 + p] = split8(v, part);
        }
    }
}

struct SplitF16rArgs {
    const float* x; int n, D, nks; const float* scales; const float* mu; _Float16* xs;
    const float* W; int S; _Float16* ws; double* dot_part; float* sq_part; float* W_T;
    int n_x;
    float* xS; int wt_slices;
};
__global__ __launch_bounds__(1024) void split_f16r_kernel(SplitF16rArgs a) {
    __shared__ float tile[32][257];
    __shared__ float mu_s[32];
    if ((int)blockIdx.x < a.n_x) split_rows_body<2>(blockIdx.x, a.x, a.n, a.D, a.nks, 1.0f, a.scales, a.mu, a.xs, a.xS);
    else split_wT_body<2>(blockIdx.x - a.n_x, gridDim.x - a.n_x, tile, mu_s, a.W, a.D, a.S, a.nks, 1.0f, a.scales + 1, a.ws, a.mu, a.dot_part,
                          a.sq_part, a.W_T, a.wt_slices);
}

__device__ __forceinline__ float xprep_round_f16_sig(float v) {
    const uint32_t b = __float_as_uint(v);
    return __uint_as_float((b + 0x0FFFu + ((b >> 13) & 1u)) & 0xFFFFE000u);
}
__global__ __launch_bounds__(1024) void xprep_kernel(XprepArgs a) {
    __shared__ float cs[256][33];
    __shared__ float cs2[32][33];
    __shared__ float shm[2][16];
    const int nks = a.nks;
    const int bid = blockIdx.x, blk = bid / nks, ks = bid % nks;
    const int i = threadIdx.x, lane = i & 63, w = i >> 6;
    const int rl = i >> 2, p = i & 3;
    const int c = p ^ ((4 - ((rl >> 2) & 3)) & 3);
    const int r = blk * 256 + rl, k = ks * 32 + c * 8;
    const float scale = a.scales[0];
    const float up = a.scales[4];
    const float back = (up > 0.f && up < 3.0e38f) ? up : 1.0f, inv = 1.0f / back;
    float v[8] = {0.f, 0.f, 0.f, 0.f, 0.f, 0.f, 0.f, 0.f};
    float raw[8] = {0.f, 0.f, 0.f, 0.f, 0.f, 0.f, 0.f, 0.f};
    float am = 0.f, cm = 0.f, s2 = 0.f, d2 = 0.f;
    if (r < a.n) {
        const size_t src = a.rows != nullptr ? (size_t)a.rows[r] : (size_t)r;
        const f32x4 x0 = *reinterpret_cast<const f32x4*>(a.x + src * a.D + k);
        const f32x4 x1 = *reinterpret_cast<const f32x4*>(a.x + src * a.D + k + 4);
        if (a.x_out != nullptr) {
            f32x4* o = reinterpret_cast<f32x4*>(a.x_out + (size_t)r * a.D + k);
            o[0] = x0; o[1] = x1;
        }
        f32x4* o = reinterpret_cast<f32x4*>(a.xS + ((size_t)ks * a.n + r) * 32 + c * 8);
        o[0] = x0; o[1] = x1;
        const f32x4 m0 = *reinterpret_cast<const f32x4*>(a.mu + k), m1 = *reinterpret_cast<const f32x4*>(a.mu + k + 4);
#pragma unroll
        for (int e = 0; e < 8; ++e) {
            raw[e] = e < 4 ? x0[e] : x1[e - 4];
            const float ce = raw[e] - (e < 4 ? m0[e] : m1[e - 4]);
            am = fmaxf(am, fabsf(raw[e]));
            cm = fmaxf(cm, fabsf(ce));
            const float d = (ce - xprep_round_f16_sig(ce)) * inv, q = ce * inv;
            s2 = __builtin_fmaf(q, q, s2);
            d2 = __builtin_fmaf(d, d, d2);
            v[e] = ce * scale;
        }
        if (!(s2 < 3.0e38f)) { cm = __builtin_inff(); }
    }
    reinterpret_cast<half8*>(a.xs + (size_t)bid * 256 * 32)[i] = pack8<2>(v, 0);
    s2 += __shfl_xor(s2, 1, 64); s2 += __shfl_xor(s2, 2, 64);
    d2 += __shfl_xor(d2, 1, 64); d2 += __shfl_xor(d2, 2, 64);
    if (p == 0 && r < a.n) reinterpret_cast<float2*>(a.xn_part)[(size_t)ks * a.n_pad + r] = float2{s2, d2};
#pragma unroll
    for (int e = 0; e < 8; ++e) cs[rl][c * 8 + e] = raw[e];
    am = wave_max(am); cm = wave_max(cm);
    if (lane == 0) { shm[0][w] = am; shm[1][w] = cm; }
    __syncthreads();
    {
        const int col = i & 31, seg = i >> 5;
        float t = 0.f;
#pragma unroll
        for (int j = 0; j < 8; ++j) t += cs[seg * 8 + j][col];
        cs2[seg][col] = t;
    }
    __syncthreads();
    if (i < 32) {
        float t = 0.f;
#pragma unroll
        for (int j = 0; j < 32; ++j) t += cs2[j][i];
        a.col_part[(size_t)blk * a.D + ks * 32 + i] = t;
    }
    if (i == 32) {
        float m0 = 0.f, m1 = 0.f;
        for (int j = 0; j < 16; ++j) { m0 = fmaxf(m0, shm[0][j]); m1 = fmaxf(m1, shm[1][j]); }
        a.amax_part[bid] = m0;
        a.cmax_part[bid] = m1;
    }
    if (a.mu_keep != nullptr && bid == 0 && i >= 192) {
        for (int d = i - 192; d < a.D; d += 1024 - 192) a.mu_keep[d] = a.mu[d];
        if (i == 192) { a.xside_keep[0] = scale; a.xside_keep[1] = 0.f; }
    }
    if (a.stale != nullptr && i >= 64 && i < 66) {
        uint32_t h = ((uint32_t)bid * 3u + (uint32_t)(i - 64)) * 2654435761u + a.salt * 40503u;
        h ^= h >> 15; h *= 2246822519u; h ^= h >> 13;
        const uint32_t d = h % (uint32_t)a.D, sidx = (h >> 8) % (uint32_t)a.S;
        const float w = a.W_enc[(size_t)d * a.S + sidx], c = a.WeS[((size_t)(d >> 5) * a.S + sidx) * 32 + (d & 31)];
        if (__float_as_uint(w) != __float_as_uint(c)) atomicOr(a.stale, 1);
    }
    if (a.stale != nullptr && i >= 128 && i < 192) {
        bool differs = false;
        for (int sidx = bid * 64 + (i - 128); sidx < a.S; sidx += (int)gridDim.x * 64)
            differs |= __float_as_uint(a.b_enc[sidx]) != __float_as_uint(a.b_seen[sidx]);
        if (differs) atomicOr(a.stale, 1);
    }
}

__global__ __launch_bounds__(256) void bias_finish_kernel(const double* __restrict__ dot_part,
                                                          const float* __restrict__ sq_part, int nks, int S, int S_pad,
                                                          const float* __restrict__ w_scale, const float* __restrict__ b_enc,
                                                          float* __restrict__ b_shift, float* __restrict__ wg_max,
                                                          float* __restrict__ b_seen) {
    __shared__ float sh[3][4];
    const int sidx = blockIdx.x * 256 + threadIdx.x;
    float out = 0.f, nrm = 0.f, dnrm = 0.f;
    if (sidx < S) {
        double acc = 0.0, sq = 0.0, dsq = 0.0;
        for (int ks = 0; ks < nks; ++ks) {
            acc += dot_part[(size_t)ks * S_pad + sidx];
            sq += (double)sq_part[(size_t)ks * S_pad + sidx];
            dsq += (double)sq_part[(size_t)(nks + ks) * S_pad + sidx];
        }
        const double sc = (double)(*w_scale);
        const float be = b_enc[sidx];
        out = (float)(acc / sc + (double)be);
        b_shift[sidx] = out;
        if (b_seen != nullptr) b_seen[sidx] = be;
        nrm = (float)(sqrt(sq) / sc) * 1.000001f;
        dnrm = (float)(sqrt(dsq) / sc) * 1.00001f;
    }
    float m = fabsf(out);
    for (int o = 32; o > 0; o >>= 1) { m = fmaxf(m, __shfl_xor(m, o, 64)); nrm = fmaxf(nrm, __shfl_xor(nrm, o, 64)); dnrm = fmaxf(dnrm, __shfl_xor(dnrm, o, 64)); }
    if ((threadIdx.x & 63) == 0) { sh[0][threadIdx.x >> 6] = m; sh[1][threadIdx.x >> 6] = nrm; sh[2][threadIdx.x >> 6] = dnrm; }
    __syncthreads();
    if (threadIdx.x < 3) {
        const float* q = sh[threadIdx.x];
        wg_max[threadIdx.x * gridDim.x + blockIdx.x] = fmaxf(fmaxf(q[0], q[1]), fmaxf(q[2], q[3]));
    }
}


}

hipError_t launch_split_rows(const float* x, int n, int D, int Dp, void* xs, int mode, hipStream_t stream, float scale,
                             const float* scale_dev, const float* mu, float* xS) {
    const int nks = Dp / (mode != 0 ? 32 : 16), nblk = (n + 255) / 256;
    if (nblk <= 0) return hipSuccess;
    _Float16* o = reinterpret_cast<_Float16*>(xs);
    if (mode == 1) hipLaunchKernelGGL(split_rows_kernel<1>, dim3(nblk * nks), dim3(1024), 0, stream, x, n, D, nks, scale, scale_dev, mu, o, nullptr);
    else if (mode == 2) hipLaunchKernelGGL(split_rows_kernel<2>, dim3(nblk * nks), dim3(1024), 0, stream, x, n, D, nks, scale, scale_dev, mu, o, xS);
    else hipLaunchKernelGGL(split_rows_kernel<0>, dim3(nblk * nks), dim3(1024), 0, stream, x, n, D, nks, scale, scale_dev, mu, o, nullptr);
    return hipGetLastError();
}

hipError_t launch_split_wT(const float* W, int D, int S, int S_pad, int Dp, float scale, void* ws, int mode,
                           hipStream_t stream, const float* scale_dev, const float* mu, double* dot_part, float* sq_part,
                           float* W_T, int wt_slices) {
    const int nks = Dp / (mode != 0 ? 32 : 16);
    const dim3 grid((S_pad / 256) * nks);
    _Float16* o = reinterpret_cast<_Float16*>(ws);
    if (mode == 1) hipLaunchKernelGGL(split_wT_kernel<1>, grid, dim3(1024), 0, stream, W, D, S, nks, scale, scale_dev, o, nullptr, nullptr, nullptr, nullptr, 0);
    else if (mode == 2) hipLaunchKernelGGL(split_wT_kernel<2>, grid, dim3(1024), 0, stream, W, D, S, nks, scale, scale_dev, o, mu, dot_part, sq_part, W_T, wt_slices);
    else hipLaunchKernelGGL(split_wT_kernel<0>, grid, dim3(1024), 0, stream, W, D, S, nks, scale, scale_dev, o, nullptr, nullptr, nullptr, nullptr, 0);
    return hipGetLastError();
}

hipError_t launch_split_both(const float* M, int R, int C, float scale, const float* scale_dev, void* rf, int kp_r, void* tf, int kp_t,
                             hipStream_t stream) {
    if (R <= 0 || C <= 0) return hipSuccess;
    const int grid = ((R + 255) / 256) * ((C + 63) / 64);
    hipLaunchKernelGGL(split_both_kernel, dim3(grid), dim3(1024), 0, stream, M, R, C, scale, scale_dev, reinterpret_cast<_Float16*>(rf), kp_r / 16,
                       reinterpret_cast<_Float16*>(tf), kp_t / 16);
    return hipGetLastError();
}

hipError_t launch_split_f16r(const float* x, int n, int D, int Dp, void* xs, const float* scales, const float* mu, const float* W,
                             int S, int S_pad, void* ws, double* dot_part, float* sq_part, float* W_T, hipStream_t stream, float* xS,
                             int wt_slices) {
    SplitF16rArgs a{};
    a.xS = xS; a.wt_slices = wt_slices;
    a.x = x; a.n = n; a.D = D; a.nks = Dp / 32; a.scales = scales; a.mu = mu; a.xs = reinterpret_cast<_Float16*>(xs);
    a.W = W; a.S = S; a.ws = reinterpret_cast<_Float16*>(ws); a.dot_part = dot_part; a.sq_part = sq_part; a.W_T = W_T;
    a.n_x = ((n + 255) / 256) * a.nks;
    hipLaunchKernelGGL(split_f16r_kernel, dim3(a.n_x + (S_pad / 256) * a.nks), dim3(1024), 0, stream, a);
    return hipGetLastError();
}

hipError_t launch_bias_finish(const double* dot_part, const float* sq_part, int Dp, int S, int S_pad, const float* w_scale,
                              const float* b_enc, float* b_shift, float* wg_part, hipStream_t stream, float* b_seen) {
    const int nwg = (S + 255) / 256;
    hipLaunchKernelGGL(bias_finish_kernel, dim3(nwg), dim3(256), 0, stream, dot_part, sq_part, Dp / 32, S, S_pad, w_scale,
                       b_enc, b_shift, wg_part, b_seen);
    return hipGetLastError();
}

hipError_t launch_xprep(const XprepArgs& a, hipStream_t stream) {
    const int nblk = (a.n + 255) / 256;
    if (nblk <= 0 || a.D % 32 != 0) return hipErrorInvalidValue;
    hipLaunchKernelGGL(xprep_kernel, dim3(nblk * a.nks), dim3(1024), 0, stream, a);
    return hipGetLastError();
}
```

### saev_amd/csrc/tail.hip

```cpp
#include "common.h"
#include "kernels.h"

namespace {

template <int NV>
__global__ __launch_bounds__(256) void normalize_rows_kernel(float* W, int S, int D, float* WS, float* wn2) {
    const int lane = threadIdx.x & 63;
    const int i = blockIdx.x * 4 + (threadIdx.x >> 6);
    if (i >= S) return;
    const int D4 = D >> 2;
    f32x4* r = reinterpret_cast<f32x4*>(W + (size_t)i * D);
    f32x4 v[NV];
    float ss = 0.f;
#pragma unroll
    for (int n = 0; n < NV; ++n) {
        const int q = lane + 64 * n;
        v[n] = (q < D4) ? r[q] : f32x4{0.f, 0.f, 0.f, 0.f};
        ss += v[n][0] * v[n][0] + v[n][1] * v[n][1] + v[n][2] * v[n][2] + v[n][3] * v[n][3];
    }
    ss = wave_sum(ss);
    const float nrm = sqrtf(ss);
    float s2 = 0.f;
#pragma unroll
    for (int n = 0; n < NV; ++n) {
// ... 300 lines not shown
#pragma unroll
                for (int e = 0; e < 8; ++e) h[e] = (__bf16)tile[c * 8 + e][rl];
                imgb[rl * 4 + (c ^ swz)] = __builtin_bit_cast(half8t, h);
            }
            return;
        }
        __shared__ float mu_s[TD];
        if (threadIdx.x < TD) mu_s[threadIdx.x] = f.img.mu[d0 + threadIdx.x];
        __syncthreads();
        const float wm = *f.img.wmax_prev;
        const float scale = (wm > 0.f && wm < 3.0e38f) ? exp2f(13.0f - floorf(log2f(wm))) : 1.0f;
        if (t == 0 && threadIdx.x == 0) { f.img.scales_next[1] = scale; f.img.scales_next[3] = 1.0f; }
        double accp[4];
        float sqp[4], dsp[4];
        half8t* const img = reinterpret_cast<half8t*>(f.img.ws + ((size_t)(s0 / TS) * f.img.nks + ks) * 256 * 32);
        f32x4* const wes = reinterpret_cast<f32x4*>(f.img.WeS + ((size_t)ks * S + s0 + rl) * 32);
#pragma unroll
        for (int c = 0; c < 4; ++c) {
            float v[8];
            half8t h;
            double acc = 0.0;
            float sq = 0.f, dsq = 0.f;
#pragma unroll
            for (int e = 0; e < 8; ++e) {
                v[e] = tile[c * 8 + e][rl] * scale;
                h[e] = (_Float16)v[e];
                acc += (double)mu_s[c * 8 + e] * (double)v[e];
                sq += v[e] * v[e];
                const float d = v[e] - (float)h[e];
                dsq += d * d;
            }
            img[rl * 4 + (c ^ swz)] = h;
            if (s0 + rl < S) {
                const float inv = 1.0f / scale;
                wes[2 * c] = f32x4{v[0] * inv, v[1] * inv, v[2] * inv, v[3] * inv};
                wes[2 * c + 1] = f32x4{v[4] * inv, v[5] * inv, v[6] * inv, v[7] * inv};
            }
            accp[c] = acc; sqp[c] = sq; dsp[c] = dsq;
        }
        {
            const int c0 = swz, c1 = 1 ^ swz, c2 = 2 ^ swz, c3 = 3 ^ swz;
            const size_t o = (size_t)ks * f.img.S_pad + s0 + rl;
            f.img.dot_part[o] = (accp[c0] + accp[c1]) + (accp[c2] + accp[c3]);
            f.img.sq_part[o] = (sqp[c0] + sqp[c1]) + (sqp[c2] + sqp[c3]);
            f.img.sq_part[(size_t)f.img.nks * f.img.S_pad + o] = (dsp[c0] + dsp[c1]) + (dsp[c2] + dsp[c3]);
        }
        return;
    }
}

template <int NV, int PART>
__global__ __launch_bounds__(256, (PART == 2 ? 3 : 4)) void adam_fused_kernel(AdamFusedArgs f) {
    const AdamArgs& a = f.a;
    float norm;
    const float coef = clip_coef(a, &norm);
    if (blockIdx.x == 0 && threadIdx.x == 0 && a.stats) a.stats->grad_norm = norm;
    const float gs = a.grad_scale * coef;
    const float step_size = a.lr / a.bc1;
    const int S = f.S, D = f.D;
    if constexpr (PART == 1) {
        adam_wenc_tile(f, a, gs, step_size, (int)blockIdx.x);
        return;
    }
    if constexpr (PART == 2) {
        if ((int)blockIdx.x >= f.nb_rows && (int)blockIdx.x < f.nb_rows + f.nb_tiles) {
            adam_wenc_tile(f, a, gs, step_size, (int)blockIdx.x - f.nb_rows);
            return;
        }
    }
    if ((int)blockIdx.x < f.nb_rows) {
        const int lane = threadIdx.x & 63;
        const int i = blockIdx.x * 4 + (threadIdx.x >> 6);
        if (i >= S) return;
        adam_row<NV>(a, i, D, f.row_proj[i].x, gs, step_size, lane, f.lat_unused != nullptr && f.lat_unused[i] != 0);
        return;
    }
    const long nb = gridDim.x - f.nb_rows - (PART == 2 ? f.nb_tiles : 0);
    const long bi = blockIdx.x - f.nb_rows - (PART == 2 ? f.nb_tiles : 0);
    for (int seg = 0; seg < 2; ++seg) {
        const long off = seg ? f.off_b_enc : f.off_b_dec, n = seg ? f.n_b_enc : f.n_b_dec;
        for (long i = bi * 256 + threadIdx.x; i < n; i += nb * 256) {
            const AdamElem r = adam_elem(a.p[off + i], scaled_grad(a.g[off + i], gs), a.m[off + i], a.v[off + i], a, step_size);
            a.p[off + i] = r.p; a.m[off + i] = r.m; a.v[off + i] = r.v;
        }
    }
}

__global__ __launch_bounds__(256) void adam_kernel(AdamArgs a) {
    const float norm = a.grad_scale * (float)sqrt(*a.sumsq);
    float coef = 1.f;
    if (a.max_norm >= 0.f) coef = fminf(a.max_norm / (norm + 1e-6f), 1.f);
    if (blockIdx.x == 0 && threadIdx.x == 0 && a.stats) a.stats->grad_norm = norm;
    const float gs = a.grad_scale * coef;
    const float step_size = a.lr / a.bc1;
    const long n4 = a.n >> 2;
    constexpr int UNR = 4;
    for (long q0 = (long)blockIdx.x * 256 * UNR + threadIdx.x; q0 < n4; q0 += (long)gridDim.x * 256 * UNR) {
        f32x4 p[UNR], g[UNR], m[UNR], v[UNR];
#pragma unroll
        for (int u = 0; u < UNR; ++u) {
            const long q = q0 + u * 256;
            if (q < n4) {
                p[u] = __builtin_nontemporal_load(reinterpret_cast<f32x4*>(a.p) + q);
                g[u] = __builtin_nontemporal_load(reinterpret_cast<const f32x4*>(a.g) + q);
                m[u] = __builtin_nontemporal_load(reinterpret_cast<f32x4*>(a.m) + q);
                v[u] = __builtin_nontemporal_load(reinterpret_cast<f32x4*>(a.v) + q);
            }
        }
#pragma unroll
        for (int u = 0; u < UNR; ++u) {
            const long q = q0 + u * 256;
            if (q >= n4) continue;
#pragma unroll
            for (int e = 0; e < 4; ++e) {
                const float ge = scaled_grad(g[u][e], gs);
                const AdamElem r = adam_elem(p[u][e], ge, m[u][e], v[u][e], a, step_size);
                p[u][e] = r.p; m[u][e] = r.m; v[u][e] = r.v;
            }
            __builtin_nontemporal_store(p[u], reinterpret_cast<f32x4*>(a.p) + q);
            __builtin_nontemporal_store(m[u], reinterpret_cast<f32x4*>(a.m) + q);
            __builtin_nontemporal_store(v[u], reinterpret_cast<f32x4*>(a.v) + q);
        }
    }
    if (blockIdx.x == 0) {
        for (long i = (n4 << 2) + threadIdx.x; i < a.n; i += 256) {
            const AdamElem r = adam_elem(a.p[i], scaled_grad(a.g[i], gs), a.m[i], a.v[i], a, step_size);
            a.p[i] = r.p; a.m[i] = r.m; a.v[i] = r.v;
        }
    }
}

__device__ __forceinline__ void dead_compact_block(const int32_t* dead, int S, int32_t* list, int (&wave_tot)[16]) {
    const int tid = threadIdx.x, lane = tid & 63, w = tid >> 6;
    const int per = (S + 1023) / 1024;
    const int i0 = tid * per, i1 = min(S, i0 + per);
    int cnt = 0;
    for (int i = i0; i < i1; ++i) cnt += dead[i] ? 1 : 0;
    int incl = cnt;
#pragma unroll
    for (int o = 1; o < 64; o <<= 1) {
        const int n = __shfl_up(incl, o, 64);
        if (lane >= o) incl += n;
    }
    if (lane == 63) wave_tot[w] = incl;
    __syncthreads();
    int pos = incl - cnt;
    for (int j = 0; j < w; ++j) pos += wave_tot[j];
    if (cnt > 0)
        for (int i = i0; i < i1; ++i)
            if (dead[i]) list[pos++] = i;
}

__device__ __forceinline__ void dead_update_body(const DeadArgs& a, int bid, int n_blocks) {
    __shared__ int sh[2][16];
    __shared__ int wave_tot[16];
    __shared__ int last_n;
    const int i = bid * blockDim.x + threadIdx.x;
    const int nw = blockDim.x >> 6;
    int d = 0, near = 0;
    if (i < a.S) {
        int64_t t = a.toks[i] + a.add_tokens;
        if (a.fired[i]) t = 0;
        a.fired[i] = 0;
        a.toks[i] = t;
        d = (t >= a.threshold) ? 1 : 0;
        near = (t >= a.threshold - a.horizon_tokens) ? 1 : 0;
// ... 276 lines not shown
```

Before: 6.220 million.

## Defer bias finish into xprep, pack pair records, grid-stride dense select

Moves the encoder bias-finish launch that followed the fused Adam step into the next step's xprep kernel as extra workgroups. Adam now writes b_seen directly so the separate pass is unnecessary. Packs the per-pair backward data (flags, latent, value, dval) into one 16-byte record read by the dW slice and finalize kernels, replacing separate pv/pv2/plat loads. Caps the dense top-k select grid at 2048 workgroups that loop over rows. The goal is fewer launches and fewer scattered loads, at the cost of more deferred-state bookkeeping and a 16-byte record in place of split arrays.

```diff
diff --git a/saev_amd/csrc/ctx.hip b/saev_amd/csrc/ctx.hip
--- a/saev_amd/csrc/ctx.hip
+++ b/saev_amd/csrc/ctx.hip
@@ -97,6 +97,8 @@
     float* rs_part = nullptr;
     float* xS_c = nullptr;
     int2 *pv = nullptr, *pv2 = nullptr;
+    int4* pair_rec = nullptr;
+    bool rec_pairs = false;
     int32_t *plat = nullptr, *cut_lat = nullptr, *cut_list = nullptr;
     int32_t* lat_unused = nullptr;
     bool fused_step = false;
@@ -151,6 +153,7 @@
     float *WeS = nullptr;
     float *xn_part = nullptr, *amax_part = nullptr, *cmax_part = nullptr;
     float* b_seen = nullptr;
+    bool bias_pending = false;
     int32_t *stale_host = nullptr, *stale_dev = nullptr;
     uint32_t* wchk = nullptr;
     float *mu_keep = nullptr, *xside_keep = nullptr;
@@ -373,7 +376,9 @@
         if (c->dval_rows != nullptr && c->dbg.dw_route == 4 && decode_slices_supported((int)D, (int)S, (int)K, (int)K) && c->cfg.normalize_w_dec) {
             A(WdS, S * D); A(dec_part, (size_t)(D / 32) * MB * 3);
         }
-        A(pv, MBB * K); A(pv2, MBB * K); A(plat, MBB * K); A(cut_lat, (MBB * K + DWS_RUN - 1) / DWS_RUN); A(cut_list, 4 * (1 + (MBB * K + DWS_RUN - 1) / DWS_RUN)); A(lat_unused, S);
+        A(pair_rec, MBB * K);
+        if (rc == SAEV_OK) { c->pv = reinterpret_cast<int2*>(c->pair_rec); c->pv2 = c->pv + MBB * K; }
+        A(plat, MBB * K); A(cut_lat, (MBB * K + DWS_RUN - 1) / DWS_RUN); A(cut_list, 4 * (1 + (MBB * K + DWS_RUN - 1) / DWS_RUN)); A(lat_unused, S);
         if (c->dval_rows != nullptr && c->dbg.fin_route == 0) { A(wn2, S); A(sq_wave, (size_t)2 * dw_slices_waves((int)D, (int)(MBB * K))); }
     }
     A(colsum_partials, ((MBB + 63) / 64) * D);
@@ -732,6 +737,7 @@
         c->wimg_mu_serial = c->mu_serial;
         HIPCHK(c, launch_bias_finish(reinterpret_cast<const double*>(c->dot_part), c->sq_part, c->Dp, S, c->S_pad,
                                      scl(c) + 1, c->params + c->off_b_enc, c->b_shift, c->wnorm_scratch, s, c->b_seen));
+        c->bias_pending = false;
         if (!defer_margins)
             HIPCHK(c, launch_row_margins(c->xnorm_c, n, D, c->wnorm_scratch, (S + 255) / 256, scl(c), pre_flag,
                                          c->wmax_prev, c->row_margin, s));
@@ -834,6 +840,13 @@
     const bool predict_mode = fused_supported(c->cfg) && c->cfg.bound_mode != 0 && c->cfg.encoder_mode != SAEV_ENCODER_F32 &&
                               f16_ngroups(c) == 32;
     const bool one_launch_pre = fused_supported(c->cfg) && !predict_mode;
+    const bool xprep_route = c->stream_step && fused_supported(c->cfg) && !(c->cfg.bound_mode != 0 && f16_ngroups(c) == 32 &&
+                                                                            c->cfg.encoder_mode != SAEV_ENCODER_F32);
+    if (c->bias_pending && !xprep_route) {
+        HIPCHK(c, launch_bias_finish(reinterpret_cast<const double*>(c->dot_part), c->sq_part, c->Dp, c->cfg.d_sae, c->S_pad,
+                                     scl(c) + 1, c->params + c->off_b_enc, c->b_shift, c->wnorm_scratch, s, c->b_seen));
+        c->bias_pending = false;
+    }
     if (c->follow_stream) {
         HIPCHK(c, launch_follower_scales(c->leader->xside_keep, c->wmax_prev, scl(c), const_cast<int32_t*>(pre_flag), 1, s));
     } else if (!c->stream_step) {
@@ -916,6 +929,12 @@
                 xp.W_enc = c->params + c->off_W_enc; xp.WeS = c->WeS; xp.b_enc = c->params + c->off_b_enc; xp.b_seen = c->b_seen;
                 xp.S = S_; xp.salt = ++c->stale_salt; xp.stale = c->flags + 12;
                 if (!c->followers.empty()) { xp.mu_keep = c->mu_keep; xp.xside_keep = c->xside_keep; }
+                if (c->bias_pending) {
+                    xp.n_bias = (S_ + 1023) / 1024; xp.bias_nks = c->Dp / 32; xp.S_pad = c->S_pad;
+                    xp.dot_part = reinterpret_cast<const double*>(c->dot_part); xp.sq_part = c->sq_part; xp.w_scale = scl(c) + 1;
+                    xp.b_shift = c->b_shift; xp.wg_max = c->wnorm_scratch;
+                    c->bias_pending = false;
+                }
                 HIPCHK(c, launch_xprep(xp, s));
                 PreEncode2Args pe{};
                 pe.cand_cnt = c->cand_cnt; pe.n_rows = n; pe.gmax = c->gmax; pe.n_gmax = ng * c->gmax_stride;
@@ -1612,6 +1631,8 @@
         if (!ov && c->dval_fwd) { a.pv2 = c->pv2; a.dval = c->dval_rows; }
     }
     c->dval_pairs_ready = c->dws_pairs && a.pv2 != nullptr;
+    c->rec_pairs = c->fused_step && c->dval_pairs_ready && !ov && c->P_last == 1 && c->wn2_fresh && c->dbg.fin_route == 0;
+    if (c->rec_pairs) a.rec = c->pair_rec;
     if (c->fused_step && c->dws_pairs) { a.pairs = nullptr; a.chunk_starts = nullptr; a.part_starts = nullptr; a.work_latent = nullptr; }
     const float* gmat = ov ? c->ov_g : (c->P_last > 1 ? c->G : c->g);
     const bool prefilled = !ov && c->bitmap_prefill_words == words && c->bitmap_prefill_rows == n;
@@ -1640,6 +1661,8 @@
     const bool ov = c->ov_x != nullptr;
     const int n = ov ? c->ov_n : c->n_last;
     REQUIRE(c, 0 <= lat_lo && lat_lo < lat_hi && lat_hi <= S, SAEV_INVALID_ARG, "saev_backward_rows: bad latent range");
+    REQUIRE(c, !c->rec_pairs || (part == 0 && lat_lo == 0 && lat_hi == S), SAEV_INVALID_ARG,
+            "saev_backward_rows: saev_train_step's pair records serve one pass over all latents");
     hipStream_t s = (hipStream_t)stream;
     DwRowsArgs a{};
     a.starts = c->starts; a.chunk_starts = c->chunk_starts; a.work_latent = c->work_latent;
@@ -1676,6 +1699,7 @@
         c->sq_wave_n = 0;
         if (c->dval_pairs_ready && c->wn2_fresh && part == 0) {
             w.wn2 = c->wn2;
+            if (c->rec_pairs) w.rec = c->pair_rec;
             if (c->fused_step && all_rows && c->sq_wave != nullptr && c->dbg.fin_route != 2) {
                 c->sq_wave_n = dw_slices_waves(D, (int)((long)n * K));
                 w.sq_wave_dec = c->sq_wave; w.sq_wave_enc = c->sq_wave + c->sq_wave_n;
@@ -1910,6 +1934,8 @@
             im.verify = (chk_was_valid && c->fwd_reused_wimg && im.late != nullptr) ? 1 : 0;
             im.early = (emit && c->leader == nullptr) ? c->flags + 13 : nullptr;
         }
+        const bool defer_bias = emit && c->leader == nullptr;
+        if (defer_bias) im.b_seen = c->b_seen;
         HIPCHK(c, launch_adam_fused(a, c->row_proj, c->dW_encT, (int)S, (int)D, S * D, c->off_W_enc - S * D, c->off_W_enc,
                                     c->off_b_enc, c->n_params - c->off_b_enc, s, c->unused_valid ? c->lat_unused : nullptr,
                                     (emit || emit_bf16) ? &im : nullptr));
@@ -1917,8 +1943,11 @@
         c->wchk_valid = (emit || emit_bf16) && c->wchk != nullptr && c->dbg.own_check == 0;
         c->wimg_bf16_fresh = emit_bf16;
         if (emit) {
-            HIPCHK(c, launch_bias_finish(reinterpret_cast<const double*>(c->dot_part), c->sq_part, c->Dp, (int)S, c->S_pad, scl_next(c) + 1,
-                                         c->params + c->off_b_enc, c->b_shift, c->wnorm_scratch, s, c->b_seen));
+            if (defer_bias)
+                c->bias_pending = true;
+            else
+                HIPCHK(c, launch_bias_finish(reinterpret_cast<const double*>(c->dot_part), c->sq_part, c->Dp, (int)S, c->S_pad, scl_next(c) + 1,
+                                             c->params + c->off_b_enc, c->b_shift, c->wnorm_scratch, s, c->b_seen));
             c->scale_par ^= 1;
             c->wimg_fresh = true;
             c->wimg_mu_serial = c->leader != nullptr ? c->leader->mu_serial : c->mu_serial;
diff --git a/saev_amd/csrc/kernels.h b/saev_amd/csrc/kernels.h
--- a/saev_amd/csrc/kernels.h
+++ b/saev_amd/csrc/kernels.h
@@ -183,6 +183,7 @@
     const float* val;
     int2* pv2;
     const float* dval;
+    int4* rec;
     int P;
     int32_t cuts[16];
     int32_t* zero_word;
@@ -232,6 +233,7 @@
     const int2* pv;
     int2* pv2;
     const int32_t* plat;
+    const int4* rec;
     const float* gS;
     const float* xS;
     const float* W_dec;
@@ -299,6 +301,7 @@
     int mode;
     uint32_t* chk; int32_t* late; int verify;
     const int32_t* early;
+    float* b_seen;
 };
 hipError_t launch_adam_fused(const AdamArgs& a, const float2* row_proj, const float* gT, int S, int D, long off_b_dec, long n_b_dec,
                              long off_W_enc, long off_b_enc, long n_b_enc, hipStream_t stream, const int32_t* lat_unused = nullptr,
@@ -401,6 +404,9 @@
     float* cmax_part;
     const float* W_enc; const float* WeS; const float* b_enc; const float* b_seen;
     int S; uint32_t salt; int32_t* stale;
+    int n_bias, bias_nks, S_pad;
+    const double* dot_part; const float* sq_part; const float* w_scale;
+    float* b_shift; float* wg_max;
     float* mu_keep; float* xside_keep;
 };
 hipError_t launch_xprep(const XprepArgs& a, hipStream_t stream);
diff --git a/saev_amd/csrc/select.hip b/saev_amd/csrc/select.hip
--- a/saev_amd/csrc/select.hip
+++ b/saev_amd/csrc/select.hip
@@ -4,6 +4,7 @@
 namespace {
 
 constexpr int SD_THREADS = 256;
+constexpr int SD_MAX_WGS = 2048;
 
 __device__ __forceinline__ int block_excl_scan_256(int v, int* lds_wave_tot, int& total) {
     const int lane = threadIdx.x & 63, w = threadIdx.x >> 6;
@@ -27,13 +28,11 @@
     return base + incl - v;
 }
 
-__global__ __launch_bounds__(SD_THREADS) void select_dense_kernel(SelectDenseArgs a) {
-    if (a.enable_flag != nullptr && (*a.enable_flag != 0) != (a.enable_when != 0)) return;
+__device__ __forceinline__ void select_dense_row(const SelectDenseArgs& a, const int row) {
     __shared__ int hist[256];
     __shared__ int sh_digit, sh_need;
     __shared__ int wave_tot[4];
 
-    const int row = blockIdx.x;
     const int S = a.S;
     int k = a.k_dev ? min(*a.k_dev, a.k) : a.k;
     if (a.k_dev && k <= 0) return;
@@ -133,6 +132,13 @@
         }
         base_gt += tot & 0xFFFF;
         base_eq += tot >> 16;
+    }
+}
+__global__ __launch_bounds__(SD_THREADS) void select_dense_kernel(SelectDenseArgs a) {
+    if (a.enable_flag != nullptr && (*a.enable_flag != 0) != (a.enable_when != 0)) return;
+    for (int row = blockIdx.x; row < a.n_rows; row += gridDim.x) {
+        if (row != (int)blockIdx.x) __syncthreads();
+        select_dense_row(a, row);
     }
 }
 
@@ -1034,7 +1040,7 @@
 
 hipError_t launch_select_dense(const SelectDenseArgs& a, hipStream_t stream) {
     if (a.n_rows <= 0) return hipSuccess;
-    hipLaunchKernelGGL(select_dense_kernel, dim3(a.n_rows), dim3(SD_THREADS), 0, stream, a);
+    hipLaunchKernelGGL(select_dense_kernel, dim3(std::min(a.n_rows, SD_MAX_WGS)), dim3(SD_THREADS), 0, stream, a);
     return hipGetLastError();
 }
 
diff --git a/saev_amd/csrc/sparse.hip b/saev_amd/csrc/sparse.hip
--- a/saev_amd/csrc/sparse.hip
+++ b/saev_amd/csrc/sparse.hip
@@ -606,6 +606,9 @@
     }
 }
 
+typedef int i32x2 __attribute__((ext_vector_type(2)));
+typedef int i32x4 __attribute__((ext_vector_type(4)));
+
 __global__ void csc_place_kernel(CscArgs a) {
     const int k = a.k_dev ? min(*a.k_dev, a.k) : a.k;
     if (k <= 0) return;
@@ -632,7 +635,11 @@
         }
         const int slot = a.starts[i] + rank;
         if (a.pairs != nullptr) a.pairs[slot] = int2{b, (int)((size_t)b * a.code_stride + j)};
-        if (a.pv != nullptr) {
+        if (a.rec != nullptr) {
+            const int fl = (rank == 0 ? DWS_FIRST : 0) | (rank == a.counts[i] - 1 ? DWS_LAST : 0);
+            const size_t c = (size_t)b * a.code_stride + j;
+            reinterpret_cast<i32x4*>(a.rec)[slot] = i32x4{(b << 7) | fl, i, __float_as_int(a.val[c]), __float_as_int(a.dval[c])};
+        } else if (a.pv != nullptr) {
             const int fl = (rank == 0 ? DWS_FIRST : 0) | (rank == a.counts[i] - 1 ? DWS_LAST : 0);
             int pblk = 0;
             if (a.P > 1) while (pblk < a.P - 1 && i >= a.cuts[pblk]) ++pblk;
@@ -868,8 +875,6 @@
 }
 
 
-typedef int i32x2 __attribute__((ext_vector_type(2)));
-typedef int i32x4 __attribute__((ext_vector_type(4)));
 
 __device__ __forceinline__ f32x4 buf_load16(__amdgpu_buffer_rsrc_t r, uint32_t voff) {
     const i32x4 v = __builtin_amdgcn_raw_buffer_load_b128(r, voff, 0, 0);
@@ -896,9 +901,11 @@
     }
 }
 
-template <bool DEC, bool DVAL = true>
+template <bool DEC, bool DVAL = true, bool REC = false>
 __global__ __launch_bounds__(256, (DEC && DVAL) ? 4 : 5) void dw_slices_kernel(DwSlicesArgs a, int wg_per_slice) {
     constexpr bool PASS_A = DEC && DVAL;
+    static_assert(!(REC && PASS_A), "the records carry dval: pass A does not form its shares");
+    const i32x4* const rec = reinterpret_cast<const i32x4*>(a.rec);
     constexpr int L = DWS_RUN;
     const int lane = threadIdx.x & 63, gi = lane >> 3, li = lane & 7;
     const int xcd = blockIdx.x & 7, q = blockIdx.x >> 3;
@@ -917,7 +924,7 @@
     auto bound = [&](int r) -> int {
         const long nb = (long)r * L;
         if (nb >= NP) return NP;
-        const int lat = a.plat[nb];
+        const int lat = REC ? rec[nb][1] : a.plat[nb];
         const int s = a.starts[lat];
         return (a.starts[lat + 1] - s < L) ? s : (int)nb;
     };
@@ -942,9 +949,15 @@
         e = int2{0, 0};
         lat = 0;
         if (p < p1) {
-            const i32x2 v = reinterpret_cast<const i32x2*>(pv)[p];
-            e = int2{v[0], v[1]};
-            lat = a.plat[p];
+            if constexpr (REC) {
+                const i32x4 v = rec[p];
+                e = int2{v[0], DEC ? v[2] : v[3]};
+                lat = v[1];
+            } else {
+                const i32x2 v = reinterpret_cast<const i32x2*>(pv)[p];
+                e = int2{v[0], v[1]};
+                lat = a.plat[p];
+            }
             if (p == p1 - 1) e.x |= DWS_END;
             if (p == p0) e.x &= ~DWS_FIRST;
         }
@@ -1001,7 +1014,7 @@
     bool head_open = false;
     load_info(0, e_c, lat_c);
     if (live) {
-        head_open = (pv[p0].x & DWS_FIRST) == 0;
+        head_open = ((REC ? rec[p0][0] : pv[p0].x) & DWS_FIRST) == 0;
         if (PASS_A) w4 = buf_load16(wres, (uint32_t)a.plat[p0] * rowb + colb);
     }
     issue(e_c, lat_c, 0, xa, la, ga, wa);
@@ -1173,9 +1186,10 @@
     }
 }
 
-template <int NV>
+template <int NV, bool REC>
 __global__ __launch_bounds__(256) void dw_finalize_light_kernel(DwSlicesArgs a, int n_cut_blocks) {
     constexpr int L = DWS_RUN;
+    const i32x4* const rec = reinterpret_cast<const i32x4*>(a.rec);
     __shared__ f32x4 sh[3][NV * 64];
     __shared__ float shdb[4];
     const int lane = threadIdx.x & 63, w = threadIdx.x >> 6;
@@ -1253,7 +1267,14 @@
             for (int p0 = s + w * q4 + lane; p0 < pend; p0 += 64 * 8) {
                 int2 pe[8];
 #pragma unroll
-                for (int u = 0; u < 8; ++u) pe[u] = (p0 + 64 * u < pend) ? a.pv2[p0 + 64 * u] : int2{0, 0};
+                for (int u = 0; u < 8; ++u) {
+                    if constexpr (REC) {
+                        const i32x4 v = p0 + 64 * u < pend ? rec[p0 + 64 * u] : i32x4{0, 0, 0, 0};
+                        pe[u] = int2{v[0], v[3]};
+                    } else {
+                        pe[u] = (p0 + 64 * u < pend) ? a.pv2[p0 + 64 * u] : int2{0, 0};
+                    }
+                }
 #pragma unroll
                 for (int u = 0; u < 8; ++u) {
                     if (p0 + 64 * u < pend) {
@@ -1340,10 +1361,19 @@
         for (int t = 0; t < 2; ++t) {
             const int p = s + li + 8 * j + 64 * t;
             if (p < e) {
-                const int2 pd = a.pv2[p];
+                int2 pd;
+                float vl;
+                if constexpr (REC) {
+                    const i32x4 v = rec[p];
+                    pd = int2{v[0], v[3]};
+                    vl = __int_as_float(v[2]);
+                } else {
+                    pd = a.pv2[p];
+                    vl = __int_as_float(a.pv[p].y);
+                }
                 const float dv = __int_as_float(pd.y);
                 dbs += dv;
-                dot = __builtin_fmaf(__int_as_float(a.pv[p].y), dv, dot);
+                dot = __builtin_fmaf(vl, dv, dot);
                 if (a.clear_bitmap != nullptr) a.clear_bitmap[(size_t)i * a.clear_words + (pd.x >> 12)] = 0u;
             }
         }
@@ -1880,6 +1910,16 @@
     const int grid = ((a.D / DWS_SLICE + 7) / 8) * 8 * wg_per_slice;
     const bool light = part == 0 && a.have_dval && a.wn2 != nullptr;
     if (!light) { a.sq_wave_dec = nullptr; a.sq_wave_enc = nullptr; }
+    if (a.rec != nullptr) {
+        if (!light || a.P > 1) return hipErrorInvalidValue;
+        hipLaunchKernelGGL((dw_slices_kernel<true, false, true>), dim3(grid), dim3(256), 0, stream, a, wg_per_slice);
+        hipLaunchKernelGGL((dw_slices_kernel<false, true, true>), dim3(grid), dim3(256), 0, stream, a, wg_per_slice);
+        const int n_cut = a.cut_list != nullptr ? std::min(2 * (n_runs - 1), 8192) : 0;
+        if (a.cut_list == nullptr && n_runs > 1) return hipErrorInvalidValue;
+        return dispatch_nv(a.D, [&](auto nv) {
+            hipLaunchKernelGGL((dw_finalize_light_kernel<decltype(nv)::value, true>), dim3(n_cut + (a.S + 31) / 32), dim3(256), 0, stream, a, n_cut);
+        });
+    }
     if (part != 2 && a.have_dval) {
         hipLaunchKernelGGL((dw_slices_kernel<true, false>), dim3(grid), dim3(256), 0, stream, a, wg_per_slice);
         if (a.clear_bitmap != nullptr && !light) hipLaunchKernelGGL(dw_clear_bitmap_kernel, dim3((max_pairs + 255) / 256), dim3(256), 0, stream, a);
@@ -1893,7 +1933,7 @@
         const int n_cut = a.cut_list != nullptr ? std::min(2 * (n_runs - 1), 8192) : 0;
         if (a.cut_list == nullptr && n_runs > 1) return hipErrorInvalidValue;
         return dispatch_nv(a.D, [&](auto nv) {
-            hipLaunchKernelGGL(dw_finalize_light_kernel<decltype(nv)::value>, dim3(n_cut + (a.S + 31) / 32), dim3(256), 0, stream, a, n_cut);
+            hipLaunchKernelGGL((dw_finalize_light_kernel<decltype(nv)::value, false>), dim3(n_cut + (a.S + 31) / 32), dim3(256), 0, stream, a, n_cut);
         });
     }
     return dispatch_nv(a.D, [&](auto nv) {
diff --git a/saev_amd/csrc/split.hip b/saev_amd/csrc/split.hip
--- a/saev_amd/csrc/split.hip
+++ b/saev_amd/csrc/split.hip
@@ -205,6 +205,36 @@
                           a.sq_part, a.W_T, a.wt_slices);
 }
 
+__device__ __forceinline__ void bias_finish_group(const double* __restrict__ dot_part, const float* __restrict__ sq_part, int nks,
+                                                  int S, int S_pad, const float* __restrict__ w_scale, const float* __restrict__ b_enc,
+                                                  float* __restrict__ b_shift, float* __restrict__ wg_max, float* __restrict__ b_seen,
+                                                  int g, int t, int nwg, float (*sh)[4]) {
+    const int sidx = g * 256 + t;
+    float out = 0.f, nrm = 0.f, dnrm = 0.f;
+    if (g < nwg && sidx < S) {
+        double acc = 0.0, sq = 0.0, dsq = 0.0;
+        for (int ks = 0; ks < nks; ++ks) {
+            acc += dot_part[(size_t)ks * S_pad + sidx];
+            sq += (double)sq_part[(size_t)ks * S_pad + sidx];
+            dsq += (double)sq_part[(size_t)(nks + ks) * S_pad + sidx];
+        }
+        const double sc = (double)(*w_scale);
+        const float be = b_enc[sidx];
+        out = (float)(acc / sc + (double)be);
+        b_shift[sidx] = out;
+        if (b_seen != nullptr) b_seen[sidx] = be;
+        nrm = (float)(sqrt(sq) / sc) * 1.000001f;
+        dnrm = (float)(sqrt(dsq) / sc) * 1.00001f;
+    }
+    float m = fabsf(out);
+    for (int o = 32; o > 0; o >>= 1) { m = fmaxf(m, __shfl_xor(m, o, 64)); nrm = fmaxf(nrm, __shfl_xor(nrm, o, 64)); dnrm = fmaxf(dnrm, __shfl_xor(dnrm, o, 64)); }
+    if ((t & 63) == 0) { sh[0][t >> 6] = m; sh[1][t >> 6] = nrm; sh[2][t >> 6] = dnrm; }
+    __syncthreads();
+    if (t < 3 && g < nwg) {
+        const float* q = sh[t];
+        wg_max[t * nwg + g] = fmaxf(fmaxf(q[0], q[1]), fmaxf(q[2], q[3]));
+    }
+}
 __device__ __forceinline__ float xprep_round_f16_sig(float v) {
     const uint32_t b = __float_as_uint(v);
     return __uint_as_float((b + 0x0FFFu + ((b >> 13) & 1u)) & 0xFFFFE000u);
@@ -213,8 +243,15 @@
     __shared__ float cs[256][33];
     __shared__ float cs2[32][33];
     __shared__ float shm[2][16];
+    if ((int)blockIdx.x < a.n_bias) {
+        const int t = threadIdx.x & 255, grp = threadIdx.x >> 8;
+        bias_finish_group(a.dot_part, a.sq_part, a.bias_nks, a.S, a.S_pad, a.w_scale, a.b_enc, a.b_shift, a.wg_max, nullptr,
+                          (int)blockIdx.x * 4 + grp, t, (a.S + 255) / 256, reinterpret_cast<float (*)[4]>(&cs[grp][0]));
+        return;
+    }
     const int nks = a.nks;
-    const int bid = blockIdx.x, blk = bid / nks, ks = bid % nks;
+    const int n_img = (int)gridDim.x - a.n_bias;
+    const int bid = (int)blockIdx.x - a.n_bias, blk = bid / nks, ks = bid % nks;
     const int i = threadIdx.x, lane = i & 63, w = i >> 6;
     const int rl = i >> 2, p = i & 3;
     const int c = p ^ ((4 - ((rl >> 2) & 3)) & 3);
@@ -291,7 +328,7 @@
     }
     if (a.stale != nullptr && i >= 128 && i < 192) {
         bool differs = false;
-        for (int sidx = bid * 64 + (i - 128); sidx < a.S; sidx += (int)gridDim.x * 64)
+        for (int sidx = bid * 64 + (i - 128); sidx < a.S; sidx += n_img * 64)
             differs |= __float_as_uint(a.b_enc[sidx]) != __float_as_uint(a.b_seen[sidx]);
         if (differs) atomicOr(a.stale, 1);
     }
@@ -303,31 +340,8 @@
                                                           float* __restrict__ b_shift, float* __restrict__ wg_max,
                                                           float* __restrict__ b_seen) {
     __shared__ float sh[3][4];
-    const int sidx = blockIdx.x * 256 + threadIdx.x;
-    float out = 0.f, nrm = 0.f, dnrm = 0.f;
-    if (sidx < S) {
-        double acc = 0.0, sq = 0.0, dsq = 0.0;
-        for (int ks = 0; ks < nks; ++ks) {
-            acc += dot_part[(size_t)ks * S_pad + sidx];
-            sq += (double)sq_part[(size_t)ks * S_pad + sidx];
-            dsq += (double)sq_part[(size_t)(nks + ks) * S_pad + sidx];
-        }
-        const double sc = (double)(*w_scale);
-        const float be = b_enc[sidx];
-        out = (float)(acc / sc + (double)be);
-        b_shift[sidx] = out;
-        if (b_seen != nullptr) b_seen[sidx] = be;
-        nrm = (float)(sqrt(sq) / sc) * 1.000001f;
-        dnrm = (float)(sqrt(dsq) / sc) * 1.00001f;
-    }
-    float m = fabsf(out);
-    for (int o = 32; o > 0; o >>= 1) { m = fmaxf(m, __shfl_xor(m, o, 64)); nrm = fmaxf(nrm, __shfl_xor(nrm, o, 64)); dnrm = fmaxf(dnrm, __shfl_xor(dnrm, o, 64)); }
-    if ((threadIdx.x & 63) == 0) { sh[0][threadIdx.x >> 6] = m; sh[1][threadIdx.x >> 6] = nrm; sh[2][threadIdx.x >> 6] = dnrm; }
-    __syncthreads();
-    if (threadIdx.x < 3) {
-        const float* q = sh[threadIdx.x];
-        wg_max[threadIdx.x * gridDim.x + blockIdx.x] = fmaxf(fmaxf(q[0], q[1]), fmaxf(q[2], q[3]));
-    }
+    bias_finish_group(dot_part, sq_part, nks, S, S_pad, w_scale, b_enc, b_shift, wg_max, b_seen, (int)blockIdx.x, (int)threadIdx.x,
+                      (int)gridDim.x, sh);
 }
 
 
@@ -388,6 +402,6 @@
 hipError_t launch_xprep(const XprepArgs& a, hipStream_t stream) {
     const int nblk = (a.n + 255) / 256;
     if (nblk <= 0 || a.D % 32 != 0) return hipErrorInvalidValue;
-    hipLaunchKernelGGL(xprep_kernel, dim3(nblk * a.nks), dim3(1024), 0, stream, a);
-    return hipGetLastError();
-}
+    hipLaunchKernelGGL(xprep_kernel, dim3(a.n_bias + nblk * a.nks), dim3(1024), 0, stream, a);
+    return hipGetLastError();
+}
diff --git a/saev_amd/csrc/tail.hip b/saev_amd/csrc/tail.hip
--- a/saev_amd/csrc/tail.hip
+++ b/saev_amd/csrc/tail.hip
@@ -406,6 +406,7 @@
         for (long i = bi * 256 + threadIdx.x; i < n; i += nb * 256) {
             const AdamElem r = adam_elem(a.p[off + i], scaled_grad(a.g[off + i], gs), a.m[off + i], a.v[off + i], a, step_size);
             a.p[off + i] = r.p; a.m[off + i] = r.m; a.v[off + i] = r.v;
+            if (seg && f.img.b_seen != nullptr && i < S) f.img.b_seen[i] = r.p;
         }
     }
 }
```

Measured after the change: 6.302 million, median of 6. 1.3% higher.
